# luigifreda/pyslam

Measured on AMD Instinct MI355X. Metric: RGB-D frames/sec fused (640x480, 5 mm voxel TSDF), higher is better.
Workload: dtype f32; 1 GPU; synthetic_640x480_5mm: synthetic 640x480 RGB-D @ 30 Hz stream, 5 mm TSDF (sdf_trunc 0.04 m, depth_trunc 4 m), 64 posed frames per step resident in HBM, Open3D ScalableTSDFVolume semantics; mode=multi-frame sweep (hv_tsdf_integrate_batch), units_allocated=31946, parity_pinned=False, clock_ramp_steps=60, full=False, build_digest=b0cf6d559847d2198173994ec0e18474b14d2966863d92f65f5939d93dcc7503

## Files before the change

include/hipvol.h:

```cpp
#ifndef PYSLAM_HIPVOL_H
#define PYSLAM_HIPVOL_H

#include <stdint.h>

#ifdef __cplusplus
extern "C" {
#endif

typedef struct hv_volume hv_volume;

typedef enum hv_status {
    HV_OK = 0,
    HV_ERR_INVALID = -1,
    HV_ERR_DEVICE = -2,
    HV_ERR_CAPACITY = -3,
    HV_ERR_MODE = -4
} hv_status;

typedef enum hv_mode {
    HV_MODE_VOXEL_GRID = 0,
    HV_MODE_VOXEL_SEMANTIC_GRID = 1,
    HV_MODE_VOXEL_SEMANTIC_PROBABILISTIC_GRID = 2,
    HV_MODE_TSDF = 3,
    HV_MODE_VOXEL_SEMANTIC_GRID2 = 11,
    HV_MODE_VOXEL_SEMANTIC_PROBABILISTIC_GRID2 = 12
} hv_mode;
typedef enum hv_loc { HV_HOST = 0, HV_DEVICE = 1 } hv_loc;
typedef enum hv_color_dtype { HV_COLOR_NONE = 0, HV_COLOR_U8 = 1, HV_COLOR_F32 = 2 } hv_color_dtype;
typedef enum hv_depth_dtype { HV_DEPTH_F32 = 0, HV_DEPTH_U16 = 1 } hv_depth_dtype;

typedef struct hv_config {
    int32_t mode;
    int32_t device;
    double voxel_size;
    double sdf_trunc;
    int32_t block_size;
    int32_t depth_sampling_stride;
    int64_t max_blocks;
    int64_t max_points;
} hv_config;


const char *hv_last_error(void);
int hv_device_count(void);
void hv_default_config(int32_t mode, hv_config *cfg);

int hv_create(const hv_config *cfg, hv_volume **out);
void hv_destroy(hv_volume *v);
int hv_reset(hv_volume *v);
int hv_synchronize(hv_volume *v);
int hv_set_stream(hv_volume *v, void *hip_stream);
void *hv_get_stream(hv_volume *v);

int hv_num_blocks(hv_volume *v, int64_t *n);
int hv_block_size(hv_volume *v, int32_t *bs);
int hv_reserve_blocks(hv_volume *v, int64_t new_max_blocks);
int hv_max_blocks(hv_volume *v, int64_t *n);
int hv_bytes_per_block(hv_volume *v, int64_t *bytes);
int hv_dropped_points(hv_volume *v, int64_t *n);

int hv_integrate_points(hv_volume *v, const float *points, int64_t n, const void *colors,
                        int32_t color_dtype, int32_t loc);
int hv_integrate_points_f64(hv_volume *v, const double *points, int64_t n, const void *colors,
                            int32_t color_dtype, int32_t loc);

int hv_integrate_rgbd_points(hv_volume *v, const void *depth, int32_t depth_dtype, double depth_scale,
                             const uint8_t *rgb, int32_t height, int32_t width, const double *intr,
                             const double *T_cw, double min_depth, double max_depth, int32_t loc);

int hv_integrate_rgbd_points_batch(hv_volume *v, const void *depth, int32_t depth_dtype, double depth_scale,
                                   const uint8_t *rgb, int32_t n_frames, int32_t height, int32_t width, const double *intr,
                                   const double *T_cw, double min_depth, double max_depth, int32_t loc);

int hv_remap(hv_volume *v, const void *src, int32_t src_kind, int32_t channels, int32_t height, int32_t width,
             const float *map_x, const float *map_y, int32_t linear, void *dst, int32_t loc);

int hv_filter_shadow_points(hv_volume *v, const float *depth, int32_t height, int32_t width, int32_t delta_x,
                            int32_t delta_y, float fill_value, float *out, int32_t loc);
int hv_filter_shadow_points_on_stream(hv_volume *v, const float *depth, int32_t height, int32_t width, int32_t delta_x,
                                      int32_t delta_y, float fill_value, float *out, void *stream);

int hv_get_voxels(hv_volume *v, int32_t min_count, float min_confidence, float *points,
                  float *colors, int64_t cap, int64_t *n, int32_t loc);
int hv_get_voxels_in_bb(hv_volume *v, const double *bbox, int32_t min_count, float min_confidence,
                        float *points, float *colors, int64_t cap, int64_t *n, int32_t loc);
int hv_get_voxels_in_frustum(hv_volume *v, const float *intr_f32, int32_t width, int32_t height,
                             const double *T_cw, float depth_max, float depth_min, int32_t min_count,
                             float min_confidence, float *points, float *colors, int64_t cap,
                             int64_t *n, int32_t loc);
int hv_carve(hv_volume *v, const float *intr_f32, int32_t width, int32_t height, const double *T_cw,
             float depth_max, float depth_min, const float *depth, float depth_threshold, int32_t loc);
int hv_remove_low_count_voxels(hv_volume *v, int32_t min_count);
int hv_size(hv_volume *v, int64_t *n);

int hv_dump_blocks(hv_volume *v, int32_t *keys, uint64_t *hashes, int32_t *counts, float *sums,
                   int64_t *n_blocks);
int hv_keys_from_points(hv_volume *v, const float *points, int64_t n, int32_t *voxel_keys,
                        int32_t *block_keys, int32_t *local_keys, uint64_t *block_hashes);

int hv_integrate_points_semantic(hv_volume *v, const void *points, int32_t point_dtype, int64_t n, const void *colors,
                                 int32_t color_dtype, const int32_t *class_ids, const int32_t *instance_ids,
                                 const float *depths, int32_t loc);
int hv_integrate_rgbd_semantic(hv_volume *v, const float *depth, const uint8_t *rgb, const int32_t *class_ids_image,
                               const int32_t *object_ids_image, int32_t height, int32_t width, const double *intr,
                               const double *T_cw, double min_depth, double max_depth, int32_t use_depths, int32_t loc);
int hv_get_voxels_semantic(hv_volume *v, int32_t min_count, float min_confidence, double *points, float *colors,
                           int32_t *class_ids, int32_t *object_ids, float *confidences, int64_t cap, int64_t *n);
int hv_get_voxels_semantic_in_bb(hv_volume *v, const double *bbox, int32_t min_count, float min_confidence, double *points,
                                 float *colors, int32_t *class_ids, int32_t *object_ids, float *confidences, int64_t cap,
                                 int64_t *n);
int hv_get_voxels_semantic_in_frustum(hv_volume *v, const float *intr_f32, int32_t width, int32_t height, const double *T_cw,
                                      float depth_max, float depth_min, int32_t min_count, float min_confidence, double *points,
                                      float *colors, int32_t *class_ids, int32_t *object_ids, float *confidences, int64_t cap,
                                      int64_t *n);
int hv_set_depth_threshold(hv_volume *v, float depth_threshold);
int hv_set_depth_decay_rate(hv_volume *v, float depth_decay_rate);
int hv_label_overflows(hv_volume *v, int64_t *n);
int hv_prob_nodes_used(hv_volume *v, int64_t *n);
int hv_assign_object_ids_to_instance_ids(hv_volume *v, const float *intr_f32, int32_t width, int32_t height, const double *T_cw,
                                         float depth_max, float depth_min, const int32_t *class_ids_image,
                                         const int32_t *instance_ids_image, const float *depth_image, float depth_threshold,
                                         int32_t do_carving, float min_vote_ratio, int32_t min_votes, int32_t *map_inst,
                                         int32_t *map_obj, int64_t cap, int64_t *n_map, int32_t loc);
int hv_assoc_vote(hv_volume *v, const float *intr_f32, int32_t width, int32_t height, const double *T_cw, float depth_max,
                  float depth_min, const int32_t *class_ids_image, const int32_t *instance_ids_image, const float *depth_image,
                  float depth_threshold, int32_t do_carving, int32_t loc);
int hv_assoc_pairs_fetch(hv_volume *v, uint64_t *pair_keys, int32_t *pair_counts, int64_t cap, int64_t *n_pairs);
int hv_assoc_pairs_set(hv_volume *v, const uint64_t *pair_keys, const int32_t *pair_counts, int64_t n_pairs);
int hv_assoc_pairs_export(hv_volume *v, int64_t *d_msg, int64_t cap);
int hv_assoc_pairs_import(hv_volume *v, const int64_t *d_msgs, int32_t world, int64_t cap);
int hv_assoc_decide(hv_volume *v, float min_vote_ratio, int32_t min_votes);
int hv_assoc_map_fetch(hv_volume *v, int32_t *map_inst, int32_t *map_obj, int64_t cap, int64_t *n_map);
int hv_remap_instance_ids_last(hv_volume *v, const int32_t *instance_ids, int32_t height, int32_t width, int32_t *out, int32_t loc);
int hv_semantic_fuse_keyframe(hv_volume *v, const float *depth, const uint8_t *rgb, const int32_t *class_ids_image,
                              const int32_t *instance_ids_image, int32_t height, int32_t width, const float *frustum_intr_f32,
                              float frustum_depth_max, float frustum_depth_min, const double *intr, const double *T_cw,
                              int32_t filter_shadow_points, int32_t use_instance_ids, float assoc_depth_threshold, int32_t do_carving,
                              float min_vote_ratio, int32_t min_votes, double min_depth, double max_depth, int32_t use_depths);
int32_t hv_peek_next_object_id(void);
void hv_set_next_object_id(int32_t id);
int hv_remap_instance_ids(hv_volume *v, const int32_t *instance_ids, int32_t height, int32_t width, const int32_t *map_inst,
                          const int32_t *map_obj, int64_t n_map, int32_t *out, int32_t loc);
int hv_object_segments_compute(hv_volume *v, int32_t min_count, float min_confidence, int64_t *n_rows, int64_t *n_objects);
int hv_object_segments_fetch(hv_volume *v, double *points, float *colors, int32_t *row_object_ids, int32_t *object_ids,
                             float *confidences, double *obbs);
int hv_compute_obb_pca(const double *points, int64_t n, double *obb);
int hv_merge_segments(hv_volume *v, int32_t instance_id1, int32_t instance_id2);
int hv_remove_segment(hv_volume *v, int32_t object_id);
int hv_remove_low_confidence_segments(hv_volume *v, int32_t min_confidence);
int hv_remove_low_confidence_voxels(hv_volume *v, float min_confidence);
int hv_dump_blocks_semantic(hv_volume *v, int32_t *keys, int32_t *ints, double *pos_sums, float *col_sums,
                            int64_t *n_blocks);
int hv_dump_blocks_semantic2(hv_volume *v, int32_t *keys, int32_t *ints, float *conf, double *pos_sums, float *col_sums,
                             int32_t *label_counts, int32_t *labels, float *log_probs, int32_t max_labels,
                             int64_t *n_blocks);
int hv_dump_marginals_semantic(hv_volume *v, float *object_confidences, float *class_confidences, int64_t *n_blocks);

int hv_tsdf_integrate(hv_volume *v, const void *depth, int32_t depth_dtype, const uint8_t *rgb,
                      int32_t height, int32_t width, const double *intr, const double *T_cw,
                      double depth_scale, double depth_trunc, int32_t loc);

int hv_tsdf_integrate_batch(hv_volume *v, const void *depth, int32_t depth_dtype, const uint8_t *rgb,
                            int32_t n_frames, int32_t height, int32_t width, const double *intr,
                            const double *T_cw, double depth_scale, double depth_trunc, int32_t loc);

int hv_tsdf_integrate_frames(hv_volume *v, const void *const *depth_frames, int32_t depth_dtype, const uint8_t *const *rgb_frames,
                             int32_t n_frames, int32_t height, int32_t width, const double *intr, const double *T_cw,
                             double depth_scale, double depth_trunc);

#define HV_TSDF_DEINTEGRATE_MAX_FRAMES 64
typedef struct hv_deintegrate_stats {
    int64_t units_listed;
    int64_t units_missing;
    int64_t voxels_removed;
    int64_t voxels_underflow;
} hv_deintegrate_stats;
int hv_tsdf_deintegrate(hv_volume *v, const void *depth, int32_t depth_dtype, const uint8_t *rgb, int32_t height, int32_t width,
                        const double *intr, const double *T_cw, double depth_scale, double depth_trunc, int32_t loc,
                        hv_deintegrate_stats *stats);
int hv_tsdf_deintegrate_batch(hv_volume *v, const void *depth, int32_t depth_dtype, const uint8_t *rgb, int32_t n_frames,
                              int32_t height, int32_t width, const double *intr, const double *T_cw, double depth_scale,
                              double depth_trunc, int32_t loc, hv_deintegrate_stats *stats);
int hv_tsdf_reintegrate_batch(hv_volume *v, const void *depth, int32_t depth_dtype, const uint8_t *rgb, int32_t n_frames,
                              int32_t height, int32_t width, const double *intr, const double *T_cw_old, const double *T_cw_new,
                              double depth_scale, double depth_trunc, int32_t loc, hv_deintegrate_stats *stats);

int hv_tsdf_set_rectify_maps(hv_volume *v, const float *map_x, const float *map_y, int32_t height, int32_t width, int32_t loc);

int hv_tsdf_set_color_order(hv_volume *v, int32_t bgr);

int hv_host_register(void *ptr, int64_t bytes);
int hv_host_unregister(void *ptr);

int hv_tsdf_set_tile(hv_volume *v, int32_t u0, int32_t v0, int32_t u1, int32_t v1);

int hv_set_owner(hv_volume *v, int32_t rank, int32_t world_size);
int hv_block_owner(const int32_t *block_keys, int64_t n, int32_t world_size, int32_t *owner);

int hv_tsdf_set_owner(hv_volume *v, int32_t rank, int32_t world_size);

int hv_tsdf_extract_mesh(hv_volume *v, double *vertices, double *vertex_colors, int64_t cap_vertices,
                         int32_t *triangles, int64_t cap_triangles, int64_t *n_vertices,
                         int64_t *n_triangles);
int hv_tsdf_extract_mesh_f32(hv_volume *v, float *vertices, float *vertex_colors, int64_t cap_vertices,
                             int32_t *triangles, int64_t cap_triangles, int64_t *n_vertices,
                             int64_t *n_triangles);
int hv_tsdf_extract_points(hv_volume *v, double *points, double *colors, int64_t cap, int64_t *n);
int hv_tsdf_extract_points_f32(hv_volume *v, float *points, float *colors, int64_t cap, int64_t *n);
int hv_tsdf_extract_point_normals(hv_volume *v, double *normals, int64_t cap, int64_t *n);

#define HV_RAYCAST_STEP_FRAC 0.8f
#define HV_RAYCAST_REFINE_ITERS 4
#define HV_RAYCAST_UNIT_EPS 0.01f
int hv_tsdf_ray_cast(hv_volume *v, int32_t height, int32_t width, const double *intr, const double *T_cw, double depth_min,
                     double depth_max, double weight_threshold, double depth_scale, float *depth, float *vertex, float *normal,
                     float *color, uint8_t *mask, int32_t loc);

#define HV_TRACK_MAX_LEVELS 8
#define HV_TRACK_MIN_INLIERS 6
#define HV_TRACK_PIVOT_REL 1e-10
#define HV_TRACK_CONVERGED 1e-6
#define HV_TRACK_TRACE_STRIDE 56
typedef struct hv_track_params {
    double depth_scale, depth_min, depth_max, weight_threshold;
    double depth_outlier_trunc;
    double depth_huber_delta;
    int32_t n_levels;
    int32_t iterations[HV_TRACK_MAX_LEVELS];
} hv_track_params;
typedef struct hv_track_result {
    double T_cw[16];
    double information[36];
    double fitness, inlier_rmse;
    int64_t inliers, valid;
    int32_t iterations[HV_TRACK_MAX_LEVELS];
    int32_t degenerate;
    int32_t success;
} hv_track_result;
int hv_tsdf_track(hv_volume *v, const void *depth, int32_t depth_dtype, int32_t height, int32_t width, const double *intr,
                  const double *T_cw_init, const hv_track_params *params, hv_track_result *result, double *trace, int64_t trace_cap,
                  int64_t *trace_rows, int32_t loc);

#define HV_TRACK_COLOR_TRACE_STRIDE 58
typedef struct hv_track_color_params {
    hv_track_params base;
    double intensity_weight;
    double intensity_huber_delta;
} hv_track_color_params;
typedef struct hv_track_color_result {
    hv_track_result base;
    int64_t photometric_inliers;
    double intensity_rmse;
} hv_track_color_result;
int hv_tsdf_track_color(hv_volume *v, const void *depth, int32_t depth_dtype, const uint8_t *color, int32_t height, int32_t width,
                        const double *intr, const double *T_cw_init, const hv_track_color_params *params, hv_track_color_result *result,
                        double *trace, int64_t trace_cap, int64_t *trace_rows, int32_t loc);

typedef struct hv_prune_stats {
    int64_t units_before, units_outside, units_empty, units_after;
} hv_prune_stats;
int hv_tsdf_prune(hv_volume *v, int32_t release_empty, const int32_t *unit_lo ,
                  const int32_t *unit_hi , hv_prune_stats *stats );

typedef struct hv_merge_stats {
    int64_t units_source, units_claimed, voxels_updated, voxels_trilinear, voxels_nearest;
} hv_merge_stats;
int hv_tsdf_integrate_volume(hv_volume *dst, hv_volume *src, const double *T_dst_src , hv_merge_stats *stats );

#define HV_REGISTER_MIN_INLIERS 6
#define HV_REGISTER_PIVOT_REL 1e-10
#define HV_REGISTER_CONVERGED 1e-6
#define HV_REGISTER_TRACE_STRIDE 54
typedef struct hv_register_params {
    double weight_threshold;
    double tsdf_band;
    double residual_trunc;
    double huber_delta;
    int32_t max_iterations;
    int32_t reserved;
} hv_register_params;
typedef struct hv_register_result {
    double T_dst_src[16];
    double information[36];
    double anchor[3];
    double fitness, inlier_rmse;
    int64_t inliers, candidates;
    int32_t iterations;
    int32_t success;
} hv_register_result;
int hv_tsdf_register_volume(hv_volume *dst, hv_volume *src, const double *T_init , const hv_register_params *params,
                            hv_register_result *result, double *trace, int64_t trace_cap, int64_t *trace_rows);

typedef enum hv_point_dtype { HV_F32 = 0, HV_F64 = 1 } hv_point_dtype;
#define HV_SAMPLE_OUTSIDE 0
#define HV_SAMPLE_UNOBSERVED 1
#define HV_SAMPLE_NEAREST 2
#define HV_SAMPLE_TRILINEAR 3
int hv_tsdf_sample_points(hv_volume *v, const void *points , int32_t point_dtype, int64_t n, double weight_threshold,
                          float *sdf , float *gradient , float *color , float *weight ,
                          uint8_t *status , int32_t loc);

#define HV_CHECK_INVALID 0
#define HV_CHECK_UNKNOWN 1
#define HV_CHECK_CONSISTENT 2
#define HV_CHECK_IN_FRONT 3
#define HV_CHECK_BEHIND 4
typedef struct hv_check_params {
    double depth_scale, depth_min, depth_max, weight_threshold, tolerance;
} hv_check_params;
typedef struct hv_check_stats {
    int64_t count[5];
} hv_check_stats;
int hv_tsdf_check_frame(hv_volume *v, const void *depth, int32_t depth_dtype, int32_t height, int32_t width, const double *intr,
                        const double *T_cw, const hv_check_params *params, float *sdf ,
                        uint8_t *cls , hv_check_stats *stats , int32_t loc);

#define HV_LOOKUP_MISSING 0
#define HV_LOOKUP_OWN 1
#define HV_LOOKUP_NEAR 2
#define HV_LOOKUP_INVALID 3
typedef struct hv_lookup_params {
    int32_t min_count;
// ... 94 lines not shown
```

pyslam_amd/_lib.py:

```python
import ctypes
import os

import numpy as np

from . import build as _build

_c = ctypes
_vp, _i64, _i32, _f32, _f64 = _c.c_void_p, _c.c_int64, _c.c_int32, _c.c_float, _c.c_double
_pi64 = _c.POINTER(_c.c_int64)
_pi32 = _c.POINTER(_c.c_int32)

HV_OK = 0
HV_MODE_VOXEL_GRID = 0
HV_MODE_VOXEL_SEMANTIC_GRID = 1
HV_MODE_VOXEL_SEMANTIC_PROBABILISTIC_GRID = 2
HV_MODE_TSDF = 3
HV_MODE_VOXEL_SEMANTIC_GRID2 = 11
HV_MODE_VOXEL_SEMANTIC_PROBABILISTIC_GRID2 = 12
HV_HOST, HV_DEVICE = 0, 1
HV_COLOR_NONE, HV_COLOR_U8, HV_COLOR_F32 = 0, 1, 2
HV_DEPTH_F32, HV_DEPTH_U16 = 0, 1


class HvConfig(_c.Structure):
# ... 102 lines not shown
        ("information", _f64 * 36),
        ("anchor", _f64 * 3),
        ("fitness", _f64),
        ("inlier_rmse", _f64),
        ("inliers", _i64),
        ("candidates", _i64),
        ("iterations", _i32),
        ("success", _i32),
    ]


HV_PACK_VERSION = 1
HV_PACK_HEADER_BYTES = 128


class HvPackInfo(_c.Structure):
    _fields_ = [("units", _i64), ("voxels", _i64), ("bytes", _i64)]


class HvPackedHeader(_c.Structure):
    _fields_ = [
        ("voxel_length", _f64),
        ("sdf_trunc", _f64),
        ("resolution", _i32),
        ("version", _i32),
        ("units", _i64),
        ("voxels", _i64),
        ("bytes", _i64),
    ]


HV_F32, HV_F64 = 0, 1
HV_SAMPLE_OUTSIDE, HV_SAMPLE_UNOBSERVED, HV_SAMPLE_NEAREST, HV_SAMPLE_TRILINEAR = 0, 1, 2, 3
HV_CHECK_INVALID, HV_CHECK_UNKNOWN, HV_CHECK_CONSISTENT, HV_CHECK_IN_FRONT, HV_CHECK_BEHIND = 0, 1, 2, 3, 4


class HvCheckParams(_c.Structure):
    _fields_ = [
        ("depth_scale", _f64),
        ("depth_min", _f64),
        ("depth_max", _f64),
        ("weight_threshold", _f64),
        ("tolerance", _f64),
    ]


class HvCheckStats(_c.Structure):
    _fields_ = [("count", _i64 * 5)]


HV_LOOKUP_MISSING, HV_LOOKUP_OWN, HV_LOOKUP_NEAR, HV_LOOKUP_INVALID = 0, 1, 2, 3


class HvLookupParams(_c.Structure):
    _fields_ = [("min_count", _i32), ("min_confidence", _f32), ("radius", _i32)]


class HvLookupStats(_c.Structure):
    _fields_ = [("points", _i64), ("own", _i64), ("near", _i64), ("missing", _i64), ("invalid", _i64)]


HV_DIST_UNKNOWN, HV_DIST_FREE, HV_DIST_INSIDE, HV_DIST_SITE = 0, 1, 2, 4
HV_DIST_MAX_SHAPE, HV_DIST_MAX_RADIUS = 4096, 1024


class HvDistanceParams(_c.Structure):
    _fields_ = [("origin", _i32 * 3), ("shape", _i32 * 3), ("radius", _i32), ("weight_threshold", _f64)]


class HvDistanceStats(_c.Structure):
    _fields_ = [("unknown", _i64), ("free", _i64), ("inside", _i64), ("sites", _i64), ("far", _i64)]


HV_COMPONENTS_MAX_MARGIN = 16


class HvComponentsStats(_c.Structure):
    _fields_ = [("units", _i64), ("sites", _i64), ("components", _i64), ("largest", _i64)]


class HvRemoveComponentsStats(_c.Structure):
    _fields_ = [("components", _i64), ("components_removed", _i64), ("sites", _i64), ("sites_removed", _i64), ("voxels_reset", _i64),
                ("units_changed", _i64), ("units_emptied", _i64)]


SIGNATURES = {
    "hv_last_error": (_c.c_char_p, []),
    "hv_device_count": (_i32, []),
    "hv_default_config": (None, [_i32, _c.POINTER(HvConfig)]),
    "hv_create": (_i32, [_c.POINTER(HvConfig), _c.POINTER(_vp)]),
    "hv_destroy": (None, [_vp]),
    "hv_reset": (_i32, [_vp]),
    "hv_synchronize": (_i32, [_vp]),
    "hv_set_stream": (_i32, [_vp, _vp]),
    "hv_get_stream": (_vp, [_vp]),
    "hv_num_blocks": (_i32, [_vp, _pi64]),
    "hv_block_size": (_i32, [_vp, _pi32]),
    "hv_reserve_blocks": (_i32, [_vp, _i64]),
    "hv_max_blocks": (_i32, [_vp, _pi64]),
    "hv_bytes_per_block": (_i32, [_vp, _pi64]),
    "hv_dropped_points": (_i32, [_vp, _pi64]),
    "hv_integrate_points": (_i32, [_vp, _vp, _i64, _vp, _i32, _i32]),
    "hv_integrate_points_f64": (_i32, [_vp, _vp, _i64, _vp, _i32, _i32]),
    "hv_integrate_rgbd_points": (_i32, [_vp, _vp, _i32, _f64, _vp, _i32, _i32, _vp, _vp, _f64, _f64, _i32]),
    "hv_integrate_rgbd_points_batch": (_i32, [_vp, _vp, _i32, _f64, _vp, _i32, _i32, _i32, _vp, _vp, _f64, _f64, _i32]),
    "hv_remap": (_i32, [_vp, _vp, _i32, _i32, _i32, _i32, _vp, _vp, _i32, _vp, _i32]),
    "hv_filter_shadow_points": (_i32, [_vp, _vp, _i32, _i32, _i32, _i32, _f32, _vp, _i32]),
    "hv_filter_shadow_points_on_stream": (_i32, [_vp, _vp, _i32, _i32, _i32, _i32, _f32, _vp, _vp]),
    "hv_get_voxels": (_i32, [_vp, _i32, _f32, _vp, _vp, _i64, _pi64, _i32]),
    "hv_get_voxels_in_bb": (_i32, [_vp, _vp, _i32, _f32, _vp, _vp, _i64, _pi64, _i32]),
    "hv_get_voxels_in_frustum": (_i32, [_vp, _vp, _i32, _i32, _vp, _f32, _f32, _i32, _f32, _vp, _vp, _i64, _pi64, _i32]),
    "hv_carve": (_i32, [_vp, _vp, _i32, _i32, _vp, _f32, _f32, _vp, _f32, _i32]),
    "hv_remove_low_count_voxels": (_i32, [_vp, _i32]),
    "hv_size": (_i32, [_vp, _pi64]),
    "hv_dump_blocks": (_i32, [_vp, _vp, _vp, _vp, _vp, _pi64]),
    "hv_keys_from_points": (_i32, [_vp, _vp, _i64, _vp, _vp, _vp, _vp]),
    "hv_integrate_points_semantic": (_i32, [_vp, _vp, _i32, _i64, _vp, _i32, _vp, _vp, _vp, _i32]),
    "hv_get_voxels_semantic": (_i32, [_vp, _i32, _f32, _vp, _vp, _vp, _vp, _vp, _i64, _pi64]),
    "hv_get_voxels_semantic_in_bb": (_i32, [_vp, _vp, _i32, _f32, _vp, _vp, _vp, _vp, _vp, _i64, _pi64]),
    "hv_get_voxels_semantic_in_frustum": (_i32, [_vp, _vp, _i32, _i32, _vp, _f32, _f32, _i32, _f32, _vp, _vp, _vp, _vp, _vp, _i64, _pi64]),
    "hv_set_depth_threshold": (_i32, [_vp, _f32]),
    "hv_dump_blocks_semantic": (_i32, [_vp, _vp, _vp, _vp, _vp, _pi64]),
    "hv_dump_blocks_semantic2": (_i32, [_vp, _vp, _vp, _vp, _vp, _vp, _vp, _vp, _vp, _i32, _pi64]),
    "hv_dump_marginals_semantic": (_i32, [_vp, _vp, _vp, _pi64]),
    "hv_set_depth_decay_rate": (_i32, [_vp, _f32]),
    "hv_integrate_rgbd_semantic": (_i32, [_vp, _vp, _vp, _vp, _vp, _i32, _i32, _vp, _vp, _f64, _f64, _i32, _i32]),
    "hv_label_overflows": (_i32, [_vp, _pi64]),
    "hv_prob_nodes_used": (_i32, [_vp, _pi64]),
    "hv_assign_object_ids_to_instance_ids": (_i32, [_vp, _vp, _i32, _i32, _vp, _f32, _f32, _vp, _vp, _vp, _f32, _i32, _f32, _i32,
                                                    _vp, _vp, _i64, _pi64, _i32]),
    "hv_assoc_vote": (_i32, [_vp, _vp, _i32, _i32, _vp, _f32, _f32, _vp, _vp, _vp, _f32, _i32, _i32]),
    "hv_assoc_pairs_fetch": (_i32, [_vp, _vp, _vp, _i64, _pi64]),
    "hv_assoc_pairs_set": (_i32, [_vp, _vp, _vp, _i64]),
    "hv_assoc_pairs_export": (_i32, [_vp, _vp, _i64]),
    "hv_assoc_pairs_import": (_i32, [_vp, _vp, _i32, _i64]),
    "hv_assoc_decide": (_i32, [_vp, _f32, _i32]),
    "hv_assoc_map_fetch": (_i32, [_vp, _vp, _vp, _i64, _pi64]),
    "hv_remap_instance_ids_last": (_i32, [_vp, _vp, _i32, _i32, _vp, _i32]),
    "hv_semantic_fuse_keyframe": (_i32, [_vp, _vp, _vp, _vp, _vp, _i32, _i32, _vp, _f32, _f32, _vp, _vp, _i32, _i32, _f32, _i32, _f32, _i32,
                                         _f64, _f64, _i32]),
    "hv_peek_next_object_id": (_i32, []),
    "hv_set_next_object_id": (None, [_i32]),
    "hv_remap_instance_ids": (_i32, [_vp, _vp, _i32, _i32, _vp, _vp, _i64, _vp, _i32]),
    "hv_object_segments_compute": (_i32, [_vp, _i32, _f32, _pi64, _pi64]),
    "hv_object_segments_fetch": (_i32, [_vp, _vp, _vp, _vp, _vp, _vp, _vp]),
    "hv_compute_obb_pca": (_i32, [_vp, _i64, _vp]),
    "hv_merge_segments": (_i32, [_vp, _i32, _i32]),
    "hv_remove_segment": (_i32, [_vp, _i32]),
    "hv_remove_low_confidence_segments": (_i32, [_vp, _i32]),
    "hv_remove_low_confidence_voxels": (_i32, [_vp, _f32]),
    "hv_tsdf_integrate": (_i32, [_vp, _vp, _i32, _vp, _i32, _i32, _vp, _vp, _f64, _f64, _i32]),
    "hv_tsdf_integrate_batch": (_i32, [_vp, _vp, _i32, _vp, _i32, _i32, _i32, _vp, _vp, _f64, _f64, _i32]),
    "hv_tsdf_integrate_frames": (_i32, [_vp, _vp, _i32, _vp, _i32, _i32, _i32, _vp, _vp, _f64, _f64]),
    "hv_tsdf_set_color_order": (_i32, [_vp, _i32]),
    "hv_host_register": (_i32, [_vp, _i64]),
    "hv_host_unregister": (_i32, [_vp]),
    "hv_tsdf_set_tile": (_i32, [_vp, _i32, _i32, _i32, _i32]),
    "hv_tsdf_set_rectify_maps": (_i32, [_vp, _vp, _vp, _i32, _i32, _i32]),
    "hv_tsdf_set_owner": (_i32, [_vp, _i32, _i32]),
    "hv_tsdf_extract_mesh": (_i32, [_vp, _vp, _vp, _i64, _vp, _i64, _pi64, _pi64]),
    "hv_tsdf_extract_mesh_f32": (_i32, [_vp, _vp, _vp, _i64, _vp, _i64, _pi64, _pi64]),
    "hv_tsdf_extract_points": (_i32, [_vp, _vp, _vp, _i64, _pi64]),
    "hv_tsdf_extract_points_f32": (_i32, [_vp, _vp, _vp, _i64, _pi64]),
    "hv_tsdf_extract_point_normals": (_i32, [_vp, _vp, _i64, _pi64]),
    "hv_tsdf_ray_cast": (_i32, [_vp, _i32, _i32, _vp, _vp, _f64, _f64, _f64, _f64, _vp, _vp, _vp, _vp, _vp, _i32]),
    "hv_tsdf_deintegrate": (_i32, [_vp, _vp, _i32, _vp, _i32, _i32, _vp, _vp, _f64, _f64, _i32, _c.POINTER(HvDeintegrateStats)]),
    "hv_tsdf_deintegrate_batch": (_i32, [_vp, _vp, _i32, _vp, _i32, _i32, _i32, _vp, _vp, _f64, _f64, _i32, _c.POINTER(HvDeintegrateStats)]),
    "hv_tsdf_reintegrate_batch": (_i32, [_vp, _vp, _i32, _vp, _i32, _i32, _i32, _vp, _vp, _vp, _f64, _f64, _i32,
                                         _c.POINTER(HvDeintegrateStats)]),
    "hv_tsdf_prune": (_i32, [_vp, _i32, _pi32, _pi32, _c.POINTER(HvPruneStats)]),
    "hv_tsdf_integrate_volume": (_i32, [_vp, _vp, _vp, _c.POINTER(HvMergeStats)]),
    "hv_tsdf_register_volume": (_i32, [_vp, _vp, _vp, _c.POINTER(HvRegisterParams), _c.POINTER(HvRegisterResult), _vp, _i64, _pi64]),
    "hv_tsdf_track": (_i32, [_vp, _vp, _i32, _i32, _i32, _vp, _vp, _vp, _vp, _vp, _i64, _pi64, _i32]),
    "hv_tsdf_track_color": (_i32, [_vp, _vp, _i32, _vp, _i32, _i32, _vp, _vp, _vp, _vp, _vp, _i64, _pi64, _i32]),
    "hv_tsdf_sample_points": (_i32, [_vp, _vp, _i32, _i64, _f64, _vp, _vp, _vp, _vp, _vp, _i32]),
    "hv_tsdf_check_frame": (_i32, [_vp, _vp, _i32, _i32, _i32, _vp, _vp, _c.POINTER(HvCheckParams), _vp, _vp, _c.POINTER(HvCheckStats), _i32]),
    "hv_lookup_points": (_i32, [_vp, _vp, _i32, _i64, _c.POINTER(HvLookupParams), _vp, _vp, _vp, _vp, _vp, _vp, _vp, _c.POINTER(HvLookupStats), _i32]),
    "hv_tsdf_distance_field": (_i32, [_vp, _c.POINTER(HvDistanceParams), _vp, _vp, _vp, _c.POINTER(HvDistanceStats), _i32]),
    "hv_tsdf_surface_components": (_i32, [_vp, _f64, _vp, _vp, _vp, _vp, _i64, _vp, _vp, _i64, _pi64, _pi64, _c.POINTER(HvComponentsStats), _i32]),
    "hv_tsdf_remove_components": (_i32, [_vp, _f64, _i64, _i32, _c.POINTER(HvRemoveComponentsStats)]),
    "hv_tsdf_dump": (_i32, [_vp, _vp, _vp, _vp, _vp, _pi64]),
    "hv_tsdf_touched": (_i32, [_vp, _vp, _i64, _pi64]),
    "hv_tsdf_export_numerators": (_i32, [_vp, _vp, _i64, _vp, _i32]),
    "hv_tsdf_import_numerators": (_i32, [_vp, _vp, _i64, _vp, _i32]),
    "hv_tsdf_unit_keys": (_i32, [_vp, _vp, _i64, _pi64]),
    "hv_tsdf_pack_size": (_i32, [_vp, _c.POINTER(HvPackInfo)]),
    "hv_tsdf_pack": (_i32, [_vp, _vp, _i64, _i32, _c.POINTER(HvPackInfo)]),
    "hv_tsdf_unpack": (_i32, [_vp, _vp, _i64, _i32, _c.POINTER(HvPackInfo)]),
    "hv_tsdf_packed_check": (_i32, [_vp, _i64, _c.POINTER(HvPackedHeader)]),
    "hv_tsdf_dirty_keys": (_i32, [_vp, _vp, _i64, _pi64]),
    "hv_tsdf_mark_merged": (_i32, [_vp]),
    "hv_set_owner": (_i32, [_vp, _i32, _i32]),
    "hv_block_owner": (_i32, [_vp, _i64, _i32, _vp]),
    "hv_merge_halo_plan": (_i32, [_vp, _vp, _i32, _i32, _vp, _vp, _i64, _pi64]),
    "hv_merge_halo_plan_held": (_i32, [_vp, _vp, _vp, _vp, _i32, _i32, _vp, _vp, _i64, _pi64]),
    "hv_merge_halo_pack": (_i32, [_vp, _vp, _i64, _vp, _i32]),
    "hv_merge_halo_unpack": (_i32, [_vp, _vp, _i64, _vp, _vp, _i32]),
    "hv_merge_halo_lists_device": (_i32, [_vp, _vp, _i64, _vp, _i64, _pi64, _pi64]),
    "hv_merge_halo_plan_device": (_i32, [_vp, _vp, _vp, _i64, _vp, _vp, _i64, _i32, _i32, _i32, _pi64]),
    "hv_merge_halo_plan_fetch": (_i32, [_vp, _vp, _vp, _i64, _pi64]),
    "hv_merge_halo_pack_planned": (_i32, [_vp, _i64, _i64, _vp]),
    "hv_merge_halo_unpack_planned": (_i32, [_vp, _i64, _i64, _vp]),
    "hv_profile_enable": (_i32, [_vp, _i32]),
    "hv_profile_read": (_i32, [_vp, _c.POINTER(_f64), _pi64, _pi64]),
    "hv_profile_read_launches": (_i32, [_vp, _vp, _i64, _pi64]),
}

_lib = None


class HipVolError(RuntimeError):
    """Raised for every non-zero hv_status; message = hv_last_error()."""


def library_path():
    return _build.LIB_PATH


def load():
    global _lib
    if _lib is not None:
        return _lib
    path = _build.LIB_PATH
    if not os.path.exists(path):
        _build.build(verbose=False)
    import torch

    lib = _c.CDLL(path)
    for name, (restype, argtypes) in SIGNATURES.items():
        fn = getattr(lib, name)
        fn.restype = restype
        fn.argtypes = argtypes
    _lib = lib
    return lib


def check(rc):
    if rc != HV_OK:
        msg = load().hv_last_error()
        raise HipVolError(msg.decode() if msg else f"hipvol error {rc}")


def ptr(a):
    if a is None:
        return None
    if isinstance(a, np.ndarray):
        return a.ctypes.data_as(_vp)
    if hasattr(a, "data_ptr"):
        return _vp(a.data_ptr())
    raise TypeError(f"unsupported buffer type {type(a)}")


def location(a):
    if a is not None and hasattr(a, "is_cuda") and a.is_cuda:
        return HV_DEVICE
    return HV_HOST
```

pyslam_amd/csrc/hv_common.h:

```cpp
#pragma once
#include <cstdint>
#include <cstdio>
#include <cstring>
#include <string>
#include <vector>

#include <hip/hip_runtime.h>

#include "hipvol.h"

#define HV_WAVE 64

void hv_set_error(const char *fmt, ...);

#define HV_HIP(call)                                                                               \
    do {                                                                                           \
        hipError_t e_ = (call);                                                                    \
        if (e_ != hipSuccess) {                                                                    \
            hv_set_error("%s failed: %s (%s:%d)", #call, hipGetErrorString(e_), __FILE__,          \
                         __LINE__);                                                                \
            return HV_ERR_DEVICE;                                                                  \
        }                                                                                          \
    } while (0)

#define HV_REQUIRE(cond, code, ...)                                                                \
    do {                                                                                           \
        if (!(cond)) {                                                                             \
            hv_set_error(__VA_ARGS__);                                                             \
            return (code);                                                                         \
        }                                                                                          \
    } while (0)

static constexpr int HV_KEY_BITS = 21;
static constexpr int32_t HV_KEY_BIAS = 1 << (HV_KEY_BITS - 1);
static constexpr uint64_t HV_KEY_MASK = (1ull << HV_KEY_BITS) - 1;
static constexpr uint64_t HV_EMPTY_KEY = ~0ull;

__host__ __device__ inline bool hv_key_in_range(int32_t x, int32_t y, int32_t z) {
    return x >= -HV_KEY_BIAS && x < HV_KEY_BIAS && y >= -HV_KEY_BIAS && y < HV_KEY_BIAS &&
           z >= -HV_KEY_BIAS && z < HV_KEY_BIAS;
}
__host__ __device__ inline uint64_t hv_pack_key(int32_t x, int32_t y, int32_t z) {
    return (uint64_t)(uint32_t)(x + HV_KEY_BIAS) | ((uint64_t)(uint32_t)(y + HV_KEY_BIAS) << HV_KEY_BITS) |
           ((uint64_t)(uint32_t)(z + HV_KEY_BIAS) << (2 * HV_KEY_BITS));
}
__host__ __device__ inline void hv_unpack_key(uint64_t k, int32_t &x, int32_t &y, int32_t &z) {
    x = (int32_t)(k & HV_KEY_MASK) - HV_KEY_BIAS;
    y = (int32_t)((k >> HV_KEY_BITS) & HV_KEY_MASK) - HV_KEY_BIAS;
    z = (int32_t)((k >> (2 * HV_KEY_BITS)) & HV_KEY_MASK) - HV_KEY_BIAS;
}
__host__ __device__ inline uint32_t hv_slot_hash(uint64_t k) {
    k ^= k >> 33;
    k *= 0xff51afd7ed558ccdull;
    k ^= k >> 33;
    k *= 0xc4ceb9fe1a85ec53ull;
    k ^= k >> 33;
    return (uint32_t)k;
}
__host__ __device__ inline int32_t hv_owner_of(uint64_t k, int32_t world) {
    k ^= k >> 29;
    k *= 0x9E3779B97F4A7C15ull;
    k ^= k >> 32;
    return (int32_t)((k >> 7) % (uint64_t)world);
}
__host__ __device__ inline uint64_t hv_reference_hash(int32_t x, int32_t y, int32_t z) {
    return (uint64_t)(int64_t)x ^ ((uint64_t)(int64_t)y << 1) ^ ((uint64_t)(int64_t)z << 2);
}

struct HvTable {
    unsigned long long *keys;
    int32_t *vals;
    unsigned long long *block_keys;
    int32_t *counters;
    uint32_t mask;
    int32_t max_blocks;
    void *prob_nodes;
    int32_t prob_node_cap;
};

struct HvBins {
    int32_t *cnt;
    uint32_t *inl;
    int32_t *touched;
    int32_t *len;
    unsigned long long *pg_keys;
    uint32_t *pg_data;
    uint32_t pg_mask;
    uint32_t epoch;
    int32_t touched_cap;
    int32_t idx_bits;
    int32_t parity;
};

enum {
    HV_CNT_BLOCKS = 0,
    HV_CNT_OVERFLOW = 1,
    HV_CNT_DROPPED = 2,
    HV_CNT_OUT = 5,
    HV_CNT_OUT2 = 6,
    HV_CNT_AUX = 7,
    HV_CNT_LABEL_OVERFLOW = 8,
    HV_CNT_PROB_NODES = 9,
    HV_CNT_TOUCH0 = 32,
    HV_CNT_TOUCH1 = 64,
    HV_CNT_COUNT = 96
};
#define HV_CNT_TOUCH(set) (HV_CNT_TOUCH0 + 32 * (set))
static constexpr int HV_TSDF_SETS = 2;
static constexpr size_t HV_CNT_TOUCH_SPAN_BYTES = sizeof(int32_t) * (32 * (HV_TSDF_SETS - 1) + 1);

#ifdef __HIPCC__
__device__ inline int32_t hv_table_find(const HvTable &t, uint64_t key) {
    uint32_t s = hv_slot_hash(key) & t.mask;
    for (uint32_t probe = 0; probe <= t.mask; ++probe) {
        const unsigned long long k = t.keys[s];
        if (k == key) return (int32_t)s;
        if (k == HV_EMPTY_KEY) return -1;
        s = (s + 1) & t.mask;
    }
    return -1;
}

__device__ inline int32_t hv_table_insert(const HvTable &t, uint64_t key) {
    uint32_t s = hv_slot_hash(key) & t.mask;
    for (uint32_t probe = 0; probe <= t.mask; ++probe) {
        unsigned long long k = t.keys[s];
        if (k == key) return (int32_t)s;
        if (k == HV_EMPTY_KEY) {
            k = atomicCAS(&t.keys[s], HV_EMPTY_KEY, (unsigned long long)key);
            if (k == HV_EMPTY_KEY) {
                const int32_t idx = atomicAdd(&t.counters[HV_CNT_BLOCKS], 1);
                if (idx >= t.max_blocks) {
                    atomicAdd(&t.counters[HV_CNT_OVERFLOW], 1);
                    return -1;
                }
                t.vals[s] = idx;
                t.block_keys[idx] = key;
                return (int32_t)s;
            }
            if (k == key) return (int32_t)s;
        }
        s = (s + 1) & t.mask;
    }
    atomicAdd(&t.counters[HV_CNT_OVERFLOW], 1);
    return -1;
}

__device__ inline int32_t hv_table_claim(const HvTable &t, uint64_t key, bool *is_new) {
    *is_new = false;
    uint32_t s = hv_slot_hash(key) & t.mask;
    for (uint32_t probe = 0; probe <= t.mask; ++probe) {
        unsigned long long k = t.keys[s];
        if (k == key) return (int32_t)s;
        if (k == HV_EMPTY_KEY) {
            k = atomicCAS(&t.keys[s], HV_EMPTY_KEY, (unsigned long long)key);
            if (k == HV_EMPTY_KEY) {
                *is_new = true;
                return (int32_t)s;
            }
            if (k == key) return (int32_t)s;
        }
        s = (s + 1) & t.mask;
    }
    atomicAdd(&t.counters[HV_CNT_OVERFLOW], 1);
    return -1;
}
__device__ inline void hv_table_assign(const HvTable &t, int32_t slot, uint64_t key, int32_t idx) {
    if (idx >= t.max_blocks) {
        atomicAdd(&t.counters[HV_CNT_OVERFLOW], 1);
        return;
    }
    t.vals[slot] = idx;
    t.block_keys[idx] = key;
}

__device__ inline int hv_lane_id() { return (int)(threadIdx.x & (HV_WAVE - 1)); }
__device__ __forceinline__ void hv_wave_lds_sync() {
    __builtin_amdgcn_fence(__ATOMIC_ACQ_REL, "wavefront");
    __builtin_amdgcn_wave_barrier();
}

__device__ inline int32_t hv_wave_append(int32_t *counter, bool pred) {
    const unsigned long long m = __ballot(pred);
    if (m == 0) return -1;
    const int lane = hv_lane_id();
    const int leader = __ffsll((long long)m) - 1;
    int32_t base = 0;
    if (lane == leader) base = atomicAdd(counter, (int32_t)__popcll(m));
    base = __shfl(base, leader);
    const unsigned long long lt = (lane == 0) ? 0ull : (~0ull >> (64 - lane));
    return pred ? base + (int32_t)__popcll(m & lt) : -1;
}

template <typename T>
__device__ __forceinline__ T hv_wave_sum(T x) {
#pragma unroll
    for (int o = HV_WAVE / 2; o > 0; o >>= 1) x += __shfl_xor(x, o, HV_WAVE);
    return x;
}
template <typename T>
__device__ __forceinline__ T hv_wave_min(T x) {
#pragma unroll
    for (int o = HV_WAVE / 2; o > 0; o >>= 1) x = min(x, __shfl_xor(x, o, HV_WAVE));
    return x;
}
template <typename T>
__device__ __forceinline__ T hv_wave_max(T x) {
#pragma unroll
    for (int o = HV_WAVE / 2; o > 0; o >>= 1) x = max(x, __shfl_xor(x, o, HV_WAVE));
    return x;
}

__device__ inline int32_t hv_keyset_insert(unsigned long long *keys, uint32_t mask, unsigned long long key, bool *is_new) {
    *is_new = false;
    uint32_t s = hv_slot_hash(key) & mask;
    for (uint32_t probe = 0; probe <= mask; ++probe) {
        unsigned long long k = keys[s];
        if (k == key) return (int32_t)s;
        if (k == HV_EMPTY_KEY) {
            k = atomicCAS(&keys[s], HV_EMPTY_KEY, key);
            if (k == HV_EMPTY_KEY) {
                *is_new = true;
                return (int32_t)s;
            }
            if (k == key) return (int32_t)s;
        }
        s = (s + 1) & mask;
    }
    return -1;
}
#endif

static constexpr int HV_TSDF_PLANES = 5;
static constexpr int HV_TSDF_R = 16;
static constexpr int HV_TSDF_RR = HV_TSDF_R * HV_TSDF_R;
static constexpr int HV_TSDF_RRR = HV_TSDF_RR * HV_TSDF_R;
static constexpr int HV_TSDF_PLANE_BYTES = HV_TSDF_RRR * 4;
static constexpr int HV_TSDF_UNIT_BYTES = HV_TSDF_PLANE_BYTES * HV_TSDF_PLANES;

__host__ __device__ __forceinline__ int hv_tsdf_word(int x, int y, int z) { return z * HV_TSDF_RR + x * HV_TSDF_R + y; }

#ifdef __HIPCC__
__device__ __forceinline__ bool hv_tsdf_unit_has_weight(const char *__restrict__ pool, int32_t unit, int lane) {
    const uint4 *w = (const uint4 *)(pool + (size_t)unit * HV_TSDF_UNIT_BYTES + HV_TSDF_PLANE_BYTES);
    bool seen = false;
    for (int k = 0; k < HV_TSDF_PLANE_BYTES / 1024 && !seen; k += 4) {
        const uint4 a = w[(k + 0) * 64 + lane], b = w[(k + 1) * 64 + lane], c = w[(k + 2) * 64 + lane], d = w[(k + 3) * 64 + lane];
        const uint32_t any = a.x | a.y | a.z | a.w | b.x | b.y | b.z | b.w | c.x | c.y | c.z | c.w | d.x | d.y | d.z | d.w;
        seen = __ballot(any != 0) != 0ull;
    }
    return seen;
}
#endif

struct __attribute__((aligned(16))) HvVoxel {
    int32_t count;
    float pos[3];
    float col[3];
    int32_t pad;
};
static_assert(sizeof(HvVoxel) == 32, "HvVoxel must be 32 bytes");

struct HvFrameParams {
    float sweep_k[16];
    float ext[12];
    float ext_scaled_col2[3];
    float fx, fy, cx, cy;
    float ffl_inv_x, ffl_inv_y;
    float voxel_length_f, half_voxel_length_f;
    float sdf_trunc_f, sdf_trunc_inv_f;
    float safe_width_f, safe_height_f;
    double unit_length;
    double pose[12];
    double fx_d, fy_d, cx_d, cy_d;
    double sdf_trunc_d;
    float depth_scale_f;
    double depth_trunc_d;
    int32_t H, W, stride;
    int32_t depth_is_u16;
    int32_t frame_id;
    int32_t tile_u0, tile_v0, tile_u1, tile_v1;
    int32_t tiled;
    int32_t owner_rank, owner_world;
    int32_t touch_box_bits;
    int32_t bgr;
};

struct HvStatus {
    int32_t blocks;
    int32_t overflow;
    int32_t seq;
    int32_t pad;
    int32_t assoc_flags;
    int32_t reserved[3];
};

#ifdef __HIPCC__
__device__ inline void hv_publish_status(const HvTable &t, HvStatus *status, int32_t seq) {
    volatile HvStatus *s = status;
    s->blocks = t.counters[HV_CNT_BLOCKS];
    s->overflow = t.counters[HV_CNT_OVERFLOW];
    __threadfence_system();
    s->seq = seq;
}
#endif

struct HvEventPair {
    hipEvent_t start, stop;
};

static inline bool hv_mode_is_semantic(int32_t mode) {
    return mode == HV_MODE_VOXEL_SEMANTIC_GRID || mode == HV_MODE_VOXEL_SEMANTIC_PROBABILISTIC_GRID || mode == HV_MODE_VOXEL_SEMANTIC_GRID2 ||
           mode == HV_MODE_VOXEL_SEMANTIC_PROBABILISTIC_GRID2;
}
static inline bool hv_mode_has_label_maps(int32_t mode) {
    return mode == HV_MODE_VOXEL_SEMANTIC_PROBABILISTIC_GRID || mode == HV_MODE_VOXEL_SEMANTIC_PROBABILISTIC_GRID2;
}

struct hv_volume {
    hv_config cfg;
    int device = 0;
    hipStream_t stream = nullptr;
    bool own_stream = true;

    HvTable table{};
    uint64_t table_capacity = 0;
    void *pool = nullptr;
    int64_t bytes_per_block = 0;
    int32_t *h_counters = nullptr;
    HvStatus *h_status = nullptr;
    HvStatus *d_status = nullptr;
    int32_t status_seq_issued = 0, status_seq_seen = 0;
    int64_t known_blocks = 0;
    int64_t max_new_per_call = 0;
    double avg_new_per_call = 0.0;
    bool status_exact = false;
    bool overflow_latched = false;

    int32_t *touched_stamp = nullptr;
    int32_t *touched_list = nullptr;
    uint64_t *touched_mask = nullptr;
    void *frame_px = nullptr;
    int color_bgr = 0;
    int touch_box_bits = 2048;
    int32_t frame_counter = 0;
    int32_t merge_stamp = 0;
    int32_t last_touch_parity = 0;
    bool touch_counters_clean = true;
    void *batch_buf = nullptr;
    size_t batch_buf_bytes = 0;
    void *batch_buf2 = nullptr;
    size_t batch_buf2_bytes = 0;
    hipEvent_t ev_h2d = nullptr;
    hipStream_t stream_aux = nullptr;
    hipEvent_t ev_prep = nullptr;
    hipEvent_t ev_presweep = nullptr;
    int batch_parity = 0;
    bool pipe_armed = false;
    uint64_t pipe_version = 0;
    float *rect_map_x = nullptr, *rect_map_y = nullptr;
    size_t rect_map_x_bytes = 0, rect_map_y_bytes = 0;
    int32_t rect_W = 0, rect_H = 0;
    void *rect_buf = nullptr;
    size_t rect_buf_bytes = 0;
    float *mult_table = nullptr;
    size_t mult_table_bytes = 0;
    float mult_key[4] = {0.f, 0.f, 0.f, 0.f};
    int32_t mult_W = 0, mult_H = 0;
    void *pinned_params[4] = {nullptr, nullptr, nullptr, nullptr};
    hipEvent_t params_ev[4] = {nullptr, nullptr, nullptr, nullptr};
    int params_idx = 0;
    int32_t tile[4] = {0, 0, 0, 0};
    int32_t owner_rank = 0, owner_world = 1;
    float sem_depth_threshold = 10.0f;
    float sem_depth_decay_rate = 0.07f;
    void *assoc_buf = nullptr;
    void *assoc_clean = nullptr;
    size_t assoc_clean_bytes = 0;
    size_t assoc_buf_bytes = 0;
    int32_t assoc_pending_cap = 0;
    int assoc_state = 0;
    void *segments_cache = nullptr;
    unsigned long long *occ = nullptr;
    void *semb_tasks = nullptr;
    size_t semb_tasks_bytes = 0;

    void *stage_a = nullptr;
    void *stage_b = nullptr;
    size_t stage_a_bytes = 0, stage_b_bytes = 0;
    void *hs_pinned[2] = {nullptr, nullptr};
    size_t hs_pinned_bytes[2] = {0, 0};
    hipEvent_t hs_pinned_done[2] = {nullptr, nullptr};
    void *hs_dev[2][2] = {{nullptr, nullptr}, {nullptr, nullptr}};
    size_t hs_dev_bytes[2][2] = {{0, 0}, {0, 0}};
    hipEvent_t hs_dev_ready[2] = {nullptr, nullptr};
    hipEvent_t hs_dev_free[2] = {nullptr, nullptr};
    bool hs_dev_free_valid[2] = {false, false};
    hipStream_t hs_stream = nullptr;
    int hs_set = 0, hs_slot = 0;

    uint32_t *sort_keys_in = nullptr, *sort_keys_out = nullptr;
    uint32_t *sort_vals_in = nullptr, *sort_vals_out = nullptr;
    void *sort_tmp = nullptr;
    size_t sort_tmp_bytes = 0;
    HvBins bins{};
    uint64_t bins_cap = 0;
    bool bins_clean = false;
    uint32_t bins_epoch = 0;
    void *bin_rec = nullptr;
    size_t bin_rec_bytes = 0;
    float *scratch_points = nullptr;
    float *scratch_colors = nullptr;
    int local_bits = 9;

    uint64_t content_version = 1;
    uint64_t mesh_cache_version = 0, points_cache_version = 0;
    int64_t mesh_cache_nv = 0, mesh_cache_nt = 0, points_cache_n = 0;
    bool mesh_cache_f32 = false, points_cache_f32 = false;
    void *unit_masks = nullptr;
    uint64_t unit_masks_version = 0;
    int unit_masks_units = 0;
    uint64_t extract_epoch = 1;
    int unit_cache_cap = 0;
    uint64_t unit_masks_epoch = 0, mc_epoch = 0, pc_epoch = 0;
    int32_t unit_masks_stamp = -1, mc_stamp = -1, pc_stamp = -1;
    int mc_units = 0, pc_units = 0;
    void *mc_cache = nullptr;
    void *pc_cache = nullptr;

    void *out_a = nullptr;
    void *out_b = nullptr;
    void *out_c = nullptr;
    size_t out_a_bytes = 0, out_b_bytes = 0, out_c_bytes = 0;
    void *raycast_buf = nullptr;
    size_t raycast_buf_bytes = 0;
    void *sample_buf = nullptr;
    size_t sample_buf_bytes = 0;
    void *dist_buf = nullptr;
    size_t dist_buf_bytes = 0;
    void *track_buf = nullptr;
    size_t track_buf_bytes = 0;
    void *shadow_ring = nullptr;
    int shadow_ring_next = 0;
    void *halo_plan = nullptr;
    size_t halo_plan_bytes = 0;
    int64_t halo_plan_n = 0;
    void *kf_buf = nullptr;
    size_t kf_buf_bytes = 0;
    void *deint_buf = nullptr;
    size_t deint_buf_bytes = 0;
    uint64_t deint_miss_cap = 0;

    bool profiling = false;
    std::vector<HvEventPair> events;
    size_t events_used = 0;
    int64_t prof_units = 0;
};

int hv_ensure_buffer(hv_volume *v, void **buf, size_t *cur, size_t want);
int hv_capacity_gate(hv_volume *v, bool *checked);
int hv_claims_fit(hv_volume *v);
static constexpr int HV_RETRY_CLAIM = 1000;
int hv_rekey_in_place(hv_volume *v, int64_t keep);
int32_t hv_next_status_seq(hv_volume *v);
void hv_launch_publish_status(hv_volume *v);
int hv_read_counters(hv_volume *v);
int hv_tsdf_require_whole_map(const hv_volume *v, const char *fn, const char *subject);
int hv_tsdf_drain(hv_volume *v, const char *fn, bool refuse_overflow, int64_t *used);
int hv_tsdf_key_order(hv_volume *v, int64_t used, std::vector<int32_t> &order, std::vector<int32_t> *xyz_in_order);
struct HvScratch {
    std::vector<void *> held;
    HvScratch() = default;
    HvScratch(const HvScratch &) = delete;
    HvScratch &operator=(const HvScratch &) = delete;
    ~HvScratch() {
        for (void *p : held) (void)hipFree(p);
    }
    template <typename T>
    hipError_t get(T **p, size_t n) {
        void *raw = nullptr;
        const hipError_t e = hipMalloc(&raw, (n > 0 ? n : 1) * sizeof(T));
        if (e == hipSuccess) held.push_back(raw);
        *p = (T *)raw;
        return e;
    }
};
int hv_rectify_frames_device(hv_volume *v, hipStream_t s, const void *d_depth, int32_t depth_dtype, const uint8_t *d_rgb, int n_frames,
                             int height, int width, void *d_depth_out, uint8_t *d_rgb_out);
int hv_stage_in(hv_volume *v, const void *src, size_t bytes, int32_t loc, int which, const void **dev);
int hv_stage_out(hv_volume *v, int32_t loc, size_t head, const size_t *sizes, void *const *user, void **dev, int count);
int hv_h2d(hv_volume *v, void *dst, const void *src, size_t bytes);
int hv_h2d_lazy(hv_volume *v, void *dst, const void *src, size_t bytes, bool *pending);
int hv_h2d_fence(hv_volume *v, bool pending);
int hv_stage_frames(hv_volume *v, const void *const *depth_ptrs, const void *depth_base, size_t depth_frame_bytes,
                    const void *const *rgb_ptrs, const void *rgb_base, size_t rgb_frame_bytes, int n_frames,
                    const void **d_depth, const void **d_rgb, int *set);
int hv_stage_frames_consumed(hv_volume *v, int set, hipStream_t consumer);
void hv_profile_begin(hv_volume *v);
void hv_profile_end(hv_volume *v, int64_t units);
void hv_invert4x4(const double *m, double *out);
int hv_ray_cast_launch(hv_volume *v, int32_t height, int32_t width, const double *intr, const double *T_cw, double depth_min,
                       double depth_max, double weight_threshold, double depth_scale, float *depth, float *vertex, float *normal,
                       float *color, uint8_t *mask);
void hv_segments_cache_free(void *cache);
void hv_launch_tsdf_import_claim(hv_volume *v, const int32_t *d_keys, int64_t k);
// ... 1 lines not shown
```

pyslam_amd/csrc/hv_core.hip:

```cpp
#include <cstdarg>
#include <cstdlib>

#include <immintrin.h>

#include <algorithm>
#include <array>
#include <condition_variable>
#include <functional>
#include <mutex>
#include <thread>

#include "hv_common.h"

static thread_local std::string g_last_error;

void hv_set_error(const char *fmt, ...) {
    char buf[1024];
    va_list ap;
    va_start(ap, fmt);
    vsnprintf(buf, sizeof(buf), fmt, ap);
    va_end(ap);
    g_last_error = buf;
}

// ... 498 lines not shown
    return n;
}

void hv_default_config(int32_t mode, hv_config *cfg) {
    memset(cfg, 0, sizeof(*cfg));
    cfg->mode = mode;
    cfg->device = 0;
    if (mode == HV_MODE_TSDF) {
        cfg->voxel_size = 0.015;
        cfg->sdf_trunc = 0.04;
        cfg->block_size = 16;
        cfg->depth_sampling_stride = 4;
        cfg->max_blocks = 1 << 16;
    } else {
        cfg->voxel_size = 0.015;
        cfg->sdf_trunc = 0.0;
        cfg->block_size = 8;
        cfg->depth_sampling_stride = 1;
        cfg->max_blocks = 1 << 19;
    }
    cfg->max_points = 2 * 1024 * 1024;
}

int hv_create(const hv_config *cfg, hv_volume **out) {
    HV_REQUIRE(cfg != nullptr && out != nullptr, HV_ERR_INVALID, "hv_create: null argument");
    HV_REQUIRE(cfg->mode == HV_MODE_VOXEL_GRID || hv_mode_is_semantic(cfg->mode) || cfg->mode == HV_MODE_TSDF, HV_ERR_INVALID,
               "hv_create: unsupported mode %d", cfg->mode);
    HV_REQUIRE(cfg->voxel_size > 0.0, HV_ERR_INVALID, "hv_create: voxel_size must be > 0");
    HV_REQUIRE(cfg->max_blocks > 0 && cfg->max_blocks < (1ll << 30), HV_ERR_INVALID,
               "hv_create: max_blocks out of range");
    HV_REQUIRE(cfg->max_points > 0 && cfg->max_points < (1ll << 31), HV_ERR_INVALID,
               "hv_create: max_points out of range");
    if (cfg->mode == HV_MODE_TSDF) {
        HV_REQUIRE(cfg->block_size == 16, HV_ERR_INVALID,
                   "hv_create: TSDF mode supports volume_unit_resolution 16 only (Open3D default)");
        HV_REQUIRE(cfg->sdf_trunc > 0.0, HV_ERR_INVALID, "hv_create: sdf_trunc must be > 0");
        HV_REQUIRE(cfg->depth_sampling_stride >= 1, HV_ERR_INVALID, "hv_create: bad sampling stride");
    } else {
        HV_REQUIRE(cfg->block_size >= 1 && cfg->block_size <= 16, HV_ERR_INVALID,
                   "hv_create: block_size must be in [1,16]");
    }
    int ndev = 0;
    HV_HIP(hipGetDeviceCount(&ndev));
    HV_REQUIRE(ndev > 0 && cfg->device >= 0 && cfg->device < ndev, HV_ERR_DEVICE,
               "hv_create: HIP device %d not available (%d devices)", cfg->device, ndev);
    hipDeviceProp_t prop;
    HV_HIP(hipGetDeviceProperties(&prop, cfg->device));
    HV_REQUIRE(strncmp(prop.gcnArchName, "gfx950", 6) == 0, HV_ERR_DEVICE,
               "hv_create: device %d is %s; this library is built for gfx950 only", cfg->device,
               prop.gcnArchName);
    HV_HIP(hipSetDevice(cfg->device));

    hv_volume *v = new hv_volume();
    v->cfg = *cfg;
    v->device = cfg->device;
    int rc = HV_OK;
    auto fail = [&](int code) {
        hv_destroy(v);
        return code;
    };
#define HV_TRY(call)                                                                               \
    do {                                                                                           \
        hipError_t e_ = (call);                                                                    \
        if (e_ != hipSuccess) {                                                                    \
            hv_set_error("%s failed: %s", #call, hipGetErrorString(e_));                           \
            return fail(HV_ERR_DEVICE);                                                            \
        }                                                                                          \
    } while (0)

    HV_TRY(hipStreamCreateWithFlags(&v->stream, hipStreamNonBlocking));
    v->own_stream = true;

    const int64_t nvox = (int64_t)cfg->block_size * cfg->block_size * cfg->block_size;
    v->bytes_per_block = cfg->mode == HV_MODE_TSDF ? nvox * 4 * HV_TSDF_PLANES
                         : hv_mode_has_label_maps(cfg->mode) ? nvox * 128
                         : hv_mode_is_semantic(cfg->mode)    ? nvox * 64
                                                             : nvox * (int64_t)sizeof(HvVoxel);
    if (hv_mode_has_label_maps(cfg->mode)) v->sem_depth_threshold = 5.0f;
    v->local_bits = 0;
    while ((1ll << v->local_bits) < nvox) v->local_bits++;

    v->table_capacity = next_pow2((uint64_t)cfg->max_blocks * 4);
    if (v->table_capacity < 1024) v->table_capacity = 1024;
    if (cfg->mode != HV_MODE_TSDF && (v->table_capacity << v->local_bits) >= (1ull << 32)) {
        hv_set_error("hv_create: max_blocks too large for 32-bit (slot, voxel) sort keys");
        return fail(HV_ERR_INVALID);
    }
    v->table.mask = (uint32_t)(v->table_capacity - 1);
    v->table.max_blocks = (int32_t)cfg->max_blocks;
    HV_TRY(hipMalloc(&v->table.keys, sizeof(uint64_t) * v->table_capacity));
    HV_TRY(hipMalloc(&v->table.vals, sizeof(int32_t) * v->table_capacity));
    HV_TRY(hipMalloc(&v->table.block_keys, sizeof(uint64_t) * cfg->max_blocks));
    HV_TRY(hipMalloc(&v->table.counters, sizeof(int32_t) * HV_CNT_COUNT));
    HV_TRY(hipHostMalloc((void **)&v->h_counters, sizeof(int32_t) * HV_CNT_COUNT));
    memset(v->h_counters, 0, sizeof(int32_t) * HV_CNT_COUNT);
    HV_TRY(hipHostMalloc((void **)&v->h_status, sizeof(HvStatus), hipHostMallocMapped));
    memset(v->h_status, 0, sizeof(HvStatus));
    HV_TRY(hipHostGetDevicePointer((void **)&v->d_status, v->h_status, 0));
    HV_TRY(hipMalloc(&v->pool, (size_t)cfg->max_blocks * v->bytes_per_block));

    if (cfg->mode == HV_MODE_TSDF) {
        HV_TRY(hipMalloc(&v->touched_stamp, sizeof(int32_t) * v->table_capacity));
        HV_TRY(hipMalloc(&v->touched_list, sizeof(int32_t) * HV_TSDF_SETS * cfg->max_blocks));
        HV_TRY(hipMalloc(&v->touched_mask, sizeof(uint64_t) * HV_TSDF_SETS * v->table_capacity));
        HV_TRY(hipMalloc(&v->frame_px, 8 * (size_t)cfg->max_points));
        if (const char *tb = getenv("HV_TSDF_TOUCH_BOX_BITS")) v->touch_box_bits = std::min(std::max(atoi(tb), 0), 2048);
    } else {
        HV_TRY(hipMalloc(&v->sort_keys_in, sizeof(uint32_t) * cfg->max_points));
        HV_TRY(hipMalloc(&v->sort_keys_out, sizeof(uint32_t) * cfg->max_points));
        HV_TRY(hipMalloc(&v->sort_vals_in, sizeof(uint32_t) * cfg->max_points));
        HV_TRY(hipMalloc(&v->sort_vals_out, sizeof(uint32_t) * cfg->max_points));
        HV_TRY(hipMalloc(&v->scratch_points, sizeof(float) * 3 * cfg->max_points));
        HV_TRY(hipMalloc(&v->scratch_colors, sizeof(float) * 3 * cfg->max_points));
        if (cfg->mode != HV_MODE_VOXEL_GRID) {
            const size_t occ_words = ((size_t)cfg->max_blocks * nvox + 63) / 64;
            HV_TRY(hipMalloc((void **)&v->occ, sizeof(unsigned long long) * occ_words));
            HV_TRY(hipMemsetAsync(v->occ, 0, sizeof(unsigned long long) * occ_words, v->stream));
        }
        if (hv_mode_has_label_maps(cfg->mode)) {
            int64_t cap = std::max<int64_t>(1 << 16, (int64_t)cfg->max_blocks * 4);
            if (const char *e = getenv("HV_PROB_NODE_CAP")) cap = std::max<int64_t>(atoll(e), 1);
            cap = std::min<int64_t>(cap, INT32_MAX / 2);
            HV_TRY(hipMalloc(&v->table.prob_nodes, (size_t)cap * 128));
            v->table.prob_node_cap = (int32_t)cap;
        }
    }
#undef HV_TRY
    HV_HIP(hipMemsetAsync(v->pool, 0, (size_t)cfg->max_blocks * v->bytes_per_block, v->stream));
    rc = hv_reset(v);
    if (rc != HV_OK) return fail(rc);
    *out = v;
    return HV_OK;
}

void hv_destroy(hv_volume *v) {
    if (!v) return;
    (void)hipSetDevice(v->device);
    if (v->stream_aux) (void)hipStreamSynchronize(v->stream_aux);
    if (v->stream) (void)hipStreamSynchronize(v->stream);
    if (v->hs_stream) (void)hipStreamSynchronize(v->hs_stream);
    for (int i = 0; i < 2; ++i) {
        if (v->hs_pinned[i]) (void)hipHostFree(v->hs_pinned[i]);
        for (int a = 0; a < 2; ++a)
            if (v->hs_dev[i][a]) (void)hipFree(v->hs_dev[i][a]);
        if (v->hs_pinned_done[i]) (void)hipEventDestroy(v->hs_pinned_done[i]);
        if (v->hs_dev_ready[i]) (void)hipEventDestroy(v->hs_dev_ready[i]);
        if (v->hs_dev_free[i]) (void)hipEventDestroy(v->hs_dev_free[i]);
    }
    if (v->hs_stream) (void)hipStreamDestroy(v->hs_stream);
    void *bufs[] = {v->table.keys, v->table.vals, v->table.block_keys, v->table.counters, v->pool,
                    v->touched_stamp, v->touched_list, v->touched_mask, v->frame_px,
                    v->stage_a, v->stage_b, v->sort_keys_in, v->sort_keys_out, v->sort_vals_in,
                    v->sort_vals_out, v->sort_tmp, v->scratch_points, v->scratch_colors, v->out_a,
                    v->out_b, v->out_c, v->rect_map_x, v->rect_map_y, v->rect_buf, v->batch_buf, v->assoc_buf, v->mult_table, v->bins.cnt, v->bins.inl, v->bins.touched, v->bins.len, v->bins.pg_keys, v->bins.pg_data, v->bin_rec, v->batch_buf2, v->unit_masks, v->occ, v->semb_tasks, v->table.prob_nodes, v->shadow_ring, v->mc_cache, v->pc_cache, v->kf_buf, v->halo_plan, v->raycast_buf, v->track_buf, v->deint_buf, v->sample_buf, v->dist_buf};
    for (void *b : bufs)
        if (b) (void)hipFree(b);
    if (v->h_counters) (void)hipHostFree(v->h_counters);
    if (v->h_status) (void)hipHostFree(v->h_status);
    hv_segments_cache_free(v->segments_cache);
    for (int i = 0; i < 4; ++i) {
        if (v->pinned_params[i]) (void)hipHostFree(v->pinned_params[i]);
        if (v->params_ev[i]) (void)hipEventDestroy(v->params_ev[i]);
    }
    for (auto &p : v->events) {
        (void)hipEventDestroy(p.start);
        (void)hipEventDestroy(p.stop);
    }
    if (v->ev_h2d) (void)hipEventDestroy(v->ev_h2d);
    if (v->ev_prep) (void)hipEventDestroy(v->ev_prep);
    if (v->ev_presweep) (void)hipEventDestroy(v->ev_presweep);
    if (v->stream_aux) (void)hipStreamDestroy(v->stream_aux);
    if (v->stream && v->own_stream) (void)hipStreamDestroy(v->stream);
    delete v;
}

int hv_reset(hv_volume *v) {
    HV_REQUIRE(v != nullptr, HV_ERR_INVALID, "hv_reset: null volume");
    HV_HIP(hipSetDevice(v->device));
    int64_t used = 0;
    if (v->frame_counter != 0 || v->h_counters[HV_CNT_BLOCKS] != 0) {
        int rc = hv_read_counters(v);
        if (rc != HV_OK) return rc;
        used = v->h_counters[HV_CNT_BLOCKS];
        if (used > v->cfg.max_blocks) used = v->cfg.max_blocks;
    }
    if (used > 0) HV_HIP(hipMemsetAsync(v->pool, 0, (size_t)used * v->bytes_per_block, v->stream));
    if (used > 0 && v->occ) {
        const int64_t nvox = (int64_t)v->cfg.block_size * v->cfg.block_size * v->cfg.block_size;
        HV_HIP(hipMemsetAsync(v->occ, 0, sizeof(unsigned long long) * (size_t)((used * nvox + 63) / 64), v->stream));
    }
    HV_HIP(hipMemsetAsync(v->table.keys, 0xFF, sizeof(uint64_t) * v->table_capacity, v->stream));
    HV_HIP(hipMemsetAsync(v->table.vals, 0xFF, sizeof(int32_t) * v->table_capacity, v->stream));
    HV_HIP(hipMemsetAsync(v->table.counters, 0, sizeof(int32_t) * HV_CNT_COUNT, v->stream));
    if (v->touched_stamp) HV_HIP(hipMemsetAsync(v->touched_stamp, 0, sizeof(int32_t) * v->table_capacity, v->stream));
    if (v->touched_mask) HV_HIP(hipMemsetAsync(v->touched_mask, 0, sizeof(uint64_t) * HV_TSDF_SETS * v->table_capacity, v->stream));
    memset(v->h_counters, 0, sizeof(int32_t) * HV_CNT_COUNT);
    v->content_version += 1;
    v->extract_epoch += 1;
    v->frame_counter = 0;
    v->merge_stamp = 0;
    HV_HIP(hipStreamSynchronize(v->stream));
    memset(v->h_status, 0, sizeof(HvStatus));
    v->status_seq_issued = v->status_seq_seen = 0;
    v->known_blocks = 0;
    v->max_new_per_call = 0;
    v->avg_new_per_call = 0.0;
    v->status_exact = true;
    v->bins_clean = false;
    v->last_touch_parity = 0;
    v->touch_counters_clean = true;
    v->overflow_latched = false;
    return HV_OK;
}

int hv_synchronize(hv_volume *v) {
    HV_REQUIRE(v != nullptr, HV_ERR_INVALID, "hv_synchronize: null volume");
    HV_HIP(hipStreamSynchronize(v->stream));
    return HV_OK;
}

int hv_set_stream(hv_volume *v, void *hip_stream) {
    HV_REQUIRE(v != nullptr, HV_ERR_INVALID, "hv_set_stream: null volume");
    HV_HIP(hipStreamSynchronize(v->stream));
    if (v->own_stream && v->stream) HV_HIP(hipStreamDestroy(v->stream));
    v->stream = (hipStream_t)hip_stream;
    v->own_stream = false;
    return HV_OK;
}

void *hv_get_stream(hv_volume *v) { return v ? (void *)v->stream : nullptr; }

__global__ void k_rehash(HvTable t, const unsigned long long *__restrict__ block_keys, int32_t n) {
    const int32_t idx = blockIdx.x * blockDim.x + threadIdx.x;
    if (idx >= n) return;
    const unsigned long long key = block_keys[idx];
    uint32_t s = hv_slot_hash(key) & t.mask;
    for (uint32_t probe = 0; probe <= t.mask; ++probe) {
        if (atomicCAS(&t.keys[s], HV_EMPTY_KEY, key) == HV_EMPTY_KEY) {
            t.vals[s] = idx;
            return;
        }
        s = (s + 1) & t.mask;
    }
}

__global__ void k_restamp(HvTable old_t, HvTable new_t, const int32_t *__restrict__ old_stamp, int32_t *__restrict__ new_stamp, int32_t n) {
    const int32_t idx = blockIdx.x * blockDim.x + threadIdx.x;
    if (idx >= n) return;
    const unsigned long long key = new_t.block_keys[idx];
    const int32_t so = hv_table_find(old_t, key), sn = hv_table_find(new_t, key);
    if (so >= 0 && sn >= 0) new_stamp[sn] = old_stamp[so];
}

static int hv_rebuild(hv_volume *v, int64_t new_max_blocks, int64_t keep);

int hv_reserve_blocks(hv_volume *v, int64_t new_max_blocks) {
    HV_REQUIRE(v != nullptr, HV_ERR_INVALID, "hv_reserve_blocks: null volume");
    if (new_max_blocks <= v->cfg.max_blocks) return HV_OK;
    return hv_rebuild(v, new_max_blocks, -1);
}

static int hv_rebuild(hv_volume *v, int64_t new_max_blocks, int64_t keep) {
    HV_REQUIRE(new_max_blocks < (1ll << 30), HV_ERR_INVALID, "hv_reserve_blocks: max_blocks out of range");
    const uint64_t new_cap = next_pow2((uint64_t)new_max_blocks * 4);
    HV_REQUIRE(v->cfg.mode == HV_MODE_TSDF || (new_cap << v->local_bits) < (1ull << 32), HV_ERR_CAPACITY,
               "hv_reserve_blocks: %lld blocks are too many for 32-bit (slot, voxel) sort keys", (long long)new_max_blocks);
    HV_HIP(hipSetDevice(v->device));
    HV_HIP(hipStreamSynchronize(v->stream));
    v->extract_epoch += 1;
    int rc = hv_read_counters(v);
    if (rc != HV_OK) return rc;
    int64_t used = std::min<int64_t>(v->h_counters[HV_CNT_BLOCKS], v->cfg.max_blocks);
    if (keep >= 0) used = std::min(used, keep);
    size_t free_b = 0, total_b = 0;
    HV_HIP(hipMemGetInfo(&free_b, &total_b));
    const size_t need = (size_t)new_max_blocks * v->bytes_per_block + new_cap * 24 + (size_t)new_max_blocks * 16;
    HV_REQUIRE(need < free_b, HV_ERR_CAPACITY, "hv_reserve_blocks: %.1f GiB needed, %.1f GiB of HBM free", need / 1073741824.0,
               free_b / 1073741824.0);
    void *pool = nullptr;
    unsigned long long *keys = nullptr, *block_keys = nullptr, *occ = nullptr;
    int32_t *vals = nullptr, *stamp = nullptr, *list = nullptr;
    uint64_t *mask = nullptr;
    auto release = [&]() {
        for (void *p : {pool, (void *)keys, (void *)vals, (void *)block_keys, (void *)stamp, (void *)list, (void *)mask, (void *)occ})
            if (p) (void)hipFree(p);
    };
#define HV_TRY_GROW(call)                                                                          \
    do {                                                                                           \
        hipError_t e_ = (call);                                                                    \
        if (e_ != hipSuccess) {                                                                    \
            hv_set_error("hv_reserve_blocks: %s failed: %s", #call, hipGetErrorString(e_));        \
            release();                                                                             \
            return HV_ERR_DEVICE;                                                                  \
        }                                                                                          \
    } while (0)
    HV_TRY_GROW(hipMalloc(&pool, (size_t)new_max_blocks * v->bytes_per_block));
    HV_TRY_GROW(hipMalloc((void **)&keys, sizeof(uint64_t) * new_cap));
    HV_TRY_GROW(hipMalloc((void **)&vals, sizeof(int32_t) * new_cap));
    HV_TRY_GROW(hipMalloc((void **)&block_keys, sizeof(uint64_t) * new_max_blocks));
    HV_TRY_GROW(hipMemcpyAsync(pool, v->pool, (size_t)used * v->bytes_per_block, hipMemcpyDeviceToDevice, v->stream));
    HV_TRY_GROW(hipMemsetAsync((char *)pool + (size_t)used * v->bytes_per_block, 0, (size_t)(new_max_blocks - used) * v->bytes_per_block,
                               v->stream));
    HV_TRY_GROW(hipMemcpyAsync(block_keys, v->table.block_keys, sizeof(uint64_t) * used, hipMemcpyDeviceToDevice, v->stream));
    if (v->occ) {
        const int64_t nvox = (int64_t)v->cfg.block_size * v->cfg.block_size * v->cfg.block_size;
        const size_t new_words = ((size_t)new_max_blocks * nvox + 63) / 64, used_words = ((size_t)used * nvox + 63) / 64;
        HV_TRY_GROW(hipMalloc((void **)&occ, sizeof(unsigned long long) * new_words));
        HV_TRY_GROW(hipMemsetAsync(occ, 0, sizeof(unsigned long long) * new_words, v->stream));
        if (used_words) HV_TRY_GROW(hipMemcpyAsync(occ, v->occ, sizeof(unsigned long long) * used_words, hipMemcpyDeviceToDevice, v->stream));
    }
    HV_TRY_GROW(hipMemsetAsync(keys, 0xFF, sizeof(uint64_t) * new_cap, v->stream));
    HV_TRY_GROW(hipMemsetAsync(vals, 0xFF, sizeof(int32_t) * new_cap, v->stream));
    HvTable nt = v->table;
    nt.keys = keys;
    nt.vals = vals;
    nt.block_keys = block_keys;
    nt.mask = (uint32_t)(new_cap - 1);
    nt.max_blocks = (int32_t)new_max_blocks;
    if (used > 0) hipLaunchKernelGGL(k_rehash, dim3((unsigned)((used + 255) / 256)), dim3(256), 0, v->stream, nt, block_keys, (int32_t)used);
    HV_TRY_GROW(hipGetLastError());
    if (v->cfg.mode == HV_MODE_TSDF) {
        HV_TRY_GROW(hipMalloc((void **)&stamp, sizeof(int32_t) * new_cap));
        HV_TRY_GROW(hipMalloc((void **)&list, sizeof(int32_t) * HV_TSDF_SETS * new_max_blocks));
        HV_TRY_GROW(hipMalloc((void **)&mask, sizeof(uint64_t) * HV_TSDF_SETS * new_cap));
        HV_TRY_GROW(hipMemsetAsync(stamp, 0, sizeof(int32_t) * new_cap, v->stream));
        HV_TRY_GROW(hipMemsetAsync(mask, 0, sizeof(uint64_t) * HV_TSDF_SETS * new_cap, v->stream));
        if (used > 0 && v->touched_stamp != nullptr)
            hipLaunchKernelGGL(k_restamp, dim3((unsigned)((used + 255) / 256)), dim3(256), 0, v->stream, v->table, nt,
                               (const int32_t *)v->touched_stamp, stamp, (int32_t)used);
        HV_TRY_GROW(hipGetLastError());
    }
    const int32_t fixed[2] = {(int32_t)used, 0};
    HV_TRY_GROW(hipMemcpyAsync(&v->table.counters[HV_CNT_BLOCKS], fixed, sizeof(fixed), hipMemcpyHostToDevice, v->stream));
    if (v->cfg.mode == HV_MODE_TSDF) {
        HV_TRY_GROW(hipMemsetAsync(&v->table.counters[HV_CNT_TOUCH0], 0, HV_CNT_TOUCH_SPAN_BYTES, v->stream));
        v->touch_counters_clean = true;
    }
    HV_TRY_GROW(hipStreamSynchronize(v->stream));
#undef HV_TRY_GROW
    if (v->cfg.mode == HV_MODE_TSDF) {
        (void)hipFree(v->touched_stamp);
        (void)hipFree(v->touched_list);
        (void)hipFree(v->touched_mask);
        v->touched_stamp = stamp;
        v->touched_list = list;
        v->touched_mask = mask;
    }
    if (occ) {
        (void)hipFree(v->occ);
        v->occ = occ;
    }
    (void)hipFree(v->pool);
    (void)hipFree(v->table.keys);
// ... 170 lines not shown
```

pyslam_amd/csrc/hv_tsdf.hip:

```cpp
#include <algorithm>
#include <array>
#include <cmath>
#include <cstring>
#include <numeric>

#include "hv_tsdf_device.h"

__global__ __launch_bounds__(256) void k_tsdf_multiplier_table(HvFrameParams P, float *__restrict__ out) {
    const int i = blockIdx.x * blockDim.x + threadIdx.x;
    if (i >= P.H * P.W) return;
    out[i] = hv_multiplier(P, i % P.W, i / P.W);
}


__global__ __launch_bounds__(256) void k_tsdf_prep_touch(HvTable table, int32_t *__restrict__ stamp,
                                                          int32_t *__restrict__ list, int parity,
                                                          const void *__restrict__ depth_raw,
                                                          const uint8_t *__restrict__ rgb,
                                                          uint2 *__restrict__ frame_px, HvFrameParams P,
                                                          int n_touch_blocks) {
    const int64_t npx = (int64_t)P.H * P.W;
    if ((int)blockIdx.x >= n_touch_blocks) {
        const int64_t i = (int64_t)((int)blockIdx.x - n_touch_blocks) * blockDim.x + threadIdx.x;
        if (i >= npx) return;
// ... 68 lines not shown
}

template <int ZB>
__device__ __forceinline__ void hv_tsdf_slabs(const HvFrameParams &P, const uint2 *__restrict__ frame_px, char *__restrict__ unit, int wordb,
                                              float (&pc)[4][3], float inc0, float inc1, float inc2) {
    float tv[ZB][4];
    uint32_t cv[ZB][4];
    unsigned mask = 0;
    bool near_plane = false;
#pragma unroll
    for (int c = 0; c < 4; ++c) {
        const float e = pc[c][2] + (float)ZB * inc2;
        near_plane |= (int)(fminf(pc[c][2], e) < 0x1p-10f) & (int)(fmaxf(pc[c][2], e) > -0x1p-10f);
    }
    if (P.tiled || __any(near_plane)) {
#pragma unroll
        for (int zz = 0; zz < ZB; ++zz) {
#pragma unroll
            for (int c = 0; c < 4; ++c) {
                if (hv_tsdf_eval_fast<true, false>(P, frame_px, nullptr, pc[c][0], pc[c][1], pc[c][2], tv[zz][c], cv[zz][c]))
                    mask |= 1u << (zz * 4 + c);
                pc[c][0] += inc0;
                pc[c][1] += inc1;
                pc[c][2] += inc2;
            }
        }
    } else {
#pragma unroll
        for (int zz = 0; zz < ZB; ++zz) {
#pragma unroll
            for (int c = 0; c < 4; ++c) {
                if (hv_tsdf_eval_fast<false, false>(P, frame_px, nullptr, pc[c][0], pc[c][1], pc[c][2], tv[zz][c], cv[zz][c]))
                    mask |= 1u << (zz * 4 + c);
                pc[c][0] += inc0;
                pc[c][1] += inc1;
                pc[c][2] += inc2;
            }
        }
    }
    float4 vt[ZB];
    uint4 vw[ZB], vr[ZB], vg[ZB], vb[ZB];
#pragma unroll
    for (int zz = 0; zz < ZB; ++zz) {
        if ((mask >> (zz * 4)) & 15u) {
            const int q = (wordb + zz * HV_TSDF_RR) >> 2;
            vt[zz] = ((const float4 *)(unit + 0 * HV_TSDF_PLANE_BYTES))[q];
            vw[zz] = ((const uint4 *)(unit + 1 * HV_TSDF_PLANE_BYTES))[q];
            vr[zz] = ((const uint4 *)(unit + 2 * HV_TSDF_PLANE_BYTES))[q];
            vg[zz] = ((const uint4 *)(unit + 3 * HV_TSDF_PLANE_BYTES))[q];
            vb[zz] = ((const uint4 *)(unit + 4 * HV_TSDF_PLANE_BYTES))[q];
        }
    }
#pragma unroll
    for (int zz = 0; zz < ZB; ++zz) {
        const unsigned m = (mask >> (zz * 4)) & 15u;
        if (m) {
            hv_tsdf_apply(m & 1u, tv[zz][0], cv[zz][0], vt[zz].x, vw[zz].x, vr[zz].x, vg[zz].x, vb[zz].x);
            hv_tsdf_apply(m & 2u, tv[zz][1], cv[zz][1], vt[zz].y, vw[zz].y, vr[zz].y, vg[zz].y, vb[zz].y);
            hv_tsdf_apply(m & 4u, tv[zz][2], cv[zz][2], vt[zz].z, vw[zz].z, vr[zz].z, vg[zz].z, vb[zz].z);
            hv_tsdf_apply(m & 8u, tv[zz][3], cv[zz][3], vt[zz].w, vw[zz].w, vr[zz].w, vg[zz].w, vb[zz].w);
            const int q = (wordb + zz * HV_TSDF_RR) >> 2;
            ((float4 *)(unit + 0 * HV_TSDF_PLANE_BYTES))[q] = vt[zz];
            ((uint4 *)(unit + 1 * HV_TSDF_PLANE_BYTES))[q] = vw[zz];
            ((uint4 *)(unit + 2 * HV_TSDF_PLANE_BYTES))[q] = vr[zz];
            ((uint4 *)(unit + 3 * HV_TSDF_PLANE_BYTES))[q] = vg[zz];
            ((uint4 *)(unit + 4 * HV_TSDF_PLANE_BYTES))[q] = vb[zz];
        }
    }
}

__global__ __launch_bounds__(256) void k_tsdf_integrate(HvTable table, const int32_t *__restrict__ list,
                                                         int parity, char *__restrict__ pool,
                                                         const uint2 *__restrict__ frame_px, HvFrameParams P,
                                                         HvStatus *status, int32_t status_seq) {
    int n_touched = table.counters[HV_CNT_TOUCH(parity)];
    if (n_touched > table.max_blocks) n_touched = table.max_blocks;
    if (blockIdx.x == 0 && threadIdx.x == 0) {
        table.counters[HV_CNT_TOUCH(parity ^ 1)] = 0;
        hv_publish_status(table, status, status_seq);
    }
    const int wave = threadIdx.x >> 6;
    const int lane = threadIdx.x & 63;
    const int x = lane >> 2;
    const int y0 = (lane & 3) << 2;
    const int z0 = wave * 4;
    const float inc0 = P.ext_scaled_col2[0], inc1 = P.ext_scaled_col2[1], inc2 = P.ext_scaled_col2[2];

    for (int t = blockIdx.x; t < n_touched; t += gridDim.x) {
        const int32_t slot = list[t];
        const int32_t idx = table.vals[slot];
        if (idx < 0) continue;
        int32_t ux, uy, uz;
        hv_unpack_key(table.keys[slot], ux, uy, uz);
        const double o0 = (double)ux * P.unit_length;
        const double o1 = (double)uy * P.unit_length;
        const double o2 = (double)uz * P.unit_length;
        const float p0 = (float)((double)(P.half_voxel_length_f + P.voxel_length_f * (float)x) + o0);
        const float p2 = (float)((double)P.half_voxel_length_f + o2);
        float pc[4][3];
#pragma unroll
        for (int c = 0; c < 4; ++c) {
            const float p1 = (float)((double)(P.half_voxel_length_f + P.voxel_length_f * (float)(y0 + c)) + o1);
#pragma unroll
            for (int r = 0; r < 3; ++r) {
                pc[c][r] = ((P.ext[r * 4 + 0] * p0 + P.ext[r * 4 + 1] * p1) + P.ext[r * 4 + 2] * p2) + P.ext[r * 4 + 3];
            }
        }
        for (int s = 0; s < z0; ++s) {
#pragma unroll
            for (int c = 0; c < 4; ++c) {
                pc[c][0] += inc0;
                pc[c][1] += inc1;
                pc[c][2] += inc2;
            }
        }
        char *unit = pool + (int64_t)idx * HV_TSDF_UNIT_BYTES;
        constexpr int ZB = 2;
#pragma unroll
        for (int zb = 0; zb < 4; zb += ZB) hv_tsdf_slabs<ZB>(P, frame_px, unit, hv_tsdf_word(x, y0, z0 + zb), pc, inc0, inc1, inc2);
    }
}

__device__ __forceinline__ void hv_touch_batch_patch(const HvTable &table, const HvFrameParams &P, const void *depth_f, const int patch,
                                                     HvTouchScratch &scratch, const int f, unsigned long long *__restrict__ frame_mask,
                                                     int32_t *__restrict__ stamp, int32_t *__restrict__ list, const int batch_stamp,
                                                     const int parity) {
    const unsigned long long fbit = 1ull << f;
    hv_touch_patch(table, P, depth_f, patch, scratch,
                   [&](unsigned long long key, int32_t ux, int32_t uy, int32_t uz) {
                       if (!hv_unit_hits_tile(P, ux, uy, uz)) return;
                       const int32_t slot = hv_table_insert(table, key);
                       if (slot < 0) return;
                       const unsigned long long seen = __hip_atomic_load(&frame_mask[slot], __ATOMIC_RELAXED, __HIP_MEMORY_SCOPE_AGENT);
                       const int32_t stamped = __hip_atomic_load(&stamp[slot], __ATOMIC_RELAXED, __HIP_MEMORY_SCOPE_AGENT);
                       if (!(seen & fbit)) atomicOr(&frame_mask[slot], fbit);
                       if (stamped != batch_stamp) {
                           const int32_t old = atomicExch(&stamp[slot], batch_stamp);
                           if (old != batch_stamp) {
                               const int32_t at = atomicAdd(&table.counters[HV_CNT_TOUCH(parity)], 1);
                               if (at < table.max_blocks) list[at] = slot;
                           }
                       }
                   });
}

__global__ __launch_bounds__(256) void k_tsdf_prep_touch_batch(HvTable table, int32_t *__restrict__ stamp,
                                                                unsigned long long *__restrict__ frame_mask,
                                                                int32_t *__restrict__ list, int batch_stamp,
                                                                const char *__restrict__ depth_raw, int64_t depth_stride,
                                                                const uint8_t *__restrict__ rgb,
                                                                uint2 *__restrict__ frame_px,
                                                                const HvFrameParams *__restrict__ Ps, int n_prep_blocks,
                                                                int n_touch_blocks, int n_frames, int parity,
                                                                const float *__restrict__ mult12) {
    int f, bx;
    const bool touch_role = (int)blockIdx.x < n_touch_blocks * n_frames;
    if (touch_role) {
        f = (int)blockIdx.x / n_touch_blocks;
        bx = (int)blockIdx.x % n_touch_blocks;
    } else {
        const int b = (int)blockIdx.x - n_touch_blocks * n_frames;
        f = b / n_prep_blocks;
        bx = b % n_prep_blocks;
    }
    const HvFrameParams &P = Ps[f];
    const int64_t npx = (int64_t)P.H * P.W;
    const void *depth_f = depth_raw + (int64_t)f * depth_stride;
    const uint8_t *rgb_f = rgb + (int64_t)f * npx * 3;
    if (!touch_role) {
        hv_pack_px4(P, f, ((int64_t)bx * blockDim.x + threadIdx.x) * 4, depth_f, rgb_f, frame_px, mult12);
        return;
    }
    __shared__ HvTouchScratch scratch[4];
    const int patch = bx * 4 + (int)(threadIdx.x / HV_WAVE);
    if (patch < hv_touch_patches(P))
        hv_touch_batch_patch(table, P, depth_f, patch, scratch[threadIdx.x / HV_WAVE], f, frame_mask, stamp, list, batch_stamp, parity);
}

typedef float hv_f2 __attribute__((ext_vector_type(2)));

__device__ __forceinline__ hv_f2 hv_fma2(hv_f2 a, hv_f2 b, hv_f2 c) { return __builtin_elementwise_fma(a, b, c); }
__device__ __forceinline__ hv_f2 hv_splat(float x) { return hv_f2{x, x}; }

struct HvSweepFrameK {
    hv_f2 e04, e15, e26, e37;
    float e8, e11;
    hv_f2 e9_10, i01;
    float i2;
};
__device__ __forceinline__ HvSweepFrameK hv_sweep_frame_k(const HvFrameParams *__restrict__ Ps, int f) {
    const float *k = Ps[f].sweep_k;
    return HvSweepFrameK{hv_f2{k[0], k[1]}, hv_f2{k[2], k[3]}, hv_f2{k[4], k[5]}, hv_f2{k[6], k[7]}, k[8], k[9], hv_f2{k[10], k[11]}, hv_f2{k[12], k[13]}, k[14]};
}

static constexpr unsigned HV_SWEEP_XCD_GROUP = 2;
__device__ __forceinline__ int hv_sweep_items(const int n_units, const int parts) {
    constexpr int G = HV_SWEEP_XCD_GROUP;
    return (n_units + 8 * G - 1) / (8 * G) * 8 * G * parts;
}
__device__ __forceinline__ void hv_sweep_item(const unsigned item, const unsigned parts, int &t, int &part) {
    constexpr unsigned G = HV_SWEEP_XCD_GROUP;
    const unsigned xcd = item & 7u, j = item >> 3;
    const unsigned g = j / (G * parts), within = j % (G * parts);
    t = (int)((g * 8 + xcd) * G + within / parts);
    part = (int)(within % parts);
}

static constexpr int HV_SWEEP_ZH = 4;
static constexpr int HV_SWEEP_SPLIT = 8;
static constexpr int HV_SWEEP_WAVES = 64 / HV_SWEEP_ZH / HV_SWEEP_SPLIT;
static constexpr int HV_SWEEP_WPE = 4;
static_assert(HV_SWEEP_ZH % 2 == 0, "voxels are folded in pairs");

struct HvSweepGather {
    uint2 rec[HV_SWEEP_ZH];
    float mm[HV_SWEEP_ZH], zk[HV_SWEEP_ZH];
    bool ok[HV_SWEEP_ZH];
};

__global__ __launch_bounds__(64 * HV_SWEEP_WAVES, HV_SWEEP_WPE) void k_tsdf_sweep(
    HvTable table, const int32_t *__restrict__ list, const unsigned long long *__restrict__ frame_mask,
    char *__restrict__ pool, const uint2 *__restrict__ frame_px, const HvFrameParams *__restrict__ Ps, int n_frames,
    int general, const float *__restrict__ mult, int parity) {
    constexpr int ZH = HV_SWEEP_ZH, SPLIT = HV_SWEEP_SPLIT, WAVES = HV_SWEEP_WAVES;
    int n_units = table.counters[HV_CNT_TOUCH(parity)];
    if (n_units > table.max_blocks) n_units = table.max_blocks;
    const int wave = __builtin_amdgcn_readfirstlane(threadIdx.x >> 6);
    const int lane = threadIdx.x & 63;
    const HvFrameParams &P0 = Ps[0];
    const float vl = P0.voxel_length_f, hl = P0.half_voxel_length_f;
    const double unit_length = P0.unit_length;
    const bool tiled = P0.tiled != 0;
    const int npx = P0.H * P0.W;
    const hv_f2 F = {P0.fx, P0.fy}, C = {P0.cx, P0.cy};
    const uint32_t lo = __float_as_uint(0.0001f);
    const uint32_t wlim = __float_as_uint(P0.safe_width_f) - lo, hlim = __float_as_uint(P0.safe_height_f) - lo;
    const uint32_t W24 = (uint32_t)P0.W;
    const float ntrunc = -P0.sdf_trunc_f, tinv = P0.sdf_trunc_inv_f;
    const __amdgpu_buffer_rsrc_t rs_m = __builtin_amdgcn_make_buffer_rsrc((void *)mult, 0, npx * 4, 0x00020000);
    const int n_items = hv_sweep_items(n_units, SPLIT);
    for (int item = blockIdx.x; item < n_items; item += gridDim.x) {
        int t, part;
        hv_sweep_item(item, SPLIT, t, part);
        if (t >= n_units) continue;
        const int task = part * WAVES + wave;
        const int cg = task & 3;
        const int z0 = (task >> 2) * ZH;
        const int x = cg * 4 + (lane >> 4);
        const int y = lane & 15;
        const int32_t slot = list[t];
        const int32_t idx = table.vals[slot];
        unsigned long long mask = frame_mask[slot];
        if (idx < 0 || mask == 0ull) continue;
        int32_t ux, uy, uz;
        hv_unpack_key(table.keys[slot], ux, uy, uz);
        const double o0 = (double)ux * unit_length, o1 = (double)uy * unit_length, o2 = (double)uz * unit_length;
        bool near = false;
        if (lane < n_frames && ((mask >> lane) & 1ull)) {
            const HvFrameParams &Pl = Ps[lane];
            const float bx = (float)((double)(hl + vl * (float)(cg * 4)) + o0), by = (float)((double)hl + o1),
                        bz = (float)((double)(hl + vl * (float)z0) + o2);
            const float zmin = (Pl.ext[8] * bx + Pl.ext[9] * by + Pl.ext[10] * bz + Pl.ext[11]) + fminf(Pl.ext[8] * (3.0f * vl), 0.f) +
                               fminf(Pl.ext[9] * (15.0f * vl), 0.f) + fminf(Pl.ext[10] * ((float)(ZH - 1) * vl), 0.f);
            near = !(zmin > 0.03f);
        }
        const bool near_any = __any(near);
        char *unit = pool + (int64_t)idx * HV_TSDF_UNIT_BYTES;
        const int wordb = z0 * HV_TSDF_RR + cg * 64 + lane;
        float vt[ZH];
        uint32_t vw[ZH];
#pragma unroll
        for (int zz = 0; zz < ZH; ++zz) {
            const int q = wordb + zz * HV_TSDF_RR;
            vt[zz] = ((const float *)(unit + 0 * HV_TSDF_PLANE_BYTES))[q];
            vw[zz] = ((const uint32_t *)(unit + 1 * HV_TSDF_PLANE_BYTES))[q];
        }
        const float p0 = (float)((double)(hl + vl * (float)x) + o0);
        const float p1 = (float)((double)(hl + vl * (float)y) + o1);
        const float p2 = (float)((double)hl + o2);
        bool heavy = false;
#pragma unroll
        for (int zz = 0; zz < ZH; ++zz) heavy |= vw[zz] >= (1u << 24) - 64u;
        unsigned dirty = 0;
        if (general || tiled || near_any || __any(heavy)) {
            uint32_t vr[ZH], vg[ZH], vb[ZH];
#pragma unroll
            for (int zz = 0; zz < ZH; ++zz) {
                const int q = wordb + zz * HV_TSDF_RR;
                vr[zz] = ((const uint32_t *)(unit + 2 * HV_TSDF_PLANE_BYTES))[q];
                vg[zz] = ((const uint32_t *)(unit + 3 * HV_TSDF_PLANE_BYTES))[q];
                vb[zz] = ((const uint32_t *)(unit + 4 * HV_TSDF_PLANE_BYTES))[q];
            }
            while (mask) {
                const int f = __ffsll((long long)mask) - 1;
                mask &= mask - 1;
                const HvFrameParams &P = Ps[f];
                const uint2 *px = frame_px + (int64_t)f * npx;
                const float inc0 = P.ext_scaled_col2[0], inc1 = P.ext_scaled_col2[1], inc2 = P.ext_scaled_col2[2];
                float pc0 = ((P.ext[0] * p0 + P.ext[1] * p1) + P.ext[2] * p2) + P.ext[3];
                float pc1 = ((P.ext[4] * p0 + P.ext[5] * p1) + P.ext[6] * p2) + P.ext[7];
                float pc2 = ((P.ext[8] * p0 + P.ext[9] * p1) + P.ext[10] * p2) + P.ext[11];
                for (int s = 0; s < z0; ++s) {
                    pc0 += inc0;
                    pc1 += inc1;
                    pc2 += inc2;
                }
#pragma unroll
                for (int zz = 0; zz < ZH; ++zz) {
                    float tv;
                    uint32_t cv;
                    const bool ok = hv_tsdf_eval_fast<true, true>(P, px, mult, pc0, pc1, pc2, tv, cv);
                    pc0 += inc0;
                    pc1 += inc1;
                    pc2 += inc2;
                    hv_tsdf_apply(ok, tv, cv, vt[zz], vw[zz], vr[zz], vg[zz], vb[zz]);
                    if (ok) dirty |= 1u << zz;
                }
            }
#pragma unroll
            for (int zz = 0; zz < ZH; ++zz) {
                if (dirty & (1u << zz)) {
                    const int q = wordb + zz * HV_TSDF_RR;
                    ((float *)(unit + 0 * HV_TSDF_PLANE_BYTES))[q] = vt[zz];
                    ((uint32_t *)(unit + 1 * HV_TSDF_PLANE_BYTES))[q] = vw[zz];
                    ((uint32_t *)(unit + 2 * HV_TSDF_PLANE_BYTES))[q] = vr[zz];
                    ((uint32_t *)(unit + 3 * HV_TSDF_PLANE_BYTES))[q] = vg[zz];
                    ((uint32_t *)(unit + 4 * HV_TSDF_PLANE_BYTES))[q] = vb[zz];
                }
            }
            continue;
        }
        hv_f2 VT[ZH / 2], WF[ZH / 2];
        uint32_t arb[ZH], ag[ZH];
#pragma unroll
        for (int zp = 0; zp < ZH / 2; ++zp) {
            VT[zp] = hv_f2{vt[2 * zp], vt[2 * zp + 1]};
            WF[zp] = hv_f2{(float)vw[2 * zp], (float)vw[2 * zp + 1]};
            arb[2 * zp] = arb[2 * zp + 1] = ag[2 * zp] = ag[2 * zp + 1] = 0u;
        }
        auto project_frame = [&](const HvSweepFrameK K, const int f, HvSweepFrameK &Knext, const unsigned long long rest,
                                 HvSweepGather &g) __attribute__((always_inline)) {
            const __amdgpu_buffer_rsrc_t rs_px = __builtin_amdgcn_make_buffer_rsrc((void *)(frame_px + (int64_t)f * npx), 0, npx * 8, 0x00020000);
            const hv_f2 INC = K.i01;
            const float inc2 = K.i2;
            hv_f2 XY = ((K.e04 * p0 + K.e15 * p1) + K.e26 * p2) + K.e37;
            const hv_f2 Z12 = K.e9_10 * hv_f2{p1, p2};
            float Z = ((K.e8 * p0 + Z12.x) + Z12.y) + K.e11;
            __builtin_amdgcn_sched_barrier(0);
            Knext = hv_sweep_frame_k(Ps, rest ? __ffsll((long long)rest) - 1 : f);
            __builtin_amdgcn_sched_barrier(0);
            for (int s = 0; s < z0; ++s) {
                XY += INC;
                Z += inc2;
            }
#pragma unroll
            for (int k = 0; k < ZH; ++k) {
                float r = __builtin_amdgcn_rcpf(Z);
                const float e = fmaf(-Z, r, 1.0f);
                r = fmaf(e, r, r);
                const hv_f2 A = XY * F;
                const hv_f2 R = hv_splat(r), NZ = hv_splat(-Z);
                hv_f2 Q = A * R;
                hv_f2 REM = hv_fma2(NZ, Q, A);
                Q = hv_fma2(REM, R, Q);
                REM = hv_fma2(NZ, Q, A);
                Q = hv_fma2(REM, R, Q);
                const hv_f2 UV = (Q + C) + hv_splat(0.5f);
                const bool in_u = (__float_as_uint(UV.x) - lo) < wlim;
                const bool in_v = (__float_as_uint(UV.y) - lo) < hlim;
                g.ok[k] = (int)(Z > 0.0f) & (int)in_u & (int)in_v;
                const uint32_t u = (uint32_t)(int)UV.x, v = (uint32_t)(int)UV.y;
                const uint32_t off = __umul24(v, W24) + u;
                g.rec[k] = __builtin_bit_cast(uint2, __builtin_amdgcn_raw_buffer_load_b64(rs_px, (int)(off << 3), 0, 0));
                g.mm[k] = __builtin_bit_cast(float, __builtin_amdgcn_raw_buffer_load_b32(rs_m, (int)(off << 2), 0, 0));
                g.zk[k] = Z;
                XY += INC;
                Z += inc2;
            }
        };
        auto apply_frame = [&](const HvSweepGather &g) __attribute__((always_inline)) {
#pragma unroll
            for (int zp = 0; zp < ZH / 2; ++zp) {
                const int k0 = 2 * zp, k1 = 2 * zp + 1;
                const float da = __uint_as_float(g.rec[k0].x), db = __uint_as_float(g.rec[k1].x);
                const float sa = (da - g.zk[k0]) * g.mm[k0], sb = (db - g.zk[k1]) * g.mm[k1];
                const bool oka = (int)g.ok[k0] & (int)(da > 0.0f) & (int)(sa > ntrunc);
                const bool okb = (int)g.ok[k1] & (int)(db > 0.0f) & (int)(sb > ntrunc);
                if (!__any((int)oka | (int)okb)) continue;
                const hv_f2 T = {fminf(sa * tinv, 1.0f), fminf(sb * tinv, 1.0f)};
                const hv_f2 W1 = WF[zp] + hv_splat(1.0f);
                const hv_f2 NUM = VT[zp] * WF[zp] + T;
                hv_f2 R = {__builtin_amdgcn_rcpf(W1.x), __builtin_amdgcn_rcpf(W1.y)};
                const hv_f2 E = hv_fma2(-W1, R, hv_splat(1.0f));
                R = hv_fma2(E, R, R);
                hv_f2 Q = NUM * R;
                hv_f2 REM = hv_fma2(-W1, Q, NUM);
                Q = hv_fma2(REM, R, Q);
                REM = hv_fma2(-W1, Q, NUM);
                Q = hv_fma2(REM, R, Q);
                VT[zp].x = oka ? Q.x : VT[zp].x;
                VT[zp].y = okb ? Q.y : VT[zp].y;
                WF[zp].x = oka ? W1.x : WF[zp].x;
                WF[zp].y = okb ? W1.y : WF[zp].y;
                const uint32_t ca = oka ? g.rec[k0].y : 0u, cb = okb ? g.rec[k1].y : 0u;
                arb[k0] += ca & 0x00ff00ffu; ag[k0] += ca & 0x0000ff00u;
                arb[k1] += cb & 0x00ff00ffu; ag[k1] += cb & 0x0000ff00u;
            }
        };
        HvSweepFrameK ka = hv_sweep_frame_k(Ps, __ffsll((long long)mask) - 1), kb = ka;
        HvSweepGather g;
        while (true) {
            const int fa = __ffsll((long long)mask) - 1;
            mask &= mask - 1;
            project_frame(ka, fa, kb, mask, g);
            apply_frame(g);
            if (!mask) break;
            const int fb = __ffsll((long long)mask) - 1;
            mask &= mask - 1;
            project_frame(kb, fb, ka, mask, g);
            apply_frame(g);
            if (!mask) break;
        }
#pragma unroll
        for (int zz = 0; zz < ZH; ++zz) {
            const float wfz = (zz & 1) ? WF[zz / 2].y : WF[zz / 2].x;
            const uint32_t nw = (uint32_t)wfz;
            if (nw != vw[zz]) {
                const int q = wordb + zz * HV_TSDF_RR;
                ((float *)(unit + 0 * HV_TSDF_PLANE_BYTES))[q] = (zz & 1) ? VT[zz / 2].y : VT[zz / 2].x;
                ((uint32_t *)(unit + 1 * HV_TSDF_PLANE_BYTES))[q] = nw;
                ((uint32_t *)(unit + 2 * HV_TSDF_PLANE_BYTES))[q] += arb[zz] & 0xffffu;
                ((uint32_t *)(unit + 3 * HV_TSDF_PLANE_BYTES))[q] += ag[zz] >> 8;
                ((uint32_t *)(unit + 4 * HV_TSDF_PLANE_BYTES))[q] += arb[zz] >> 16;
            }
        }
    }
}

template <int ZS>
__global__ __launch_bounds__(64, 4) void k_tsdf_sweep_column(
    HvTable table, const int32_t *__restrict__ list, const unsigned long long *__restrict__ frame_mask,
    char *__restrict__ pool, const uint2 *__restrict__ frame_px, const HvFrameParams *__restrict__ Ps, int n_frames,
    int general, const float *__restrict__ mult, int parity) {
    constexpr int GV = 4;
    static_assert(ZS == 1 || ZS == 2, "whole columns or z halves");
    constexpr int ZH = 16 / ZS;
    constexpr int NG = ZH / GV;
    constexpr int PARTS = 4 * ZS;
    typedef uint32_t hv_u3 __attribute__((ext_vector_type(3)));
    int n_units = table.counters[HV_CNT_TOUCH(parity)];
    if (n_units > table.max_blocks) n_units = table.max_blocks;
    const int lane = threadIdx.x & 63;
    const HvFrameParams &P0 = Ps[0];
    const float vl = P0.voxel_length_f, hl = P0.half_voxel_length_f;
    const double unit_length = P0.unit_length;
    const int npx = P0.H * P0.W;
    const hv_f2 F = {P0.fx, P0.fy}, C = {P0.cx, P0.cy};
    const float lo_uf = fmaxf(0.0001f, (float)P0.tile_u0), lo_vf = fmaxf(0.0001f, (float)P0.tile_v0);
    const float hi_uf = fminf(P0.safe_width_f, (float)P0.tile_u1), hi_vf = fminf(P0.safe_height_f, (float)P0.tile_v1);
    const uint32_t lo_u = __float_as_uint(lo_uf), lo_v = __float_as_uint(lo_vf);
    const uint32_t lim_u = hi_uf > lo_uf ? __float_as_uint(hi_uf) - lo_u : 0u, lim_v = hi_vf > lo_vf ? __float_as_uint(hi_vf) - lo_v : 0u;
    const uint32_t W24 = (uint32_t)P0.W;
    const float ntrunc = -P0.sdf_trunc_f, tinv = P0.sdf_trunc_inv_f;
    const float near_z = fmaxf(0.03f, 1.25f * P0.sdf_trunc_f);
    const int n_items = hv_sweep_items(n_units, PARTS);
    for (int item = blockIdx.x; item < n_items; item += gridDim.x) {
        int t, part;
        hv_sweep_item(item, PARTS, t, part);
        if (t >= n_units) continue;
        const int z0 = ZS == 1 ? 0 : (part >> 2) * ZH;
        const int32_t slot = list[t];
        const int cg = part & 3;
        const int x = cg * 4 + (lane >> 4);
        const int y = lane & 15;
        const int32_t idx = table.vals[slot];
        unsigned long long mask = frame_mask[slot];
        if (idx < 0 || mask == 0ull) continue;
        int32_t ux, uy, uz;
        hv_unpack_key(table.keys[slot], ux, uy, uz);
        const double o0 = (double)ux * unit_length, o1 = (double)uy * unit_length, o2 = (double)uz * unit_length;
        bool near = false;
        bool interior = false;
        if (lane < n_frames && ((mask >> lane) & 1ull)) {
            const HvFrameParams &Pl = Ps[lane];
            const float bx = (float)((double)(hl + vl * (float)(cg * 4)) + o0), by = (float)((double)hl + o1),
                        bz = (float)((double)(hl + vl * (float)z0) + o2);
            const float zmin = (Pl.ext[8] * bx + Pl.ext[9] * by + Pl.ext[10] * bz + Pl.ext[11]) + fminf(Pl.ext[8] * (3.0f * vl), 0.f) +
                               fminf(Pl.ext[9] * (15.0f * vl), 0.f) + fminf(Pl.ext[10] * ((float)(ZH - 1) * vl), 0.f);
            near = !(zmin > near_z);
            if (!near) {
                float umin = 3.0e38f, umax = -3.0e38f, vmin = 3.0e38f, vmax = -3.0e38f;
#pragma unroll
                for (int c = 0; c < 8; ++c) {
                    const float qx = bx + ((c & 1) ? 3.0f * vl : 0.0f), qy = by + ((c & 2) ? 15.0f * vl : 0.0f), qz = bz + ((c & 4) ? (float)(ZH - 1) * vl : 0.0f);
                    const float c2 = Pl.ext[8] * qx + Pl.ext[9] * qy + Pl.ext[10] * qz + Pl.ext[11];
                    const float rz = 1.0f / c2;
                    const float cu = (Pl.ext[0] * qx + Pl.ext[1] * qy + Pl.ext[2] * qz + Pl.ext[3]) * F.x * rz + C.x + 0.5f;
                    const float cv = (Pl.ext[4] * qx + Pl.ext[5] * qy + Pl.ext[6] * qz + Pl.ext[7]) * F.y * rz + C.y + 0.5f;
                    umin = fminf(umin, cu); umax = fmaxf(umax, cu);
                    vmin = fminf(vmin, cv); vmax = fmaxf(vmax, cv);
                }
                interior = umin >= lo_uf + 2.0f && umax <= hi_uf - 2.0f && vmin >= lo_vf + 2.0f && vmax <= hi_vf - 2.0f;
            }
        }
        const unsigned long long interior_mask = __ballot(interior);
        const bool near_any = __any(near);
        char *unit = pool + (int64_t)idx * HV_TSDF_UNIT_BYTES;
        const int wordb = z0 * HV_TSDF_RR + cg * 64 + lane;
        const float p0 = (float)((double)(hl + vl * (float)x) + o0);
        const float p1 = (float)((double)(hl + vl * (float)y) + o1);
        const float p2 = (float)((double)hl + o2);
        if (general || near_any) {
#pragma unroll 1
            for (int zz = 0; zz < ZH; ++zz) {
                const int q = wordb + zz * HV_TSDF_RR;
                float vt = ((const float *)(unit + 0 * HV_TSDF_PLANE_BYTES))[q];
                uint32_t vw = ((const uint32_t *)(unit + 1 * HV_TSDF_PLANE_BYTES))[q];
                uint32_t vr = ((const uint32_t *)(unit + 2 * HV_TSDF_PLANE_BYTES))[q];
                uint32_t vg = ((const uint32_t *)(unit + 3 * HV_TSDF_PLANE_BYTES))[q];
                uint32_t vb = ((const uint32_t *)(unit + 4 * HV_TSDF_PLANE_BYTES))[q];
                bool dirty = false;
                unsigned long long m = mask;
#pragma unroll 1
                while (m) {
                    const int f = __ffsll((long long)m) - 1;
                    m &= m - 1;
                    const HvFrameParams &P = Ps[f];
                    const float inc0 = P.ext_scaled_col2[0], inc1 = P.ext_scaled_col2[1], inc2 = P.ext_scaled_col2[2];
                    float pc0 = ((P.ext[0] * p0 + P.ext[1] * p1) + P.ext[2] * p2) + P.ext[3];
                    float pc1 = ((P.ext[4] * p0 + P.ext[5] * p1) + P.ext[6] * p2) + P.ext[7];
                    float pc2 = ((P.ext[8] * p0 + P.ext[9] * p1) + P.ext[10] * p2) + P.ext[11];
#pragma unroll 1
                    for (int s = 0; s < z0 + zz; ++s) {
                        pc0 += inc0;
                        pc1 += inc1;
                        pc2 += inc2;
                    }
                    float tv;
                    uint32_t cv;
                    const uint2 *px_f = (const uint2 *)((const uint32_t *)frame_px + (int64_t)f * npx * 3);
                    const bool ok = hv_tsdf_eval_fast<true, true, true>(P, px_f, mult, pc0, pc1, pc2, tv, cv);
                    hv_tsdf_apply(ok, tv, cv, vt, vw, vr, vg, vb);
                    dirty |= ok;
                }
                if (dirty) {
                    ((float *)(unit + 0 * HV_TSDF_PLANE_BYTES))[q] = vt;
                    ((uint32_t *)(unit + 1 * HV_TSDF_PLANE_BYTES))[q] = vw;
                    ((uint32_t *)(unit + 2 * HV_TSDF_PLANE_BYTES))[q] = vr;
                    ((uint32_t *)(unit + 3 * HV_TSDF_PLANE_BYTES))[q] = vg;
                    ((uint32_t *)(unit + 4 * HV_TSDF_PLANE_BYTES))[q] = vb;
                }
            }
            continue;
        }
        float S[ZH];
        uint32_t arb[ZH], agn[ZH];
#pragma unroll
        for (int k = 0; k < ZH; ++k) {
            S[k] = 0.0f;
            arb[k] = agn[k] = 0u;
        }
        struct Group {
            hv_u3 rec[GV];
            float zk[GV];
            bool inimg[GV];
        };
        hv_f2 XY, INC;
        float Z, inc2;
        __amdgpu_buffer_rsrc_t rs_px;
        auto begin_frame = [&](const HvSweepFrameK K, const int f, HvSweepFrameK &Knext, const unsigned long long rest) __attribute__((always_inline)) {
            rs_px = __builtin_amdgcn_make_buffer_rsrc((void *)((const uint32_t *)frame_px + (int64_t)f * npx * 3), 0, npx * 12, 0x00020000);
            INC = K.i01;
            inc2 = K.i2;
            XY = ((K.e04 * p0 + K.e15 * p1) + K.e26 * p2) + K.e37;
            const hv_f2 Z12 = K.e9_10 * hv_f2{p1, p2};
            Z = ((K.e8 * p0 + Z12.x) + Z12.y) + K.e11;
            if (ZS == 2 && z0 != 0) {
#pragma unroll
                for (int sidx = 0; sidx < ZH; ++sidx) {
                    XY += INC;
                    Z += inc2;
                }
            }
            __builtin_amdgcn_sched_barrier(0);
            Knext = hv_sweep_frame_k(Ps, rest ? __ffsll((long long)rest) - 1 : f);
            __builtin_amdgcn_sched_barrier(0);
        };
        bool frame_checked = true;
        auto project = [&](Group &g) __attribute__((always_inline)) {
#pragma unroll
            for (int k = 0; k < GV; ++k) {
                float r = __builtin_amdgcn_rcpf(Z);
                const float e = fmaf(-Z, r, 1.0f);
                r = fmaf(e, r, r);
                const hv_f2 A = XY * F;
                const hv_f2 R = hv_splat(r), NZ = hv_splat(-Z);
                hv_f2 Q = A * R;
                hv_f2 REM = hv_fma2(NZ, Q, A);
                Q = hv_fma2(REM, R, Q);
                const hv_f2 UV = (Q + C) + hv_splat(0.5f);
                bool in = true;
                if (frame_checked) {
                    asm volatile("" ::: "memory");
                    const bool in_u = (__float_as_uint(UV.x) - lo_u) < lim_u;
                    const bool in_v = (__float_as_uint(UV.y) - lo_v) < lim_v;
                    in = (int)in_u & (int)in_v;
                }
                g.inimg[k] = in;
                const uint32_t u = (uint32_t)(int)UV.x, v = (uint32_t)(int)UV.y;
                const uint32_t off = __umul24(v, W24) + u;
                g.rec[k] = __builtin_bit_cast(hv_u3, __builtin_amdgcn_raw_buffer_load_b96(rs_px, (int)__umul24(off, 12u), 0, 0));
                g.zk[k] = Z;
                XY += INC;
                Z += inc2;
            }
        };
        auto fold = [&](const Group &g, const int gi) __attribute__((always_inline)) {
#pragma unroll
            for (int k = 0; k < GV; ++k) {
                const int z = gi * GV + k;
                const float sdf = (__uint_as_float(g.rec[k].x) - g.zk[k]) * __uint_as_float(g.rec[k].z);
                const bool ok = (int)g.inimg[k] & (int)(sdf > ntrunc);
                if (ok) {
                    asm volatile("" ::: "memory");
                    S[z] += fminf(sdf * tinv, 1.0f);
                    arb[z] += g.rec[k].y & 0x00ff00ffu;
                    agn[z] += g.rec[k].y & 0xff00ff00u;
                }
            }
        };
        HvSweepFrameK ka = hv_sweep_frame_k(Ps, __ffsll((long long)mask) - 1), kb = ka;
        auto fold_frame = [&](const HvSweepFrameK K, const int f, HvSweepFrameK &Knext, const unsigned long long rest) __attribute__((always_inline)) {
            begin_frame(K, f, Knext, rest);
            frame_checked = !((interior_mask >> f) & 1ull);
            Group ga, gb;
            project(ga);
#pragma unroll
            for (int gi = 0; gi < NG; gi += 2) {
                project(gb);
                __builtin_amdgcn_sched_barrier(0);
                fold(ga, gi);
                __builtin_amdgcn_sched_barrier(0);
                if (gi + 2 < NG) project(ga);
                __builtin_amdgcn_sched_barrier(0);
                fold(gb, gi + 1);
                __builtin_amdgcn_sched_barrier(0);
            }
        };
        while (true) {
            const int fa = __ffsll((long long)mask) - 1;
            mask &= mask - 1;
            fold_frame(ka, fa, kb, mask);
            if (!mask) break;
            const int fb = __ffsll((long long)mask) - 1;
            mask &= mask - 1;
            fold_frame(kb, fb, ka, mask);
            if (!mask) break;
        }
#pragma unroll
        for (int z4 = 0; z4 < ZH; z4 += 4) {
            float vt[4];
            uint32_t vw[4];
#pragma unroll
            for (int k = 0; k < 4; ++k) {
                if (agn[z4 + k] >> 24) {
                    const int q = wordb + (z4 + k) * HV_TSDF_RR;
                    vt[k] = ((const float *)(unit + 0 * HV_TSDF_PLANE_BYTES))[q];
                    vw[k] = ((const uint32_t *)(unit + 1 * HV_TSDF_PLANE_BYTES))[q];
                }
            }
#pragma unroll
            for (int k = 0; k < 4; ++k) {
                const int z = z4 + k;
                const uint32_t n = agn[z] >> 24;
                if (n) {
                    const int q = wordb + z * HV_TSDF_RR;
                    const uint32_t nw = vw[k] + n;
                    ((float *)(unit + 0 * HV_TSDF_PLANE_BYTES))[q] = (vt[k] * (float)vw[k] + S[z]) / (float)nw;
                    ((uint32_t *)(unit + 1 * HV_TSDF_PLANE_BYTES))[q] = nw;
                    ((uint32_t *)(unit + 2 * HV_TSDF_PLANE_BYTES))[q] += arb[z] & 0xffffu;
                    ((uint32_t *)(unit + 3 * HV_TSDF_PLANE_BYTES))[q] += (agn[z] >> 8) & 0xffffu;
                    ((uint32_t *)(unit + 4 * HV_TSDF_PLANE_BYTES))[q] += arb[z] >> 16;
                }
            }
        }
    }
}

__global__ __launch_bounds__(256) void k_upload_words(const uint4 *__restrict__ src, uint4 *__restrict__ dst, int n16) {
    for (int i = threadIdx.x; i < n16; i += 256) dst[i] = src[i];
}

__global__ __launch_bounds__(1024) void k_tsdf_batch_finish(HvTable table, const int32_t *__restrict__ list,
                                                             unsigned long long *__restrict__ frame_mask, int parity,
                                                             HvStatus *status, int32_t status_seq) {
    int n_units = table.counters[HV_CNT_TOUCH(parity)];
    if (n_units > table.max_blocks) n_units = table.max_blocks;
    __syncthreads();
    for (int base = 0; base < n_units; base += 8 * (int)blockDim.x) {
        int32_t slot[8];
#pragma unroll
        for (int k = 0; k < 8; ++k) {
            const int t = base + k * (int)blockDim.x + (int)threadIdx.x;
            slot[k] = t < n_units ? list[t] : -1;
        }
#pragma unroll
        for (int k = 0; k < 8; ++k)
            if (slot[k] >= 0) frame_mask[slot[k]] = 0ull;
    }
    if (threadIdx.x == 0) {
        table.counters[HV_CNT_TOUCH(parity)] = 0;
        hv_publish_status(table, status, status_seq);
    }
}

int make_frame_params(hv_volume *v, int H, int W, const double *intr, const double *T_cw,
                             double depth_scale, double depth_trunc, int depth_dtype, HvFrameParams *P) {
    memset(P, 0, sizeof(*P));
    for (int r = 0; r < 3; ++r)
        for (int c = 0; c < 4; ++c) P->ext[r * 4 + c] = (float)T_cw[r * 4 + c];
    P->voxel_length_f = (float)v->cfg.voxel_size;
    P->half_voxel_length_f = P->voxel_length_f * 0.5f;
    for (int r = 0; r < 3; ++r) P->ext_scaled_col2[r] = P->ext[r * 4 + 2] * P->voxel_length_f;
    for (int c = 0; c < 4; ++c) {
        P->sweep_k[2 * c] = P->ext[c];
        P->sweep_k[2 * c + 1] = P->ext[4 + c];
    }
    P->sweep_k[8] = P->ext[8];
    P->sweep_k[9] = P->ext[11];
    P->sweep_k[10] = P->ext[9];
    P->sweep_k[11] = P->ext[10];
    for (int r = 0; r < 3; ++r) P->sweep_k[12 + r] = P->ext_scaled_col2[r];
    P->fx = (float)intr[0];
    P->fy = (float)intr[1];
    P->cx = (float)intr[2];
    P->cy = (float)intr[3];
    P->ffl_inv_x = 1.0f / (float)intr[0];
    P->ffl_inv_y = 1.0f / (float)intr[1];
    P->sdf_trunc_f = (float)v->cfg.sdf_trunc;
    P->sdf_trunc_inv_f = 1.0f / P->sdf_trunc_f;
    P->safe_width_f = (float)W - 0.0001f;
    P->safe_height_f = (float)H - 0.0001f;
    P->unit_length = v->cfg.voxel_size * (double)v->cfg.block_size;
    double pose[16];
    hv_invert4x4(T_cw, pose);
    for (int i = 0; i < 12; ++i) P->pose[i] = pose[i];
    P->fx_d = intr[0];
    P->fy_d = intr[1];
    P->cx_d = intr[2];
    P->cy_d = intr[3];
    P->sdf_trunc_d = v->cfg.sdf_trunc;
    P->depth_scale_f = (float)depth_scale;
    P->depth_trunc_d = depth_trunc;
    P->H = H;
    P->W = W;
    P->stride = v->cfg.depth_sampling_stride;
    P->touch_box_bits = v->touch_box_bits;
    P->bgr = v->color_bgr;
    P->depth_is_u16 = depth_dtype == HV_DEPTH_U16;
    const bool whole = v->tile[0] == 0 && v->tile[1] == 0 && v->tile[2] == 0 && v->tile[3] == 0;
    P->tile_u0 = whole ? 0 : v->tile[0];
    P->tile_v0 = whole ? 0 : v->tile[1];
    P->tile_u1 = whole ? W : v->tile[2];
    P->tile_v1 = whole ? H : v->tile[3];
    P->tiled = whole ? 0 : 1;
    P->owner_rank = v->owner_rank;
    P->owner_world = v->owner_world;
    return HV_OK;
}

static int tsdf_launch_touch(hv_volume *v, hipStream_t s, const HvFrameParams &P, int parity, const void *d_depth,
                             const uint8_t *d_rgb) {
    const int64_t npx = (int64_t)P.H * P.W;
    const int n_prep_blocks = (int)((npx + 255) / 256);
    const int ns = ((P.W + P.stride - 1) / P.stride) * ((P.H + P.stride - 1) / P.stride);
    const int n_touch_blocks = (ns * HV_TOUCH_FAN + 255) / 256;
    hipLaunchKernelGGL(k_tsdf_prep_touch, dim3(n_prep_blocks + n_touch_blocks), dim3(256), 0, s, v->table,
                       v->touched_stamp, v->touched_list, parity, d_depth, d_rgb, (uint2 *)v->frame_px, P, n_touch_blocks);
    return HV_OK;
}

int tsdf_multiplier_table(hv_volume *v, const HvFrameParams &P) {
    const float key[4] = {P.cx, P.cy, P.ffl_inv_x, P.ffl_inv_y};
    if (v->mult_table != nullptr && v->mult_W == P.W && v->mult_H == P.H && memcmp(key, v->mult_key, sizeof(key)) == 0)
        return HV_OK;
    const size_t npx = (size_t)P.W * P.H;
    void *buf = v->mult_table;
    int rc = hv_ensure_buffer(v, &buf, &v->mult_table_bytes, npx * sizeof(float));
    if (rc != HV_OK) return rc;
    v->mult_table = (float *)buf;
    hipLaunchKernelGGL(k_tsdf_multiplier_table, dim3((unsigned)((npx + 255) / 256)), dim3(256), 0, v->stream, P,
                       v->mult_table);
    HV_HIP(hipGetLastError());
    memcpy(v->mult_key, key, sizeof(key));
    v->mult_W = P.W;
    v->mult_H = P.H;
    return HV_OK;
}

static int tsdf_launch_integrate(hv_volume *v, const HvFrameParams &P, int parity) {
    const dim3 grid(8192), block(256);
    hv_profile_begin(v);
    hipLaunchKernelGGL(k_tsdf_integrate, grid, block, 0, v->stream, v->table, (const int32_t *)v->touched_list, parity, (char *)v->pool,
                       (const uint2 *)v->frame_px, P, v->d_status, hv_next_status_seq(v));
    hv_profile_end(v, 0);
    HV_HIP(hipGetLastError());
    return HV_OK;
}

static void tsdf_next_frame(hv_volume *v, HvFrameParams &P, int &parity) {
    v->content_version += 1;
    v->frame_counter += 1;
    P.frame_id = v->frame_counter;
    parity = v->frame_counter & 1;
    v->last_touch_parity = parity;
    v->touch_counters_clean = false;
}

int tsdf_rectify(hv_volume *v, hipStream_t s, const void **depth, int depth_dtype, const uint8_t **rgb, int B, int H, int W) {
    if (v->rect_W == 0) return HV_OK;
    HV_REQUIRE(v->rect_W == W && v->rect_H == H, HV_ERR_INVALID, "hv_tsdf_integrate: frames are %dx%d, the rectify maps %dx%d", W, H, v->rect_W, v->rect_H);
    const size_t npx = (size_t)H * W, dsz = depth_dtype == HV_DEPTH_U16 ? 2 : 4;
    const size_t depth_bytes = (npx * dsz * (size_t)B + 255) & ~(size_t)255;
    const size_t want = depth_bytes + npx * 3 * (size_t)B;
    if (v->rect_buf_bytes < want && v->stream_aux) HV_HIP(hipStreamSynchronize(v->stream_aux));
    int rc = hv_ensure_buffer(v, &v->rect_buf, &v->rect_buf_bytes, want);
    if (rc != HV_OK) return rc;
    rc = hv_rectify_frames_device(v, s, *depth, depth_dtype, *rgb, B, H, W, v->rect_buf, (uint8_t *)v->rect_buf + depth_bytes);
    if (rc != HV_OK) return rc;
    *depth = v->rect_buf;
    *rgb = (const uint8_t *)v->rect_buf + depth_bytes;
    return HV_OK;
}

static int tsdf_integrate_one(hv_volume *v, const void *d_depth, int depth_dtype, const uint8_t *d_rgb,
                              int H, int W, const double *intr, const double *T_cw, double depth_scale,
                              double depth_trunc) {
    bool checked = false;
    int rc = hv_capacity_gate(v, &checked);
    if (rc != HV_OK) return rc;
    rc = tsdf_rectify(v, v->stream, &d_depth, depth_dtype, &d_rgb, 1, H, W);
    if (rc != HV_OK) return rc;
    HvFrameParams P;
    make_frame_params(v, H, W, intr, T_cw, depth_scale, depth_trunc, depth_dtype, &P);
    int parity = 0;
    for (int attempt = 0;; ++attempt) {
        tsdf_next_frame(v, P, parity);
        if (attempt > 0) HV_HIP(hipMemsetAsync(&v->table.counters[HV_CNT_TOUCH0], 0, HV_CNT_TOUCH_SPAN_BYTES, v->stream));
        rc = tsdf_launch_touch(v, v->stream, P, parity, d_depth, d_rgb);
        if (rc != HV_OK) return rc;
        if (!checked) break;
        rc = hv_claims_fit(v);
        if (rc == HV_OK) break;
        if (rc != HV_RETRY_CLAIM || attempt >= 8) return rc == HV_RETRY_CLAIM ? HV_ERR_CAPACITY : rc;
        make_frame_params(v, H, W, intr, T_cw, depth_scale, depth_trunc, depth_dtype, &P);
    }
    return tsdf_launch_integrate(v, P, parity);
}

int check_tsdf_args(hv_volume *v, const void *depth, const uint8_t *rgb, int H, int W,
                           const double *intr, const double *T_cw, int frames) {
    HV_REQUIRE(v != nullptr, HV_ERR_INVALID, "hv_tsdf_integrate: null volume");
    HV_REQUIRE(v->cfg.mode == HV_MODE_TSDF, HV_ERR_MODE, "hv_tsdf_integrate: volume is not in TSDF mode");
    HV_REQUIRE(depth != nullptr && rgb != nullptr && intr != nullptr && T_cw != nullptr, HV_ERR_INVALID,
               "[ScalableTSDFVolume::Integrate] Unsupported image format.");
    HV_REQUIRE(H > 0 && W > 0 && frames > 0, HV_ERR_INVALID, "hv_tsdf_integrate: empty image");
    HV_REQUIRE((int64_t)H * W <= v->cfg.max_points, HV_ERR_CAPACITY,
               "hv_tsdf_integrate: image %dx%d exceeds max_points=%lld", W, H, (long long)v->cfg.max_points);
    return HV_OK;
}

extern "C" {

int hv_tsdf_integrate(hv_volume *v, const void *depth, int32_t depth_dtype, const uint8_t *rgb,
                      int32_t height, int32_t width, const double *intr, const double *T_cw,
                      double depth_scale, double depth_trunc, int32_t loc) {
    int rc = check_tsdf_args(v, depth, rgb, height, width, intr, T_cw, 1);
    if (rc != HV_OK) return rc;
    HV_HIP(hipSetDevice(v->device));
    const size_t npx = (size_t)height * width;
    const void *d_depth = nullptr, *d_rgb = nullptr;
    rc = hv_stage_in(v, depth, npx * (depth_dtype == HV_DEPTH_U16 ? 2 : 4), loc, 0, &d_depth);
    if (rc != HV_OK) return rc;
    rc = hv_stage_in(v, rgb, npx * 3, loc, 1, &d_rgb);
    if (rc != HV_OK) return rc;
    return tsdf_integrate_one(v, d_depth, depth_dtype, (const uint8_t *)d_rgb, height, width, intr, T_cw,
                              depth_scale, depth_trunc);
}

}

size_t tsdf_batch_scratch(size_t rec_bytes, size_t npx, int B, size_t *params_offset) {
    const size_t px_bytes = rec_bytes * npx * (size_t)B;
    *params_offset = (px_bytes + 255) & ~(size_t)255;
    return px_bytes + 256 + sizeof(HvFrameParams) * (size_t)B;
}

int tsdf_integrate_batch_impl(hv_volume *v, const void *depth, const void *const *depth_ptrs, int32_t depth_dtype,
                                     const uint8_t *rgb, const void *const *rgb_ptrs, int32_t n_frames, int32_t height,
                                     int32_t width, const double *intr, const double *T_cw, double depth_scale,
                                     double depth_trunc, int32_t loc) {
    int rc = HV_OK;
    HV_HIP(hipSetDevice(v->device));
    const size_t npx = (size_t)height * width;
    const size_t dsz = depth_dtype == HV_DEPTH_U16 ? 2 : 4;
    const void *d_depth = nullptr, *d_rgb = nullptr;
    int host_set = -1;
    if (loc == HV_HOST) {
        rc = hv_stage_frames(v, depth_ptrs, depth, npx * dsz, rgb_ptrs, rgb, npx * 3, n_frames, &d_depth, &d_rgb, &host_set);
        if (rc != HV_OK) return rc;
    } else {
        d_depth = depth;
        d_rgb = rgb;
    }
    if (n_frames == 1) {
        if (host_set >= 0) HV_HIP(hipStreamWaitEvent(v->stream, v->hs_dev_ready[host_set], 0));
        rc = tsdf_integrate_one(v, d_depth, depth_dtype, (const uint8_t *)d_rgb, height, width, intr, T_cw, depth_scale, depth_trunc);
        if (rc != HV_OK) return rc;
        if (host_set >= 0) return hv_stage_frames_consumed(v, host_set, v->stream);
        return HV_OK;
    }
    const bool pipeline_on = !(getenv("HV_TSDF_PIPELINE") && atoi(getenv("HV_TSDF_PIPELINE")) == 0);
    const int sweep_form = getenv("HV_TSDF_SWEEP") && atoi(getenv("HV_TSDF_SWEEP")) == 2 ? 2 : 4;
    const bool rec12 = sweep_form == 4;
    const size_t rec_bytes = rec12 ? 12 : 8;
    const int general = getenv("HV_TSDF_BATCH_GENERAL") ? atoi(getenv("HV_TSDF_BATCH_GENERAL")) : 0;
    const int zs = getenv("HV_TSDF_SWEEP_ZS") ? atoi(getenv("HV_TSDF_SWEEP_ZS")) : (v->owner_world >= 4 ? 2 : 1);
    const int sweep_grid = 65536;
    bool chain_ok = v->pipe_armed && v->pipe_version == v->content_version;
    v->content_version += 1;
    const int BMAX = HV_BATCH_MAX;
    for (int f0 = 0; f0 < n_frames; f0 += BMAX) {
        const int B = std::min(BMAX, n_frames - f0);
        bool checked = false;
        const int64_t max_before = v->cfg.max_blocks;
        rc = hv_capacity_gate(v, &checked);
        if (rc != HV_OK) return rc;
        if (v->cfg.max_blocks != max_before) chain_ok = false;
        const bool overlap = pipeline_on && chain_ok && !checked;
        if (v->stream_aux == nullptr) {
            HV_HIP(hipStreamCreateWithFlags(&v->stream_aux, hipStreamNonBlocking));
            HV_HIP(hipEventCreateWithFlags(&v->ev_prep, hipEventDisableTiming));
            HV_HIP(hipEventCreateWithFlags(&v->ev_presweep, hipEventDisableTiming));
        }
        hipStream_t ps = overlap ? v->stream_aux : v->stream;
        bool overlap_this = overlap;
        const int parity = v->batch_parity & 1;
        v->batch_parity = parity ^ 1;
        int32_t *d_list = v->touched_list + (size_t)parity * (size_t)v->cfg.max_blocks;
        unsigned long long *d_mask_rw = (unsigned long long *)v->touched_mask + (size_t)parity * (size_t)v->table_capacity;
        if (overlap) HV_HIP(hipStreamWaitEvent(v->stream_aux, v->ev_presweep, 0));
        if (host_set >= 0) HV_HIP(hipStreamWaitEvent(ps, v->hs_dev_ready[host_set], 0));
        const int ri = v->params_idx;
        v->params_idx = (ri + 1) & 3;
        if (v->pinned_params[ri] == nullptr) {
            HV_HIP(hipHostMalloc(&v->pinned_params[ri], sizeof(HvFrameParams) * BMAX));
            HV_HIP(hipEventCreateWithFlags(&v->params_ev[ri], hipEventDisableTiming));
        } else {
            HV_HIP(hipEventSynchronize(v->params_ev[ri]));
        }
        HvFrameParams *params = (HvFrameParams *)v->pinned_params[ri];
        for (int f = 0; f < B; ++f) {
            make_frame_params(v, height, width, intr, T_cw + 16 * (size_t)(f0 + f), depth_scale, depth_trunc, depth_dtype,
                              &params[f]);
            v->frame_counter += 1;
            params[f].frame_id = v->frame_counter;
        }
        int batch_stamp = v->frame_counter;
        v->last_touch_parity = parity;
        {
            const float *before = v->mult_table;
            const int mw = v->mult_W, mh = v->mult_H;
            float key_before[4];
            memcpy(key_before, v->mult_key, sizeof(key_before));
            rc = tsdf_multiplier_table(v, params[0]);
            if (rc != HV_OK) return rc;
            if (before != v->mult_table || mw != v->mult_W || mh != v->mult_H || memcmp(key_before, v->mult_key, sizeof(key_before)) != 0) {
                if (ps != v->stream) HV_HIP(hipStreamSynchronize(v->stream_aux));
                ps = v->stream;
                overlap_this = false;
                if (host_set >= 0) HV_HIP(hipStreamWaitEvent(ps, v->hs_dev_ready[host_set], 0));
            }
        }
        const float *d_mult = v->mult_table;
        size_t params_off = 0;
        const size_t want = tsdf_batch_scratch(rec_bytes, npx, B, &params_off);
        void **bb = parity ? &v->batch_buf2 : &v->batch_buf;
        size_t *bb_bytes = parity ? &v->batch_buf2_bytes : &v->batch_buf_bytes;
        if (*bb_bytes < want && v->stream_aux) HV_HIP(hipStreamSynchronize(v->stream_aux));
        rc = hv_ensure_buffer(v, bb, bb_bytes, want);
        if (rc != HV_OK) return rc;
        uint2 *d_px = (uint2 *)*bb;
        HvFrameParams *d_params = (HvFrameParams *)((char *)*bb + params_off);
        {
            const int n16 = (int)((sizeof(HvFrameParams) * (size_t)B + 15) / 16);
            hipLaunchKernelGGL(k_upload_words, dim3(1), dim3(256), 0, ps, (const uint4 *)params, (uint4 *)d_params, n16);
        }
        HV_HIP(hipEventRecord(v->params_ev[ri], ps));
        const int n_prep_blocks = (int)((npx + 1023) / 1024);
        const int n_touch_blocks = (hv_touch_patches(width, height, v->cfg.depth_sampling_stride) + 3) / 4;
        const void *c_depth = (const char *)d_depth + npx * dsz * (size_t)f0;
        const uint8_t *c_rgb = (const uint8_t *)d_rgb + npx * 3 * (size_t)f0;
        rc = tsdf_rectify(v, ps, &c_depth, depth_dtype, &c_rgb, B, height, width);
        if (rc != HV_OK) return rc;
        for (int attempt = 0;; ++attempt) {
            if (!v->touch_counters_clean) HV_HIP(hipMemsetAsync(&v->table.counters[HV_CNT_TOUCH0], 0, HV_CNT_TOUCH_SPAN_BYTES, v->stream));
            v->touch_counters_clean = true;
            hipLaunchKernelGGL(k_tsdf_prep_touch_batch, dim3((n_prep_blocks + n_touch_blocks) * B), dim3(256), 0, ps,
                               v->table, v->touched_stamp, d_mask_rw, d_list, batch_stamp,
                               (const char *)c_depth, (int64_t)(npx * dsz), c_rgb, d_px, (const HvFrameParams *)d_params, n_prep_blocks, n_touch_blocks, B, parity,
                               rec12 ? d_mult : (const float *)nullptr);
            if (!checked) break;
            rc = hv_claims_fit(v);
            if (rc == HV_OK) break;
            if (rc != HV_RETRY_CLAIM || attempt >= 8) return rc == HV_RETRY_CLAIM ? HV_ERR_CAPACITY : rc;
            v->frame_counter += 1;
            batch_stamp = v->frame_counter;
            v->touch_counters_clean = false;
            d_list = v->touched_list + (size_t)parity * (size_t)v->cfg.max_blocks;
            d_mask_rw = (unsigned long long *)v->touched_mask + (size_t)parity * (size_t)v->table_capacity;
        }
        HV_HIP(hipEventRecord(v->ev_presweep, v->stream));
        if (overlap_this) {
            HV_HIP(hipEventRecord(v->ev_prep, v->stream_aux));
            HV_HIP(hipStreamWaitEvent(v->stream, v->ev_prep, 0));
        }
        chain_ok = true;
        hv_profile_begin(v);
        const unsigned long long *d_mask = d_mask_rw;
        if (sweep_form == 2)
            hipLaunchKernelGGL(k_tsdf_sweep, dim3(sweep_grid), dim3(64 * HV_SWEEP_WAVES), 0, v->stream, v->table, (const int32_t *)d_list, d_mask,
                               (char *)v->pool, (const uint2 *)d_px, (const HvFrameParams *)d_params, B, general, d_mult, parity);
        else if (zs == 2)
            hipLaunchKernelGGL(k_tsdf_sweep_column<2>, dim3(sweep_grid), dim3(64), 0, v->stream, v->table, (const int32_t *)d_list, d_mask,
                               (char *)v->pool, (const uint2 *)d_px, (const HvFrameParams *)d_params, B, general, d_mult, parity);
        else
            hipLaunchKernelGGL(k_tsdf_sweep_column<1>, dim3(sweep_grid), dim3(64), 0, v->stream, v->table, (const int32_t *)d_list, d_mask,
                               (char *)v->pool, (const uint2 *)d_px, (const HvFrameParams *)d_params, B, general, d_mult, parity);
        hv_profile_end(v, B);
        hipLaunchKernelGGL(k_tsdf_batch_finish, dim3(1), dim3(1024), 0, v->stream, v->table, (const int32_t *)d_list, d_mask_rw, parity, v->d_status,
                           hv_next_status_seq(v));
        HV_HIP(hipGetLastError());
    }
    v->pipe_armed = true;
    v->pipe_version = v->content_version;
    if (host_set >= 0) return hv_stage_frames_consumed(v, host_set, v->stream);
    return HV_OK;
}

extern "C" {

int hv_tsdf_integrate_batch(hv_volume *v, const void *depth, int32_t depth_dtype, const uint8_t *rgb,
                            int32_t n_frames, int32_t height, int32_t width, const double *intr,
                            const double *T_cw, double depth_scale, double depth_trunc, int32_t loc) {
    int rc = check_tsdf_args(v, depth, rgb, height, width, intr, T_cw, n_frames);
    if (rc != HV_OK) return rc;
    return tsdf_integrate_batch_impl(v, depth, nullptr, depth_dtype, rgb, nullptr, n_frames, height, width, intr, T_cw, depth_scale,
                                     depth_trunc, loc);
}

int hv_tsdf_integrate_frames(hv_volume *v, const void *const *depth_frames, int32_t depth_dtype, const uint8_t *const *rgb_frames,
                             int32_t n_frames, int32_t height, int32_t width, const double *intr, const double *T_cw,
                             double depth_scale, double depth_trunc) {
    HV_REQUIRE(depth_frames != nullptr && rgb_frames != nullptr && n_frames >= 1, HV_ERR_INVALID, "hv_tsdf_integrate_frames: null argument");
    for (int f = 0; f < n_frames; ++f)
        HV_REQUIRE(depth_frames[f] != nullptr && rgb_frames[f] != nullptr, HV_ERR_INVALID, "hv_tsdf_integrate_frames: null frame %d", f);
    int rc = check_tsdf_args(v, depth_frames[0], rgb_frames[0], height, width, intr, T_cw, n_frames);
    if (rc != HV_OK) return rc;
    return tsdf_integrate_batch_impl(v, nullptr, depth_frames, depth_dtype, nullptr, (const void *const *)rgb_frames, n_frames, height,
                                     width, intr, T_cw, depth_scale, depth_trunc, HV_HOST);
}

int hv_tsdf_set_tile(hv_volume *v, int32_t u0, int32_t v0, int32_t u1, int32_t v1) {
    HV_REQUIRE(v != nullptr, HV_ERR_INVALID, "hv_tsdf_set_tile: null volume");
    HV_REQUIRE(v->cfg.mode == HV_MODE_TSDF, HV_ERR_MODE, "hv_tsdf_set_tile: volume is not in TSDF mode");
    HV_REQUIRE((u0 == 0 && v0 == 0 && u1 == 0 && v1 == 0) || (u0 >= 0 && v0 >= 0 && u1 > u0 && v1 > v0), HV_ERR_INVALID,
               "hv_tsdf_set_tile: empty tile");
    v->tile[0] = u0;
    v->tile[1] = v0;
    v->tile[2] = u1;
    v->tile[3] = v1;
    return HV_OK;
}

int hv_tsdf_set_color_order(hv_volume *v, int32_t bgr) {
    HV_REQUIRE(v != nullptr, HV_ERR_INVALID, "hv_tsdf_set_color_order: null volume");
    HV_REQUIRE(v->cfg.mode == HV_MODE_TSDF, HV_ERR_MODE, "hv_tsdf_set_color_order: volume is not in TSDF mode");
    v->color_bgr = bgr ? 1 : 0;
    return HV_OK;
}

int hv_tsdf_set_owner(hv_volume *v, int32_t rank, int32_t world_size) {
    HV_REQUIRE(v != nullptr, HV_ERR_INVALID, "hv_tsdf_set_owner: null volume");
    HV_REQUIRE(v->cfg.mode == HV_MODE_TSDF, HV_ERR_MODE, "hv_tsdf_set_owner: volume is not in TSDF mode");
    HV_REQUIRE(world_size >= 1 && rank >= 0 && rank < world_size, HV_ERR_INVALID, "hv_tsdf_set_owner: bad rank/world");
    v->owner_rank = rank;
    v->owner_world = world_size;
    return HV_OK;
}

int hv_tsdf_dump(hv_volume *v, int32_t *keys, float *tsdf, float *weight, double *color, int64_t *n_units) {
    HV_REQUIRE(v != nullptr && n_units != nullptr, HV_ERR_INVALID, "hv_tsdf_dump: null argument");
    HV_REQUIRE(v->cfg.mode == HV_MODE_TSDF, HV_ERR_MODE, "hv_tsdf_dump: volume is not in TSDF mode");
    int64_t nb = 0;
    int rc = hv_num_blocks(v, &nb);
    if (rc != HV_OK) return rc;
    *n_units = nb;
    if (nb == 0 || (keys == nullptr && tsdf == nullptr && weight == nullptr && color == nullptr)) return HV_OK;
    std::vector<int32_t> order, xyz;
    rc = hv_tsdf_key_order(v, nb, order, &xyz);
    if (rc != HV_OK) return rc;
    std::vector<char> unit((size_t)HV_TSDF_UNIT_BYTES);
    for (int64_t o = 0; o < nb; ++o) {
        const int64_t i = order[o];
        if (keys) memcpy(keys + o * 3, &xyz[o * 3], 12);
        if (!(tsdf || weight || color)) continue;
        HV_HIP(hipMemcpy(unit.data(), (char *)v->pool + i * unit.size(), unit.size(), hipMemcpyDeviceToHost));
        const float *pt = (const float *)unit.data();
        const uint32_t *pw = (const uint32_t *)(unit.data() + HV_TSDF_PLANE_BYTES);
        const uint32_t *pr = (const uint32_t *)(unit.data() + 2 * HV_TSDF_PLANE_BYTES);
        const uint32_t *pg = (const uint32_t *)(unit.data() + 3 * HV_TSDF_PLANE_BYTES);
        const uint32_t *pb = (const uint32_t *)(unit.data() + 4 * HV_TSDF_PLANE_BYTES);
        for (int x = 0; x < HV_TSDF_R; ++x)
            for (int y = 0; y < HV_TSDF_R; ++y)
                for (int z = 0; z < HV_TSDF_R; ++z) {
                    const int src = hv_tsdf_word(x, y, z);
                    const int64_t dst = o * HV_TSDF_RRR + (x * HV_TSDF_R + y) * HV_TSDF_R + z;
                    if (tsdf) tsdf[dst] = pt[src];
                    if (weight) weight[dst] = (float)pw[src];
                    if (color) {
                        const double w = (double)pw[src];
                        color[dst * 3 + 0] = w > 0 ? (double)pr[src] / w : 0.0;
                        color[dst * 3 + 1] = w > 0 ? (double)pg[src] / w : 0.0;
                        color[dst * 3 + 2] = w > 0 ? (double)pb[src] / w : 0.0;
                    }
                }
    }
    return HV_OK;
}

int hv_tsdf_touched(hv_volume *v, int32_t *keys, int64_t cap, int64_t *n) {
    HV_REQUIRE(v != nullptr && n != nullptr, HV_ERR_INVALID, "hv_tsdf_touched: null argument");
    HV_REQUIRE(v->cfg.mode == HV_MODE_TSDF, HV_ERR_MODE, "hv_tsdf_touched: volume is not in TSDF mode");
    int rc = hv_read_counters(v);
    if (rc != HV_OK) return rc;
    int64_t nt = v->h_counters[HV_CNT_TOUCH(v->last_touch_parity)];
    if (nt > v->cfg.max_blocks) nt = v->cfg.max_blocks;
    *n = nt;
    if (keys == nullptr || nt == 0) return HV_OK;
    std::vector<int32_t> slots((size_t)nt);
    HV_HIP(hipMemcpy(slots.data(), v->touched_list, sizeof(int32_t) * nt, hipMemcpyDeviceToHost));
    std::vector<uint64_t> tkeys((size_t)v->table_capacity);
    HV_HIP(hipMemcpy(tkeys.data(), v->table.keys, sizeof(uint64_t) * v->table_capacity, hipMemcpyDeviceToHost));
    std::vector<std::array<int32_t, 3>> out((size_t)nt);
    for (int64_t i = 0; i < nt; ++i) hv_unpack_key(tkeys[slots[i]], out[i][0], out[i][1], out[i][2]);
    std::sort(out.begin(), out.end());
    const int64_t m = std::min(nt, cap);
    for (int64_t i = 0; i < m; ++i) memcpy(keys + i * 3, out[i].data(), 12);
    return HV_OK;
}

int hv_tsdf_unit_keys(hv_volume *v, int32_t *keys, int64_t cap, int64_t *n) {
    HV_REQUIRE(v != nullptr && n != nullptr, HV_ERR_INVALID, "hv_tsdf_unit_keys: null argument");
    int64_t nb = 0;
    int rc = hv_num_blocks(v, &nb);
    if (rc != HV_OK) return rc;
    *n = nb;
    if (keys == nullptr || nb == 0) return HV_OK;
    std::vector<uint64_t> bkeys((size_t)nb);
    HV_HIP(hipMemcpy(bkeys.data(), v->table.block_keys, sizeof(uint64_t) * nb, hipMemcpyDeviceToHost));
    const int64_t m = std::min(nb, cap);
    for (int64_t i = 0; i < m; ++i) hv_unpack_key(bkeys[i], keys[i * 3], keys[i * 3 + 1], keys[i * 3 + 2]);
    return HV_OK;
}

}
```

pyslam_amd/csrc/hv_tsdf_device.h:

```cpp
#pragma once
#include "hv_common.h"

static constexpr int HV_TOUCH_FAN = 8;
static constexpr uint32_t HV_REC_ONE = 1u << 24;

__device__ __forceinline__ uint32_t hv_colour_order(uint32_t c, int bgr) {
    return bgr ? __builtin_amdgcn_perm(0u, c, 0x03000102u) : c;
}

__device__ __forceinline__ float hv_multiplier(const HvFrameParams &P, int u, int v) {
    const float xx = ((float)u - P.cx) * P.ffl_inv_x;
    const float yy = ((float)v - P.cy) * P.ffl_inv_y;
    return sqrtf(xx * xx + yy * yy + 1.0f);
}

__device__ __forceinline__ float hv_convert_depth(const HvFrameParams &P, const void *depth_raw, int64_t i) {
    float p = P.depth_is_u16 ? (float)((const uint16_t *)depth_raw)[i] : ((const float *)depth_raw)[i];
    p = p / P.depth_scale_f;
    if ((double)p >= P.depth_trunc_d) p = 0.0f;
    return p;
}

__device__ inline bool hv_unit_hits_tile(const HvFrameParams &P, int32_t ux, int32_t uy, int32_t uz) {
    if (P.tile_u0 <= 0 && P.tile_v0 <= 0 && P.tile_u1 >= P.W && P.tile_v1 >= P.H) return true;
// ... 124 lines not shown
                const unsigned long long key = hv_pack_key(ux, uy, uz);
                if (!(P.owner_world > 1 && hv_owner_of(key, P.owner_world) != P.owner_rank)) visit(key, ux, uy, uz);
            } else {
                atomicAdd(&table.counters[HV_CNT_DROPPED], 1);
            }
        }
        __builtin_amdgcn_wave_barrier();
        return;
    }
    const int64_t n0 = (int64_t)hi[0] - lo[0] + 1, n1 = (int64_t)hi[1] - lo[1] + 1, n2 = (int64_t)hi[2] - lo[2] + 1;
    const int64_t count = has ? n0 * n1 * n2 : 0;
    for (int64_t k = 0; __any(k < count); ++k) {
        unsigned long long key = HV_EMPTY_KEY;
        int32_t ux = 0, uy = 0, uz = 0;
        if (k < count) {
            ux = lo[0] + (int32_t)(k / (n1 * n2));
            uy = lo[1] + (int32_t)((k / n2) % n1);
            uz = lo[2] + (int32_t)(k % n2);
            if (hv_key_in_range(ux, uy, uz)) {
                key = hv_pack_key(ux, uy, uz);
                if (P.owner_world > 1 && hv_owner_of(key, P.owner_world) != P.owner_rank) key = HV_EMPTY_KEY;
            } else {
                atomicAdd(&table.counters[HV_CNT_DROPPED], 1);
            }
        }
        bool leader = false;
        unsigned long long remaining = __ballot(key != HV_EMPTY_KEY);
        while (remaining) {
            const int first = __ffsll((long long)remaining) - 1;
            const unsigned long long fkey = __shfl(key, first);
            const unsigned long long same = __ballot(key == fkey);
            if (lane == first) leader = true;
            remaining &= ~same;
        }
        if (leader) visit(key, ux, uy, uz);
    }
}

__device__ __forceinline__ void hv_div2(float a0, float a1, float b, float &q0, float &q1) {
    float r = __builtin_amdgcn_rcpf(b);
    const float e = fmaf(-b, r, 1.0f);
    r = fmaf(e, r, r);
    float q = a0 * r;
    float rem = fmaf(-b, q, a0);
    q = fmaf(rem, r, q);
    rem = fmaf(-b, q, a0);
    q0 = fmaf(rem, r, q);
    q = a1 * r;
    rem = fmaf(-b, q, a1);
    q = fmaf(rem, r, q);
    rem = fmaf(-b, q, a1);
    q1 = fmaf(rem, r, q);
}

__device__ __forceinline__ float hv_div1(float a, float b) {
    float r = __builtin_amdgcn_rcpf(b);
    const float e = fmaf(-b, r, 1.0f);
    r = fmaf(e, r, r);
    float q = a * r;
    float rem = fmaf(-b, q, a);
    q = fmaf(rem, r, q);
    rem = fmaf(-b, q, a);
    return fmaf(rem, r, q);
}

__device__ __forceinline__ void hv_tsdf_apply(bool valid, float t, uint32_t c, float &tsdf, uint32_t &w, uint32_t &sr,
                                              uint32_t &sg, uint32_t &sb) {
    if (!valid) return;
    const float wf = (float)w;
    const float num = tsdf * wf + t;
    tsdf = (w < (1u << 24)) ? hv_div1(num, wf + 1.0f) : num / (wf + 1.0f);
    w += 1u;
    sr += c & 255u;
    sg += (c >> 8) & 255u;
    sb += (c >> 16) & 255u;
}


__device__ __forceinline__ float hv_sqrt_ge1(float x) {
    const float s = __builtin_amdgcn_sqrtf(x);
    const float sd = __uint_as_float(__float_as_uint(s) - 1u);
    const float su = __uint_as_float(__float_as_uint(s) + 1u);
    const float vp = fmaf(-sd, s, x);
    const float vs = fmaf(-su, s, x);
    float r = (vp <= 0.0f) ? sd : s;
    r = (vs > 0.0f) ? su : r;
    return r;
}

template <bool EXACT, bool MT, bool REC12 = false>
__device__ __forceinline__ bool hv_tsdf_eval_fast(const HvFrameParams &P, const uint2 *__restrict__ frame_px,
                                                  const float *__restrict__ mult, float pc0, float pc1, float pc2,
                                                  float &t, uint32_t &rgb) {
    const float a0 = pc0 * P.fx, a1 = pc1 * P.fy;
    float q0, q1;
    hv_div2(a0, a1, pc2, q0, q1);
    if (EXACT) {
        const bool tiny = !(pc2 >= 0x1p-20f);
        const float e0 = a0 / pc2, e1 = a1 / pc2;
        q0 = tiny ? e0 : q0;
        q1 = tiny ? e1 : q1;
    }
    const float u_f = q0 + P.cx + 0.5f;
    const float v_f = q1 + P.cy + 0.5f;
    const uint32_t lo = __float_as_uint(0.0001f);
    const bool in_u = (__float_as_uint(u_f) - lo) < (__float_as_uint(P.safe_width_f) - lo);
    const bool in_v = (__float_as_uint(v_f) - lo) < (__float_as_uint(P.safe_height_f) - lo);
    bool ok = (int)(pc2 > 0.0f) & (int)in_u & (int)in_v;
    const int u = (int)u_f;
    const int v = (int)v_f;
    if (EXACT && P.tiled) {
        const bool in_tile_u = (int)(u >= P.tile_u0) & (int)(u < P.tile_u1);
        const bool in_tile_v = (int)(v >= P.tile_v0) & (int)(v < P.tile_v1);
        ok = (int)ok & (int)in_tile_u & (int)in_tile_v;
    }
    const uint32_t off = ok ? (uint32_t)v * (uint32_t)P.W + (uint32_t)u : 0u;
    uint2 rec;
    float m;
    if (REC12) {
        const uint32_t *r3 = (const uint32_t *)frame_px + (size_t)off * 3;
        rec = make_uint2(r3[0], r3[1]);
        m = __uint_as_float(r3[2]);
    } else {
        rec = frame_px[off];
    }
    const float d = __uint_as_float(rec.x);
    if (REC12) {
    } else if (MT) {
        m = mult[off];
    } else {
        const float xx = ((float)u - P.cx) * P.ffl_inv_x;
        const float yy = ((float)v - P.cy) * P.ffl_inv_y;
        m = hv_sqrt_ge1(xx * xx + yy * yy + 1.0f);
    }
    const float sdf = (d - pc2) * m;
    ok = (int)ok & (int)(d > 0.0f) & (int)(sdf > -P.sdf_trunc_f);
    t = fminf(sdf * P.sdf_trunc_inv_f, 1.0f);
    rgb = rec.y;
    return ok;
}

__device__ __forceinline__ void hv_tsdf_apply_fast(bool ok, float t, uint32_t rgb, float &tsdf, float &wf, uint32_t &sr,
                                                   uint32_t &sg, uint32_t &sb) {
    const float wf1 = wf + 1.0f;
    const float nt = hv_div1(tsdf * wf + t, wf1);
    tsdf = ok ? nt : tsdf;
    wf = ok ? wf1 : wf;
    const uint32_t c = ok ? rgb : 0u;
    sr += c & 255u;
    sg += (c >> 8) & 255u;
    sb += (c >> 16) & 255u;
}

__device__ __forceinline__ void hv_pack_px4(const HvFrameParams &P, const int f, const int64_t i0, const void *depth_f,
                                            const uint8_t *rgb_f, uint2 *__restrict__ frame_px, const float *__restrict__ mult12) {
    const int64_t npx = (int64_t)P.H * P.W;
    if (i0 >= npx) return;
    if (P.tiled && (P.W & 3) == 0) {
        const int u = (int)(i0 % P.W), v = (int)(i0 / P.W);
        if (u + 3 < P.tile_u0 - 4 || u >= P.tile_u1 + 4 || v < P.tile_v0 - 4 || v >= P.tile_v1 + 4) return;
    }
    uint2 *dst = frame_px + (int64_t)f * npx + i0;
    uint32_t *dst12 = (uint32_t *)frame_px + ((int64_t)f * npx + i0) * 3;
    if (i0 + 4 <= npx && (npx & 3) == 0) {
        const uint32_t *c4 = (const uint32_t *)(rgb_f + i0 * 3);
        const uint32_t w0 = c4[0], w1 = c4[1], w2 = c4[2];
        const uint32_t col[4] = {hv_colour_order(w0 & 0xffffffu, P.bgr) | HV_REC_ONE,
                                 hv_colour_order((w0 >> 24) | ((w1 & 0xffffu) << 8), P.bgr) | HV_REC_ONE,
                                 hv_colour_order((w1 >> 16) | ((w2 & 0xffu) << 16), P.bgr) | HV_REC_ONE,
                                 hv_colour_order(w2 >> 8, P.bgr) | HV_REC_ONE};
        float d[4];
        if (P.depth_is_u16) {
            const uint2 raw = *(const uint2 *)((const uint16_t *)depth_f + i0);
            d[0] = (float)(raw.x & 0xffffu); d[1] = (float)(raw.x >> 16);
            d[2] = (float)(raw.y & 0xffffu); d[3] = (float)(raw.y >> 16);
        } else {
            const float4 raw = *(const float4 *)((const float *)depth_f + i0);
            d[0] = raw.x; d[1] = raw.y; d[2] = raw.z; d[3] = raw.w;
        }
#pragma unroll
        for (int k = 0; k < 4; ++k) {
            d[k] = d[k] / P.depth_scale_f;
            if ((double)d[k] >= P.depth_trunc_d) d[k] = 0.0f;
        }
        if (mult12 != nullptr) {
            const float4 m4 = *(const float4 *)(mult12 + i0);
            ((uint4 *)dst12)[0] = make_uint4(__float_as_uint(d[0]), col[0], __float_as_uint(m4.x), __float_as_uint(d[1]));
            ((uint4 *)dst12)[1] = make_uint4(col[1], __float_as_uint(m4.y), __float_as_uint(d[2]), col[2]);
            ((uint4 *)dst12)[2] = make_uint4(__float_as_uint(m4.z), __float_as_uint(d[3]), col[3], __float_as_uint(m4.w));
        } else {
            ((uint4 *)dst)[0] = make_uint4(__float_as_uint(d[0]), col[0], __float_as_uint(d[1]), col[1]);
            ((uint4 *)dst)[1] = make_uint4(__float_as_uint(d[2]), col[2], __float_as_uint(d[3]), col[3]);
        }
    } else {
        for (int64_t i = i0; i < npx && i < i0 + 4; ++i) {
            const uint8_t *c = rgb_f + i * 3;
            uint2 rec;
            rec.x = __float_as_uint(hv_convert_depth(P, depth_f, i));
            rec.y = hv_colour_order((uint32_t)c[0] | ((uint32_t)c[1] << 8) | ((uint32_t)c[2] << 16), P.bgr) | HV_REC_ONE;
            if (mult12 != nullptr) {
                uint32_t *r3 = (uint32_t *)frame_px + ((int64_t)f * npx + i) * 3;
                r3[0] = rec.x;
                r3[1] = rec.y;
                r3[2] = __float_as_uint(mult12[i]);
            } else {
                frame_px[(int64_t)f * npx + i] = rec;
            }
        }
    }
}

static constexpr int HV_BATCH_MAX = 64;
int make_frame_params(hv_volume *v, int H, int W, const double *intr, const double *T_cw, double depth_scale, double depth_trunc,
                      int depth_dtype, HvFrameParams *P);
int tsdf_multiplier_table(hv_volume *v, const HvFrameParams &P);
int tsdf_rectify(hv_volume *v, hipStream_t s, const void **depth, int depth_dtype, const uint8_t **rgb, int B, int H, int W);
int check_tsdf_args(hv_volume *v, const void *depth, const uint8_t *rgb, int H, int W, const double *intr, const double *T_cw,
                    int frames);
size_t tsdf_batch_scratch(size_t rec_bytes, size_t npx, int B, size_t *params_offset);
int tsdf_integrate_batch_impl(hv_volume *v, const void *depth, const void *const *depth_ptrs, int32_t depth_dtype, const uint8_t *rgb,
                              const void *const *rgb_ptrs, int32_t n_frames, int32_t height, int32_t width, const double *intr,
                              const double *T_cw, double depth_scale, double depth_trunc, int32_t loc);
```

pyslam_amd/volumetric.py:

```python
import contextlib
import ctypes
import functools
import typing

import numpy as np

from . import _lib as L


def _result_array(shape, dtype):
    import os

    n = int(np.prod(shape))
    if n * np.dtype(dtype).itemsize >= (1 << 20) and os.environ.get("PYSLAM_AMD_PINNED_RESULTS", "1") != "0":
        try:
            import torch

            if torch.cuda.is_available():
                return torch.empty(tuple(shape), dtype=getattr(torch, np.dtype(dtype).name), pin_memory=True).numpy()
        except Exception:
            pass
    return np.empty(shape, dtype)


# ... 204 lines not shown
        self.gradient = gradient
        self.color = color
        self.weight = weight
        self.status = status

    def __repr__(self):
        return f"SampleResult(n={len(self.sdf)}, gradient={self.gradient is not None}, color={self.color is not None})"


class FrameCheckStats(_Stats):

    __slots__ = ("invalid", "unknown", "consistent", "in_front", "behind")


class FrameCheck:

    def __init__(self, sdf, cls, stats):
        self.sdf = sdf
        self.cls = cls
        self.stats = stats

    invalid = property(lambda self: self.stats.invalid)
    unknown = property(lambda self: self.stats.unknown)
    consistent = property(lambda self: self.stats.consistent)
    in_front = property(lambda self: self.stats.in_front)
    behind = property(lambda self: self.stats.behind)

    def __repr__(self):
        return f"FrameCheck({', '.join(f'{name}={getattr(self.stats, name)}' for name in self.stats.__slots__)})"


LOOKUP_MISSING, LOOKUP_OWN, LOOKUP_NEAR, LOOKUP_INVALID = L.HV_LOOKUP_MISSING, L.HV_LOOKUP_OWN, L.HV_LOOKUP_NEAR, L.HV_LOOKUP_INVALID


class LookupStats(_Stats):

    __slots__ = ("points", "own", "near", "missing", "invalid")


class VoxelLookup:

    def __init__(self, status, count, position, color, class_id, object_id, confidence, stats):
        self.status = status
        self.count = count
        self.position = position
        self.color = color
        self.class_id = class_id
        self.object_id = object_id
        self.confidence = confidence
        self.stats = stats

    def __repr__(self):
        return f"VoxelLookup(n={len(self.status)}, labels={self.class_id is not None}, stats={self.stats})"


DIST_UNKNOWN, DIST_FREE, DIST_INSIDE, DIST_SITE = L.HV_DIST_UNKNOWN, L.HV_DIST_FREE, L.HV_DIST_INSIDE, L.HV_DIST_SITE


class DistanceFieldStats(_Stats):

    __slots__ = ("unknown", "free", "inside", "sites", "far")


class DistanceField:

    def __init__(self, distance, dist2, cls, origin, shape, voxel_length, radius, stats):
        self.distance = distance
        self.dist2 = dist2
        self.cls = cls
        self.origin = np.asarray(origin, np.int64).reshape(3)
        self.shape = tuple(int(n) for n in shape)
        self.voxel_length = float(voxel_length)
        self.radius = int(radius)
        self.max_distance = float(self.radius * np.float64(voxel_length))
        self.stats = stats

    def cell_of(self, points):
        p = np.asarray(points, np.float64).reshape(-1, 3)
        with np.errstate(invalid="ignore"):
            q = np.floor(p / np.float64(self.voxel_length))
            ok = np.isfinite(q).all(axis=1) & (np.abs(q) < 2.0 ** 62).all(axis=1)
        idx = np.where(ok[:, None], q, 0.0).astype(np.int64) - self.origin
        inside = ok & ((idx >= 0) & (idx < np.asarray(self.shape, np.int64))).all(axis=1)
        return idx, inside

    def lookup(self, points):
        if self.distance is None:
            raise ValueError("DistanceField.lookup: the field was computed without 'distance'")
        idx, inside = self.cell_of(points)
        out = np.full(len(idx), np.float32(self.radius) * np.float32(self.voxel_length), np.float32)
        i = idx[inside]
        if _is_torch(self.distance):
            import torch

            t = torch.from_numpy(i).to(self.distance.device)
            out[inside] = self.distance[t[:, 0], t[:, 1], t[:, 2]].cpu().numpy()
        else:
            out[inside] = self.distance[i[:, 0], i[:, 1], i[:, 2]]
        return out

    def __repr__(self):
        return f"DistanceField(origin={self.origin.tolist()}, shape={self.shape}, max_distance={self.max_distance:g})"


class SurfaceComponentsStats(_Stats):

    __slots__ = ("units", "sites", "components", "largest")


class SurfaceComponents:

    def __init__(self, seed, sites, lo, hi, site_index, site_label, stats, voxel_length):
        self.seed = seed
        self.sites = sites
        self.lo = lo
        self.hi = hi
        self.site_index = site_index
        self.site_label = site_label
        self.stats = stats
        self.voxel_length = float(voxel_length)

    def __len__(self):
        return int(self.stats.components)

    def __repr__(self):
        return f"SurfaceComponents(components={self.stats.components}, sites={self.stats.sites}, largest={self.stats.largest})"


class ComponentRemovalStats(typing.NamedTuple):

    components: int
    components_removed: int
    sites: int
    sites_removed: int
    voxels_reset: int
    units_changed: int
    units_emptied: int


def _packed_operand(buf):
    if _is_torch(buf):
        import torch

        if buf.dtype != torch.uint8 or buf.dim() != 1:
            raise ValueError(f"a packed map is a 1-D uint8 buffer, got {buf.dtype} with shape {tuple(buf.shape)}")
        return buf.contiguous() if buf.is_cuda else buf.contiguous().numpy()
    a = buf if isinstance(buf, np.ndarray) else np.frombuffer(buf, dtype=np.uint8)
    if a.dtype != np.uint8 or a.ndim != 1:
        raise ValueError(f"a packed map is a 1-D uint8 buffer, got {a.dtype} with shape {a.shape}")
    return np.ascontiguousarray(a)


_UNIT_KEY_BIAS = 1 << 20


def unit_range_of_bounds(bounds, voxel_length, resolution=16):
    try:
        lo_m, hi_m = bounds
        lo_m = np.asarray(lo_m, dtype=np.float64).reshape(-1)
        hi_m = np.asarray(hi_m, dtype=np.float64).reshape(-1)
    except (TypeError, ValueError) as e:
        raise ValueError(f"bounds must be (min_xyz, max_xyz): {e}") from None
    if lo_m.shape != (3,) or hi_m.shape != (3,):
        raise ValueError("bounds must be (min_xyz, max_xyz) with three coordinates each")
    L_unit = np.float64(voxel_length) * np.float64(resolution)
    if not (np.isfinite(L_unit) and L_unit > 0.0):
        raise ValueError(f"bad unit length {L_unit}")
    if not (np.all(np.isfinite(lo_m)) and np.all(np.isfinite(hi_m))):
        raise ValueError("bounds must be finite")
    if np.any(lo_m > hi_m):
        raise ValueError(f"bounds: min {lo_m.tolist()} exceeds max {hi_m.tolist()}")
    lo, hi = np.floor(lo_m / L_unit), np.floor(hi_m / L_unit)
    if np.any(lo < -_UNIT_KEY_BIAS) or np.any(hi >= _UNIT_KEY_BIAS):
        raise ValueError(f"bounds reach beyond the unit keys [-2^20, 2^20): units {lo.tolist()} .. {hi.tolist()}")
    return lo.astype(np.int32), hi.astype(np.int32)


_TRACK_HEAD = (("level", int), ("iteration", int), ("status", int), ("inliers", int), ("valid", int), ("sq_error", float))
_REGISTER_HEAD = (("iteration", int), ("status", int), ("inliers", int), ("candidates", int), ("sq_error", float))


def _trace_rows(rows, head=_TRACK_HEAD):
    out = []
    iu = np.triu_indices(6)
    k = len(head)
    for r in rows:
        H = np.zeros((6, 6))
        H[iu] = r[k + 16:k + 37]
        H = H + np.triu(H, 1).T
        out.append({name: kind(r[i]) for i, (name, kind) in enumerate(head)})
        out[-1].update(A=r[k:k + 16].reshape(4, 4).copy(), H=H, g=r[k + 37:k + 43].copy(), xi=r[k + 43:k + 49].copy())
        if len(r) > L.HV_TRACK_TRACE_STRIDE:
            out[-1].update(photometric_inliers=int(r[56]), sq_intensity_error=float(r[57]))
    return out


_NOTHING_TO_ORDER = contextlib.nullcontext()


class _Volume:

    def __init__(self, mode, voxel_size, sdf_trunc, block_size, stride, device, max_blocks, max_points):
        lib = L.load()
        cfg = L.HvConfig()
        lib.hv_default_config(mode, ctypes.byref(cfg))
        cfg.device = int(device)
        cfg.voxel_size = float(voxel_size)
        cfg.sdf_trunc = float(sdf_trunc)
        cfg.block_size = int(block_size)
        cfg.depth_sampling_stride = int(stride)
        if max_blocks is not None:
            cfg.max_blocks = int(max_blocks)
        if max_points is not None:
            cfg.max_points = int(max_points)
        self._lib = lib
        self._cfg = cfg
        handle = ctypes.c_void_p()
        L.check(lib.hv_create(ctypes.byref(cfg), ctypes.byref(handle)))
        self._h = handle

    def close(self):
        if getattr(self, "_h", None):
            self._lib.hv_destroy(self._h)
            self._h = None

    def __del__(self):
        try:
            self.close()
        except Exception:
            pass

    def _int64(self, fn, *args):
        n = ctypes.c_int64()
        L.check(fn(self._h, *args, ctypes.byref(n)))
        return n.value

    def _sized_fetch(self, call, *specs):
        n = ctypes.c_int64()
        L.check(call(*(None,) * len(specs), 0, ctypes.byref(n)))
        out = [np.zeros((n.value,) + tuple(row), dtype) for row, dtype in specs]
        if n.value:
            L.check(call(*(L.ptr(a) for a in out), n.value, ctypes.byref(n)))
        return out

    def _device(self):
        if getattr(self, "_torch_device", None) is None:
            import torch

            self._torch_device = torch.device("cuda", int(self._cfg.device))
        return self._torch_device

    def _results(self, spec, device, pinned=True, synchronize=True):
        if not device:
            make = _result_array if pinned else np.empty
            return {name: None if s is None else make(s[0], s[1]) for name, s in spec.items()}
        import torch

        dev = self._device()
        out = {name: None if s is None else torch.empty(tuple(s[0]), dtype=getattr(torch, np.dtype(s[1]).name.replace("uint32", "int32")),
                                                        device=dev) for name, s in spec.items()}
        if synchronize:
            torch.cuda.current_stream(dev).synchronize()
        return out

    def num_blocks(self):
        return self._int64(self._lib.hv_num_blocks)

    def max_blocks(self):
        return self._int64(self._lib.hv_max_blocks)

    def reserve_blocks(self, new_max_blocks):
        L.check(self._lib.hv_reserve_blocks(self._h, int(new_max_blocks)))

    def synchronize(self):
        L.check(self._lib.hv_synchronize(self._h))

    def set_stream(self, stream_handle):
        L.check(self._lib.hv_set_stream(self._h, ctypes.c_void_p(int(stream_handle))))

    def register_host_memory(self, address, nbytes):
        L.check(self._lib.hv_host_register(ctypes.c_void_p(int(address)), int(nbytes)))

    def unregister_host_memory(self, address):
        L.check(self._lib.hv_host_unregister(ctypes.c_void_p(int(address))))

    def _torch_stream(self, device):
        import torch

        h = int(self._lib.hv_get_stream(self._h) or 0)
        if getattr(self, "_ts_key", None) != (h, device):
            self._ts = torch.cuda.ExternalStream(h, device=device) if h else torch.cuda.default_stream(device)
            self._ts_key = (h, device)
        return self._ts

    def adopt_torch_stream(self):
        import torch

        if getattr(self, "_adopted", None) is None:
            self._adopted = torch.cuda.Stream(self._device())
            self.set_stream(self._adopted.cuda_stream)
        return self._adopted

    def _torch_in(self, *tensors):
        import torch

        for t in tensors:
# ... 1200 lines not shown
```

Before: 64690 frames/s.

## Precompute per-unit sweep plan with depth-tile culling of behind and outside frames

```diff
diff --git a/include/hipvol.h b/include/hipvol.h
--- a/include/hipvol.h
+++ b/include/hipvol.h
@@ -168,6 +168,8 @@
                              int32_t n_frames, int32_t height, int32_t width, const double *intr, const double *T_cw,
                              double depth_scale, double depth_trunc);
 
+int hv_tsdf_plan_counts(hv_volume *v, int64_t *pairs, int64_t *behind, int64_t *outside);
+
 #define HV_TSDF_DEINTEGRATE_MAX_FRAMES 64
 typedef struct hv_deintegrate_stats {
     int64_t units_listed;
diff --git a/pyslam_amd/_lib.py b/pyslam_amd/_lib.py
--- a/pyslam_amd/_lib.py
+++ b/pyslam_amd/_lib.py
@@ -278,6 +278,7 @@
     "hv_tsdf_integrate": (_i32, [_vp, _vp, _i32, _vp, _i32, _i32, _vp, _vp, _f64, _f64, _i32]),
     "hv_tsdf_integrate_batch": (_i32, [_vp, _vp, _i32, _vp, _i32, _i32, _i32, _vp, _vp, _f64, _f64, _i32]),
     "hv_tsdf_integrate_frames": (_i32, [_vp, _vp, _i32, _vp, _i32, _i32, _i32, _vp, _vp, _f64, _f64]),
+    "hv_tsdf_plan_counts": (_i32, [_vp, _pi64, _pi64, _pi64]),
     "hv_tsdf_set_color_order": (_i32, [_vp, _i32]),
     "hv_host_register": (_i32, [_vp, _i64]),
     "hv_host_unregister": (_i32, [_vp]),
diff --git a/pyslam_amd/csrc/hv_common.h b/pyslam_amd/csrc/hv_common.h
--- a/pyslam_amd/csrc/hv_common.h
+++ b/pyslam_amd/csrc/hv_common.h
@@ -103,9 +103,12 @@
     HV_CNT_PROB_NODES = 9,
     HV_CNT_TOUCH0 = 32,
     HV_CNT_TOUCH1 = 64,
-    HV_CNT_COUNT = 96
+    HV_CNT_PLAN0 = 96,
+    HV_CNT_PLAN1 = 128,
+    HV_CNT_COUNT = 160
 };
 #define HV_CNT_TOUCH(set) (HV_CNT_TOUCH0 + 32 * (set))
+#define HV_CNT_PLAN(set) (HV_CNT_PLAN0 + 32 * (set))
 static constexpr int HV_TSDF_SETS = 2;
 static constexpr size_t HV_CNT_TOUCH_SPAN_BYTES = sizeof(int32_t) * (32 * (HV_TSDF_SETS - 1) + 1);
 
@@ -351,6 +354,9 @@
     size_t batch_buf_bytes = 0;
     void *batch_buf2 = nullptr;
     size_t batch_buf2_bytes = 0;
+    void *plan_buf = nullptr;
+    size_t plan_buf_bytes = 0;
+    int plan_last_set = -1;
     hipEvent_t ev_h2d = nullptr;
     hipStream_t stream_aux = nullptr;
     hipEvent_t ev_prep = nullptr;
diff --git a/pyslam_amd/csrc/hv_core.hip b/pyslam_amd/csrc/hv_core.hip
--- a/pyslam_amd/csrc/hv_core.hip
+++ b/pyslam_amd/csrc/hv_core.hip
@@ -674,7 +674,7 @@
                     v->touched_stamp, v->touched_list, v->touched_mask, v->frame_px,
                     v->stage_a, v->stage_b, v->sort_keys_in, v->sort_keys_out, v->sort_vals_in,
                     v->sort_vals_out, v->sort_tmp, v->scratch_points, v->scratch_colors, v->out_a,
-                    v->out_b, v->out_c, v->rect_map_x, v->rect_map_y, v->rect_buf, v->batch_buf, v->assoc_buf, v->mult_table, v->bins.cnt, v->bins.inl, v->bins.touched, v->bins.len, v->bins.pg_keys, v->bins.pg_data, v->bin_rec, v->batch_buf2, v->unit_masks, v->occ, v->semb_tasks, v->table.prob_nodes, v->shadow_ring, v->mc_cache, v->pc_cache, v->kf_buf, v->halo_plan, v->raycast_buf, v->track_buf, v->deint_buf, v->sample_buf, v->dist_buf};
+                    v->out_b, v->out_c, v->rect_map_x, v->rect_map_y, v->rect_buf, v->batch_buf, v->assoc_buf, v->mult_table, v->bins.cnt, v->bins.inl, v->bins.touched, v->bins.len, v->bins.pg_keys, v->bins.pg_data, v->bin_rec, v->batch_buf2, v->unit_masks, v->occ, v->semb_tasks, v->table.prob_nodes, v->shadow_ring, v->mc_cache, v->pc_cache, v->kf_buf, v->halo_plan, v->raycast_buf, v->track_buf, v->deint_buf, v->sample_buf, v->dist_buf, v->plan_buf};
     for (void *b : bufs)
         if (b) (void)hipFree(b);
     if (v->h_counters) (void)hipHostFree(v->h_counters);
@@ -721,6 +721,7 @@
     v->extract_epoch += 1;
     v->frame_counter = 0;
     v->merge_stamp = 0;
+    v->plan_last_set = -1;
     HV_HIP(hipStreamSynchronize(v->stream));
     memset(v->h_status, 0, sizeof(HvStatus));
     v->status_seq_issued = v->status_seq_seen = 0;
diff --git a/pyslam_amd/csrc/hv_tsdf.hip b/pyslam_amd/csrc/hv_tsdf.hip
--- a/pyslam_amd/csrc/hv_tsdf.hip
+++ b/pyslam_amd/csrc/hv_tsdf.hip
@@ -244,7 +244,7 @@
                                                                 uint2 *__restrict__ frame_px,
                                                                 const HvFrameParams *__restrict__ Ps, int n_prep_blocks,
                                                                 int n_touch_blocks, int n_frames, int parity,
-                                                                const float *__restrict__ mult12) {
+                                                                const float *__restrict__ mult12, uint32_t *__restrict__ tile_max) {
     int f, bx;
     const bool touch_role = (int)blockIdx.x < n_touch_blocks * n_frames;
     if (touch_role) {
@@ -260,7 +260,7 @@
     const void *depth_f = depth_raw + (int64_t)f * depth_stride;
     const uint8_t *rgb_f = rgb + (int64_t)f * npx * 3;
     if (!touch_role) {
-        hv_pack_px4(P, f, ((int64_t)bx * blockDim.x + threadIdx.x) * 4, depth_f, rgb_f, frame_px, mult12);
+        hv_pack_px4(P, f, ((int64_t)bx * blockDim.x + threadIdx.x) * 4, depth_f, rgb_f, frame_px, mult12, tile_max);
         return;
     }
     __shared__ HvTouchScratch scratch[4];
@@ -296,6 +296,103 @@
     const unsigned g = j / (G * parts), within = j % (G * parts);
     t = (int)((g * 8 + xcd) * G + within / parts);
     part = (int)(within % parts);
+}
+
+struct HvSweepPlan {
+    unsigned long long mask, interior;
+};
+static constexpr int HV_PLAN_MAX_TILES = 64;
+
+__global__ __launch_bounds__(256, 8) void k_tsdf_sweep_plan(HvTable table, const int32_t *__restrict__ list,
+                                                          const unsigned long long *__restrict__ frame_mask,
+                                                          const HvFrameParams *__restrict__ Ps, int n_frames,
+                                                          const uint32_t *__restrict__ tile_max, int cull,
+                                                          HvSweepPlan *__restrict__ plan, uint32_t *__restrict__ plan_near, int parity) {
+    int n_units = table.counters[HV_CNT_TOUCH(parity)];
+    if (n_units > table.max_blocks) n_units = table.max_blocks;
+    const int lane = threadIdx.x & 63;
+    const int wave = __builtin_amdgcn_readfirstlane((int)blockIdx.x * 4 + (int)(threadIdx.x >> 6)), n_waves = (int)gridDim.x * 4;
+    const HvFrameParams &P0 = Ps[0];
+    const float vl = P0.voxel_length_f, hl = P0.half_voxel_length_f;
+    const double unit_length = P0.unit_length;
+    const float Fx = P0.fx, Fy = P0.fy, Cx = P0.cx, Cy = P0.cy;
+    const float lo_uf = fmaxf(0.0001f, (float)P0.tile_u0), lo_vf = fmaxf(0.0001f, (float)P0.tile_v0);
+    const float hi_uf = fminf(P0.safe_width_f, (float)P0.tile_u1), hi_vf = fminf(P0.safe_height_f, (float)P0.tile_v1);
+    const float trunc = P0.sdf_trunc_f;
+    const float near_z = fmaxf(0.03f, 1.25f * trunc);
+    const float last_u = (float)(P0.W - 1), last_v = (float)(P0.H - 1);
+    const int TW = hv_tiles_across(P0.W);
+    const bool mine = lane < n_frames;
+    float e[12];
+#pragma unroll
+    for (int k = 0; k < 12; ++k) e[k] = mine ? Ps[lane].ext[k] : 0.0f;
+    uint32_t n_before = 0, n_behind = 0, n_outside = 0;
+    for (int task = wave; task < 4 * n_units; task += n_waves) {
+        const int t = task >> 2, cg = task & 3;
+        const int32_t slot = list[t];
+        const unsigned long long unit_mask = frame_mask[slot];
+        int32_t ux, uy, uz;
+        hv_unpack_key(table.keys[slot], ux, uy, uz);
+        const double o0 = (double)ux * unit_length;
+        const float by = (float)((double)hl + (double)uy * unit_length), bz = (float)((double)hl + (double)uz * unit_length);
+        const bool visits = mine && ((unit_mask >> lane) & 1ull);
+        {
+            bool near = false, interior = false, behind = false, outside = false;
+            if (visits) {
+                const float bx = (float)((double)(hl + vl * (float)(cg * 4)) + o0);
+                const float zmin = (e[8] * bx + e[9] * by + e[10] * bz + e[11]) + fminf(e[8] * (3.0f * vl), 0.f) +
+                                   fminf(e[9] * (15.0f * vl), 0.f) + fminf(e[10] * (15.0f * vl), 0.f);
+                near = !(zmin > near_z);
+                if (!near) {
+                    float umin = 3.0e38f, umax = -3.0e38f, vmin = 3.0e38f, vmax = -3.0e38f;
+#pragma unroll 1
+                    for (int c = 0; c < 8; ++c) {
+                        const float qx = bx + ((c & 1) ? 3.0f * vl : 0.0f), qy = by + ((c & 2) ? 15.0f * vl : 0.0f), qz = bz + ((c & 4) ? 15.0f * vl : 0.0f);
+                        const float c2 = e[8] * qx + e[9] * qy + e[10] * qz + e[11];
+                        const float rz = 1.0f / c2;
+                        const float cu = (e[0] * qx + e[1] * qy + e[2] * qz + e[3]) * Fx * rz + Cx + 0.5f;
+                        const float cv = (e[4] * qx + e[5] * qy + e[6] * qz + e[7]) * Fy * rz + Cy + 0.5f;
+                        umin = fminf(umin, cu); umax = fmaxf(umax, cu);
+                        vmin = fminf(vmin, cv); vmax = fmaxf(vmax, cv);
+                    }
+                    interior = umin >= lo_uf + 2.0f && umax <= hi_uf - 2.0f && vmin >= lo_vf + 2.0f && vmax <= hi_vf - 2.0f;
+                    if (cull && !interior) outside = umax < lo_uf - 2.0f || umin >= hi_uf + 2.0f || vmax < lo_vf - 2.0f || vmin >= hi_vf + 2.0f;
+                    if (cull && !outside) {
+                        const int tx0 = (int)fminf(fmaxf(umin - 2.0f, 0.0f), last_u) / HV_TILE_PX, tx1 = (int)fminf(fmaxf(umax + 2.0f, 0.0f), last_u) / HV_TILE_PX;
+                        const int ty0 = (int)fminf(fmaxf(vmin - 2.0f, 0.0f), last_v) / HV_TILE_PX, ty1 = (int)fminf(fmaxf(vmax + 2.0f, 0.0f), last_v) / HV_TILE_PX;
+                        if ((tx1 - tx0 + 1) * (ty1 - ty0 + 1) <= HV_PLAN_MAX_TILES) {
+                            uint32_t dmax = 0u;
+                            for (int ty = ty0; ty <= ty1; ++ty)
+                                for (int tx = tx0; tx <= tx1; ++tx) dmax = max(dmax, tile_max[(ty * TW + tx) * HV_TILE_FRAMES + lane]);
+                            const float M = fabsf(e[8] * bx) + fabsf(e[9] * by) + fabsf(e[10] * bz) + fabsf(e[11]) +
+                                            (3.0f * fabsf(e[8]) + 15.0f * fabsf(e[9]) + 15.0f * fabsf(e[10])) * vl;
+                            const float slack = fmaxf(0.25f * vl, 0x1p-18f * M);
+                            behind = zmin - trunc - slack >= __uint_as_float(dmax);
+                        }
+                    }
+                }
+            }
+            const unsigned long long m_behind = __ballot(behind), m_outside = __ballot(outside), m_interior = __ballot(interior);
+            n_before += (uint32_t)__popcll(unit_mask);
+            n_behind += (uint32_t)__popcll(m_behind);
+            n_outside += (uint32_t)__popcll(m_outside);
+            const bool near_any = __any(near);
+            if (lane == 0) {
+                plan[task] = HvSweepPlan{unit_mask & ~(m_behind | m_outside), m_interior};
+                plan_near[task] = near_any ? 1u : 0u;
+            }
+        }
+    }
+    __shared__ uint32_t wg_counts[3];
+    if (threadIdx.x < 3) wg_counts[threadIdx.x] = 0u;
+    __syncthreads();
+    if (lane == 0 && n_before != 0u) {
+        atomicAdd(&wg_counts[0], n_before);
+        atomicAdd(&wg_counts[1], n_behind);
+        atomicAdd(&wg_counts[2], n_outside);
+    }
+    __syncthreads();
+    if (threadIdx.x < 3 && wg_counts[threadIdx.x] != 0u) atomicAdd(&table.counters[HV_CNT_PLAN(parity) + threadIdx.x], (int32_t)wg_counts[threadIdx.x]);
 }
 
 static constexpr int HV_SWEEP_ZH = 4;
@@ -531,8 +628,8 @@
 
 template <int ZS>
 __global__ __launch_bounds__(64, 4) void k_tsdf_sweep_column(
-    HvTable table, const int32_t *__restrict__ list, const unsigned long long *__restrict__ frame_mask,
-    char *__restrict__ pool, const uint2 *__restrict__ frame_px, const HvFrameParams *__restrict__ Ps, int n_frames,
+    HvTable table, const int32_t *__restrict__ list, const HvSweepPlan *__restrict__ plan, const uint32_t *__restrict__ plan_near,
+    char *__restrict__ pool, const uint2 *__restrict__ frame_px, const HvFrameParams *__restrict__ Ps,
     int general, const float *__restrict__ mult, int parity) {
     constexpr int GV = 4;
     static_assert(ZS == 1 || ZS == 2, "whole columns or z halves");
@@ -554,7 +651,6 @@
     const uint32_t lim_u = hi_uf > lo_uf ? __float_as_uint(hi_uf) - lo_u : 0u, lim_v = hi_vf > lo_vf ? __float_as_uint(hi_vf) - lo_v : 0u;
     const uint32_t W24 = (uint32_t)P0.W;
     const float ntrunc = -P0.sdf_trunc_f, tinv = P0.sdf_trunc_inv_f;
-    const float near_z = fmaxf(0.03f, 1.25f * P0.sdf_trunc_f);
     const int n_items = hv_sweep_items(n_units, PARTS);
     for (int item = blockIdx.x; item < n_items; item += gridDim.x) {
         int t, part;
@@ -566,37 +662,14 @@
         const int x = cg * 4 + (lane >> 4);
         const int y = lane & 15;
         const int32_t idx = table.vals[slot];
-        unsigned long long mask = frame_mask[slot];
+        const HvSweepPlan pl = plan[t * 4 + cg];
+        unsigned long long mask = pl.mask;
         if (idx < 0 || mask == 0ull) continue;
+        const unsigned long long interior_mask = pl.interior;
+        const bool near_any = plan_near[t * 4 + cg] != 0u;
         int32_t ux, uy, uz;
         hv_unpack_key(table.keys[slot], ux, uy, uz);
         const double o0 = (double)ux * unit_length, o1 = (double)uy * unit_length, o2 = (double)uz * unit_length;
-        bool near = false;
-        bool interior = false;
-        if (lane < n_frames && ((mask >> lane) & 1ull)) {
-            const HvFrameParams &Pl = Ps[lane];
-            const float bx = (float)((double)(hl + vl * (float)(cg * 4)) + o0), by = (float)((double)hl + o1),
-                        bz = (float)((double)(hl + vl * (float)z0) + o2);
-            const float zmin = (Pl.ext[8] * bx + Pl.ext[9] * by + Pl.ext[10] * bz + Pl.ext[11]) + fminf(Pl.ext[8] * (3.0f * vl), 0.f) +
-                               fminf(Pl.ext[9] * (15.0f * vl), 0.f) + fminf(Pl.ext[10] * ((float)(ZH - 1) * vl), 0.f);
-            near = !(zmin > near_z);
-            if (!near) {
-                float umin = 3.0e38f, umax = -3.0e38f, vmin = 3.0e38f, vmax = -3.0e38f;
-#pragma unroll
-                for (int c = 0; c < 8; ++c) {
-                    const float qx = bx + ((c & 1) ? 3.0f * vl : 0.0f), qy = by + ((c & 2) ? 15.0f * vl : 0.0f), qz = bz + ((c & 4) ? (float)(ZH - 1) * vl : 0.0f);
-                    const float c2 = Pl.ext[8] * qx + Pl.ext[9] * qy + Pl.ext[10] * qz + Pl.ext[11];
-                    const float rz = 1.0f / c2;
-                    const float cu = (Pl.ext[0] * qx + Pl.ext[1] * qy + Pl.ext[2] * qz + Pl.ext[3]) * F.x * rz + C.x + 0.5f;
-                    const float cv = (Pl.ext[4] * qx + Pl.ext[5] * qy + Pl.ext[6] * qz + Pl.ext[7]) * F.y * rz + C.y + 0.5f;
-                    umin = fminf(umin, cu); umax = fmaxf(umax, cu);
-                    vmin = fminf(vmin, cv); vmax = fmaxf(vmax, cv);
-                }
-                interior = umin >= lo_uf + 2.0f && umax <= hi_uf - 2.0f && vmin >= lo_vf + 2.0f && vmax <= hi_vf - 2.0f;
-            }
-        }
-        const unsigned long long interior_mask = __ballot(interior);
-        const bool near_any = __any(near);
         char *unit = pool + (int64_t)idx * HV_TSDF_UNIT_BYTES;
         const int wordb = z0 * HV_TSDF_RR + cg * 64 + lane;
         const float p0 = (float)((double)(hl + vl * (float)x) + o0);
@@ -779,8 +852,11 @@
     }
 }
 
-__global__ __launch_bounds__(256) void k_upload_words(const uint4 *__restrict__ src, uint4 *__restrict__ dst, int n16) {
-    for (int i = threadIdx.x; i < n16; i += 256) dst[i] = src[i];
+__global__ __launch_bounds__(1024) void k_upload_words(const uint4 *__restrict__ src, uint4 *__restrict__ dst, int n16,
+                                                        uint4 *__restrict__ zero, int zero16, int32_t *__restrict__ plan_counters) {
+    for (int i = threadIdx.x; i < n16; i += 1024) dst[i] = src[i];
+    for (int i = threadIdx.x; i < zero16; i += 1024) zero[i] = make_uint4(0u, 0u, 0u, 0u);
+    if (plan_counters != nullptr && threadIdx.x < 3) plan_counters[threadIdx.x] = 0;
 }
 
 __global__ __launch_bounds__(1024) void k_tsdf_batch_finish(HvTable table, const int32_t *__restrict__ list,
@@ -906,6 +982,7 @@
     P.frame_id = v->frame_counter;
     parity = v->frame_counter & 1;
     v->last_touch_parity = parity;
+    v->plan_last_set = -1;
     v->touch_counters_clean = false;
 }
 
@@ -1018,6 +1095,7 @@
     const size_t rec_bytes = rec12 ? 12 : 8;
     const int general = getenv("HV_TSDF_BATCH_GENERAL") ? atoi(getenv("HV_TSDF_BATCH_GENERAL")) : 0;
     const int zs = getenv("HV_TSDF_SWEEP_ZS") ? atoi(getenv("HV_TSDF_SWEEP_ZS")) : (v->owner_world >= 4 ? 2 : 1);
+    const int plan_cull = !(getenv("HV_TSDF_PLAN_CULL") && atoi(getenv("HV_TSDF_PLAN_CULL")) == 0) && general == 0;
     const int sweep_grid = 65536;
     bool chain_ok = v->pipe_armed && v->pipe_version == v->content_version;
     v->content_version += 1;
@@ -1076,7 +1154,10 @@
         }
         const float *d_mult = v->mult_table;
         size_t params_off = 0;
-        const size_t want = tsdf_batch_scratch(rec_bytes, npx, B, &params_off);
+        size_t want = tsdf_batch_scratch(rec_bytes, npx, B, &params_off);
+        const size_t tile_off = (want + 255) & ~(size_t)255;
+        const size_t tile_bytes = rec12 ? sizeof(uint32_t) * HV_TILE_FRAMES * (size_t)hv_tiles_across(width) * (size_t)hv_tiles_across(height) : 0;
+        want = tile_off + tile_bytes;
         void **bb = parity ? &v->batch_buf2 : &v->batch_buf;
         size_t *bb_bytes = parity ? &v->batch_buf2_bytes : &v->batch_buf_bytes;
         if (*bb_bytes < want && v->stream_aux) HV_HIP(hipStreamSynchronize(v->stream_aux));
@@ -1084,9 +1165,11 @@
         if (rc != HV_OK) return rc;
         uint2 *d_px = (uint2 *)*bb;
         HvFrameParams *d_params = (HvFrameParams *)((char *)*bb + params_off);
+        uint32_t *d_tile_max = rec12 ? (uint32_t *)((char *)*bb + tile_off) : nullptr;
         {
             const int n16 = (int)((sizeof(HvFrameParams) * (size_t)B + 15) / 16);
-            hipLaunchKernelGGL(k_upload_words, dim3(1), dim3(256), 0, ps, (const uint4 *)params, (uint4 *)d_params, n16);
+            hipLaunchKernelGGL(k_upload_words, dim3(1), dim3(1024), 0, ps, (const uint4 *)params, (uint4 *)d_params, n16, (uint4 *)d_tile_max,
+                               (int)(tile_bytes / 16), rec12 ? &v->table.counters[HV_CNT_PLAN(parity)] : (int32_t *)nullptr);
         }
         HV_HIP(hipEventRecord(v->params_ev[ri], ps));
         const int n_prep_blocks = (int)((npx + 1023) / 1024);
@@ -1101,7 +1184,7 @@
             hipLaunchKernelGGL(k_tsdf_prep_touch_batch, dim3((n_prep_blocks + n_touch_blocks) * B), dim3(256), 0, ps,
                                v->table, v->touched_stamp, d_mask_rw, d_list, batch_stamp,
                                (const char *)c_depth, (int64_t)(npx * dsz), c_rgb, d_px, (const HvFrameParams *)d_params, n_prep_blocks, n_touch_blocks, B, parity,
-                               rec12 ? d_mult : (const float *)nullptr);
+                               rec12 ? d_mult : (const float *)nullptr, d_tile_max);
             if (!checked) break;
             rc = hv_claims_fit(v);
             if (rc == HV_OK) break;
@@ -1112,6 +1195,20 @@
             d_list = v->touched_list + (size_t)parity * (size_t)v->cfg.max_blocks;
             d_mask_rw = (unsigned long long *)v->touched_mask + (size_t)parity * (size_t)v->table_capacity;
         }
+        HvSweepPlan *d_plan = nullptr;
+        uint32_t *d_plan_near = nullptr;
+        v->plan_last_set = -1;
+        if (rec12) {
+            const size_t set_bytes = ((sizeof(HvSweepPlan) + sizeof(uint32_t)) * 4 * (size_t)v->cfg.max_blocks + 255) & ~(size_t)255;
+            if (v->plan_buf_bytes < set_bytes * HV_TSDF_SETS && v->stream_aux) HV_HIP(hipStreamSynchronize(v->stream_aux));
+            rc = hv_ensure_buffer(v, &v->plan_buf, &v->plan_buf_bytes, set_bytes * HV_TSDF_SETS);
+            if (rc != HV_OK) return rc;
+            d_plan = (HvSweepPlan *)((char *)v->plan_buf + set_bytes * (size_t)parity);
+            d_plan_near = (uint32_t *)(d_plan + 4 * (size_t)v->cfg.max_blocks);
+            hipLaunchKernelGGL(k_tsdf_sweep_plan, dim3(2048), dim3(256), 0, ps, v->table, (const int32_t *)d_list, (const unsigned long long *)d_mask_rw,
+                               (const HvFrameParams *)d_params, B, (const uint32_t *)d_tile_max, plan_cull, d_plan, d_plan_near, parity);
+            v->plan_last_set = parity;
+        }
         HV_HIP(hipEventRecord(v->ev_presweep, v->stream));
         if (overlap_this) {
             HV_HIP(hipEventRecord(v->ev_prep, v->stream_aux));
@@ -1124,11 +1221,13 @@
             hipLaunchKernelGGL(k_tsdf_sweep, dim3(sweep_grid), dim3(64 * HV_SWEEP_WAVES), 0, v->stream, v->table, (const int32_t *)d_list, d_mask,
                                (char *)v->pool, (const uint2 *)d_px, (const HvFrameParams *)d_params, B, general, d_mult, parity);
         else if (zs == 2)
-            hipLaunchKernelGGL(k_tsdf_sweep_column<2>, dim3(sweep_grid), dim3(64), 0, v->stream, v->table, (const int32_t *)d_list, d_mask,
-                               (char *)v->pool, (const uint2 *)d_px, (const HvFrameParams *)d_params, B, general, d_mult, parity);
+            hipLaunchKernelGGL(k_tsdf_sweep_column<2>, dim3(sweep_grid), dim3(64), 0, v->stream, v->table, (const int32_t *)d_list,
+                               (const HvSweepPlan *)d_plan, (const uint32_t *)d_plan_near, (char *)v->pool, (const uint2 *)d_px,
+                               (const HvFrameParams *)d_params, general, d_mult, parity);
         else
-            hipLaunchKernelGGL(k_tsdf_sweep_column<1>, dim3(sweep_grid), dim3(64), 0, v->stream, v->table, (const int32_t *)d_list, d_mask,
-                               (char *)v->pool, (const uint2 *)d_px, (const HvFrameParams *)d_params, B, general, d_mult, parity);
+            hipLaunchKernelGGL(k_tsdf_sweep_column<1>, dim3(sweep_grid), dim3(64), 0, v->stream, v->table, (const int32_t *)d_list,
+                               (const HvSweepPlan *)d_plan, (const uint32_t *)d_plan_near, (char *)v->pool, (const uint2 *)d_px,
+                               (const HvFrameParams *)d_params, general, d_mult, parity);
         hv_profile_end(v, B);
         hipLaunchKernelGGL(k_tsdf_batch_finish, dim3(1), dim3(1024), 0, v->stream, v->table, (const int32_t *)d_list, d_mask_rw, parity, v->d_status,
                            hv_next_status_seq(v));
@@ -1161,6 +1260,21 @@
     if (rc != HV_OK) return rc;
     return tsdf_integrate_batch_impl(v, nullptr, depth_frames, depth_dtype, nullptr, (const void *const *)rgb_frames, n_frames, height,
                                      width, intr, T_cw, depth_scale, depth_trunc, HV_HOST);
+}
+
+int hv_tsdf_plan_counts(hv_volume *v, int64_t *pairs, int64_t *behind, int64_t *outside) {
+    HV_REQUIRE(v != nullptr && pairs != nullptr && behind != nullptr && outside != nullptr, HV_ERR_INVALID, "hv_tsdf_plan_counts: null argument");
+    HV_REQUIRE(v->cfg.mode == HV_MODE_TSDF, HV_ERR_MODE, "hv_tsdf_plan_counts: volume is not in TSDF mode");
+    *pairs = *behind = *outside = 0;
+    if (v->plan_last_set < 0) return HV_OK;
+    HV_HIP(hipSetDevice(v->device));
+    int rc = hv_read_counters(v);
+    if (rc != HV_OK) return rc;
+    const int32_t *cnt = &v->h_counters[HV_CNT_PLAN(v->plan_last_set)];
+    *pairs = cnt[0];
+    *behind = cnt[1];
+    *outside = cnt[2];
+    return HV_OK;
 }
 
 int hv_tsdf_set_tile(hv_volume *v, int32_t u0, int32_t v0, int32_t u1, int32_t v1) {
diff --git a/pyslam_amd/csrc/hv_tsdf_device.h b/pyslam_amd/csrc/hv_tsdf_device.h
--- a/pyslam_amd/csrc/hv_tsdf_device.h
+++ b/pyslam_amd/csrc/hv_tsdf_device.h
@@ -300,8 +300,23 @@
     sb += (c >> 16) & 255u;
 }
 
+static constexpr int HV_TILE_PX = 16;
+static constexpr int HV_TILE_FRAMES = 64;
+__host__ __device__ inline int hv_tiles_across(int n_px) { return (n_px + HV_TILE_PX - 1) / HV_TILE_PX; }
+__device__ __forceinline__ uint32_t hv_tile_depth(const float d) {
+    if (!(fabsf(d) < __builtin_inff())) return 0x7f800000u;
+    return d > 0.0f ? __float_as_uint(d) : 0u;
+}
+__device__ __forceinline__ int hv_tile_of_pixel(const int W, const int64_t i) {
+    return (int)(i / W) / HV_TILE_PX * hv_tiles_across(W) + (int)(i % W) / HV_TILE_PX;
+}
+__device__ __forceinline__ void hv_tile_max_put(uint32_t *__restrict__ tile_max, const int tile, const int f, const uint32_t bits) {
+    if (bits != 0u) atomicMax(&tile_max[(int64_t)tile * HV_TILE_FRAMES + f], bits);
+}
+
 __device__ __forceinline__ void hv_pack_px4(const HvFrameParams &P, const int f, const int64_t i0, const void *depth_f,
-                                            const uint8_t *rgb_f, uint2 *__restrict__ frame_px, const float *__restrict__ mult12) {
+                                            const uint8_t *rgb_f, uint2 *__restrict__ frame_px, const float *__restrict__ mult12,
+                                            uint32_t *__restrict__ tile_max = nullptr) {
     const int64_t npx = (int64_t)P.H * P.W;
     if (i0 >= npx) return;
     if (P.tiled && (P.W & 3) == 0) {
@@ -331,6 +346,28 @@
             d[k] = d[k] / P.depth_scale_f;
             if ((double)d[k] >= P.depth_trunc_d) d[k] = 0.0f;
         }
+        if (tile_max != nullptr) {
+            if ((P.W & 15) == 0 && !P.tiled) {
+                uint32_t m = max(max(hv_tile_depth(d[0]), hv_tile_depth(d[1])), max(hv_tile_depth(d[2]), hv_tile_depth(d[3])));
+                m = max(m, (uint32_t)__shfl_xor((int)m, 1));
+                m = max(m, (uint32_t)__shfl_xor((int)m, 2));
+                if ((i0 & 15) == 0) hv_tile_max_put(tile_max, hv_tile_of_pixel(P.W, i0), f, m);
+            } else {
+                int tile = hv_tile_of_pixel(P.W, i0);
+                uint32_t m = hv_tile_depth(d[0]);
+#pragma unroll
+                for (int k = 1; k < 4; ++k) {
+                    const int tk = hv_tile_of_pixel(P.W, i0 + k);
+                    if (tk != tile) {
+                        hv_tile_max_put(tile_max, tile, f, m);
+                        tile = tk;
+                        m = 0u;
+                    }
+                    m = max(m, hv_tile_depth(d[k]));
+                }
+                hv_tile_max_put(tile_max, tile, f, m);
+            }
+        }
         if (mult12 != nullptr) {
             const float4 m4 = *(const float4 *)(mult12 + i0);
             ((uint4 *)dst12)[0] = make_uint4(__float_as_uint(d[0]), col[0], __float_as_uint(m4.x), __float_as_uint(d[1]));
@@ -346,6 +383,7 @@
             uint2 rec;
             rec.x = __float_as_uint(hv_convert_depth(P, depth_f, i));
             rec.y = hv_colour_order((uint32_t)c[0] | ((uint32_t)c[1] << 8) | ((uint32_t)c[2] << 16), P.bgr) | HV_REC_ONE;
+            if (tile_max != nullptr) hv_tile_max_put(tile_max, hv_tile_of_pixel(P.W, i), f, hv_tile_depth(__uint_as_float(rec.x)));
             if (mult12 != nullptr) {
                 uint32_t *r3 = (uint32_t *)frame_px + ((int64_t)f * npx + i) * 3;
                 r3[0] = rec.x;
@@ -359,6 +397,7 @@
 }
 
 static constexpr int HV_BATCH_MAX = 64;
+static_assert(HV_TILE_FRAMES == HV_BATCH_MAX, "the tile maxima hold one word per frame of a batch");
 int make_frame_params(hv_volume *v, int H, int W, const double *intr, const double *T_cw, double depth_scale, double depth_trunc,
                       int depth_dtype, HvFrameParams *P);
 int tsdf_multiplier_table(hv_volume *v, const HvFrameParams &P);
diff --git a/pyslam_amd/volumetric.py b/pyslam_amd/volumetric.py
--- a/pyslam_amd/volumetric.py
+++ b/pyslam_amd/volumetric.py
@@ -380,6 +380,12 @@
 
 
 _UNIT_KEY_BIAS = 1 << 20
+
+
+def tsdf_plan_counts(volume):
+    n = [ctypes.c_int64(0) for _ in range(3)]
+    L.check(volume._lib.hv_tsdf_plan_counts(volume._h, *[ctypes.byref(x) for x in n]))
+    return tuple(int(x.value) for x in n)
 
 
 def unit_range_of_bounds(bounds, voxel_length, resolution=16):
```

Result: slower. 63390 frames/s (-2.0%).
